# MarcoMeter/episodic-transformer-memory-ppo

Hardware: AMD Instinct MI355X
Metric: env-steps/sec (whole node) MinigridMemory 3x84x84 (higher is better)
Workload: dtype f32

## Files before the change

episodic-transformer-memory-ppo_amd/csrc/conv_b3.hip:

```cpp
#include "etm_common.h"

#include <utility>

namespace {
typedef __bf16 bf16x8 __attribute__((ext_vector_type(8)));
typedef unsigned u32x4 __attribute__((ext_vector_type(4)));
typedef unsigned u32x2 __attribute__((ext_vector_type(2)));

struct B3Args {
  const float *x;
  const long long *img_index;
  const unsigned short *wp;
  const float *bias;
  const float *ymask;
  const unsigned *bits_in;
  const unsigned *src_bits;
  unsigned *bits_out;
  float *out;
  int N, n_groups;
};

__device__ __forceinline__ unsigned b3_cvt_pk(float a, float b) {
  unsigned r;
  asm("v_cvt_pk_bf16_f32 %0, %1, %2" : "=v"(r) : "v"(a), "v"(b));
  return r;
}
__device__ __forceinline__ void b3_split_pair(float a, float b, unsigned &h, unsigned &m, unsigned &l) {
  h = b3_cvt_pk(a, b);
  a -= __uint_as_float(h << 16); b -= __uint_as_float(h & 0xffff0000u);
  m = b3_cvt_pk(a, b);
  a -= __uint_as_float(m << 16); b -= __uint_as_float(m & 0xffff0000u);
  l = b3_cvt_pk(a, b);
}

template <class F, int... I>
__device__ __forceinline__ void b3_for_impl(F &&f, std::integer_sequence<int, I...>) { (f(std::integral_constant<int, I>{}), ...); }
template <int N, class F>
__device__ __forceinline__ void b3_for(F &&f) { b3_for_impl(f, std::make_integer_sequence<int, N>{}); }

template <bool DGRAD, int C, int HW, int KS, int S, int COUT, int G_, int BAND = 0, int WPC_ = 1, bool SWZ_ = false>
struct B3Geo {
  static constexpr int G = G_, WPC = WPC_;
  static constexpr bool SWZ = SWZ_;
  static constexpr bool U8 = false;
  static constexpr int HOUT = (HW - KS) / S + 1;
  static constexpr int T = KS / S;
  static constexpr int CI = DGRAD ? COUT : C;
  static constexpr int HI = DGRAD ? HOUT : HW;
  static constexpr bool THREE = CI == 3;
  static constexpr int RS = DGRAD ? HI + T - 1 : HI;
  static constexpr int NB = BAND > 0 ? HOUT / BAND : 1;
  static constexpr int HROWS = BAND > 0 ? (BAND - 1) * S + KS : HI;
  static constexpr int ROW0 = BAND * S;
  static constexpr int SLOTS = DGRAD ? (HI + 2 * (T - 1) - 1) * RS + HI + 2 * (T - 1) : HROWS * HI;
  static constexpr int CPB = THREE ? 6 : SWZ ? CI * 2 : (CI + 8) * 2;
  static constexpr int IMGB = (SLOTS * CPB + 15) / 16 * 16;
  static constexpr int PLANE = G * IMGB;
  static constexpr int HO = DGRAD ? HI + T - 1 : HOUT;
  static constexpr int PIXI = HO * HO;
  static constexpr int PIX = BAND > 0 ? BAND * HO : PIXI, M = G * PIX, MT = (M + 31) / 32;
  static constexpr int NOUT = DGRAD ? S * S * C : COUT;
  static constexpr int NT = NOUT / 32, RP = NT >= 4 ? 1 : 4 / NT, TPW = (MT + RP - 1) / RP;
  static constexpr int TAPS = DGRAD ? T : KS;
  static constexpr int K = TAPS * TAPS * CI, KSTEPS = K / 16;
  static constexpr int KPT = THREE ? 1 : CI / 16;
  static constexpr int Q_IMG = HI * HI * CI / 4;
  static constexpr int Q_UNIT = HROWS * HI * CI / 4;
  static constexpr int Q_ROW0 = ROW0 * HI * CI / 4;
  static constexpr int NQ = (G * Q_UNIT + 255) / 256;
  static constexpr int LPK = (NQ + KSTEPS - 1) / KSTEPS;
  static constexpr int HRES = DGRAD ? S * HO : HO;
  static constexpr int CRES = DGRAD ? C : COUT;
  static_assert(K % 16 == 0 && NOUT % 32 == 0 && (THREE || CI % 16 == 0) && (NT == 1 || NT == 2 || NT == 4), "layer geometry");
  static_assert(!DGRAD || (HW % S == 0 && KS % S == 0 && HI + T - 1 == HW / S && Q_IMG % 8 == 0), "backward-data: class grids tile the input");
  static_assert(!SWZ || (!DGRAD && CI == 32 && SLOTS % 16 == 0 && IMGB == SLOTS * CPB), "swizzled slots: 64-byte pixels of four chunks");
  static_assert(BAND == 0 || (!DGRAD && G == 1 && HOUT % BAND == 0 && (ROW0 * HI * CI) % 4 == 0 && (HROWS * HI * CI) % 4 == 0), "bands: forward, one unit per group");

  static constexpr int slot(int y, int x) {
    if (DGRAD) return (y + T - 1) * RS + (x + T - 1);
    if (S == 2) return y * HI + (x & 1) * (HI / 2) + (x >> 1);
    return y * HI + x;
  }
  static constexpr int tap_slot(int ks) {
    const int tap = ks / KPT, ty = tap / TAPS, tx = tap % TAPS;
    if (!DGRAD && S == 2) return ty * HI + (tx & 1) * (HI / 2) + (tx >> 1);
    return ty * RS + tx;
  }
  static constexpr int tap_bytes(int ks) {
    const int tap = ks / KPT, cg = ks % KPT, ty = tap / TAPS, tx = tap % TAPS;
    int so = ty * RS + tx;
    if (!DGRAD && S == 2) so = ty * HI + (tx & 1) * (HI / 2) + (tx >> 1);
    return so * CPB + cg * 32;
  }
};

template <class Base>
struct B3GeoBytes : Base {
  static constexpr bool U8 = true;
};

template <class L, bool DGRAD, int C, int S>
__global__ __launch_bounds__(256, L::WPC) void conv_b3_kernel(const B3Args p) {
  constexpr bool U8 = L::U8;
  static_assert(!U8 || (L::THREE && !DGRAD && L::G == 1 && (L::Q_IMG * 4) % 16 == 0 && (L::Q_UNIT * 4) % 16 == 0 && (L::Q_ROW0 * 4) % 16 == 0),
                "byte images: layer 1 forward, units of whole 16-byte loads");
  constexpr int Q16 = L::Q_UNIT / 4;
  constexpr int G = L::G, TPW = L::TPW, NT = L::NT, RP = L::RP, KSTEPS = L::KSTEPS, NQ = U8 ? (Q16 + 255) / 256 : L::NQ, PD = 3;
  constexpr int LPK = U8 ? (NQ + KSTEPS - 1) / KSTEPS : L::LPK;
  extern __shared__ __attribute__((aligned(16))) unsigned char lds[];
  const int tid = threadIdx.x, lane = tid & 63, col = lane & 31, half = lane >> 5;
  const int wave = __builtin_amdgcn_readfirstlane(tid >> 6);
  const int ct = wave % NT, rp = wave / NT;

  if (DGRAD) {
    for (int e = tid; e < 3 * L::PLANE / 16; e += 256) reinterpret_cast<u32x4 *>(lds)[e] = u32x4{0u, 0u, 0u, 0u};
    __syncthreads();
  }

  int a_off[TPW], a_offb[TPW];
#pragma unroll
  for (int t = 0; t < TPW; ++t) {
    const int m = min((rp + t * RP) * 32 + col, L::M - 1);
    const int g = m / L::PIX, r = m - g * L::PIX, oy = r / L::HO, ox = r - oy * L::HO;
    if (L::THREE) {
      const int e0 = (oy * S * L::HI + ox * S) * 3;
      a_off[t] = g * L::IMGB + e0 * 2 + half * 16;
      a_offb[t] = g * L::IMGB + e0 * 2 + half * ((L::HI * 3 - 16) * 2);
    } else {
      const int q0 = DGRAD ? oy * L::RS + ox : (S == 2 ? (2 * oy) * L::HI + ox : (oy * S) * L::HI + ox * S);
      a_off[t] = L::SWZ ? g * L::SLOTS + q0 : g * L::IMGB + q0 * L::CPB + half * 16;
      a_offb[t] = 0;
    }
  }

  int o_t[TPW], g_t[TPW];
#pragma unroll
  for (int t = 0; t < TPW; ++t) {
    const int T_ = rp + t * RP, m = T_ * 32 + col;
    const int g = m / L::PIX, r = m - g * L::PIX;
    int o;
    if (DGRAD) {
      constexpr int CT_ = C >= 32 ? C / 32 : 1;
      const int cls = ct / CT_, py = cls / S, px = cls - py * S;
      const int cy = r / L::HO, cx = r - cy * L::HO;
      o = (((g * L::HRES + S * cy + py) * L::HRES + S * cx + px) * C + (ct % CT_) * 32 + 4 * half) * 4;
    } else {
      o = (((L::NB > 1 ? 0 : g * L::PIXI) + r) * L::CRES + ct * 32 + 4 * half) * 4;
    }
    o_t[t] = (T_ < L::MT && m < L::M) ? o : -1;
    g_t[t] = g;
  }

  auto fill_dst = [&](int u) {
    const int q = tid + u * 256;
    if constexpr (U8) return q * 32;
    const int g = q / L::Q_UNIT, qi = q - g * L::Q_UNIT;
    if (L::THREE) return g * L::IMGB + qi * 8;
    const int pix = qi / (L::CI / 4), c4 = qi - pix * (L::CI / 4), y = pix / L::HI, x = pix - y * L::HI;
    if (L::SWZ) {
      const int q = g * L::SLOTS + L::slot(y, x);
      return q * L::CPB + (((c4 >> 1) ^ ((q >> 2) & 3)) << 4) + (c4 & 1) * 8;
    }
    return g * L::IMGB + L::slot(y, x) * L::CPB + c4 * 8;
  };
  auto group_rsrc = [&](int grp) {
    const bool exists = grp < p.n_groups;
    const int u0 = exists ? grp * G : 0;
    const int n0 = u0 / L::NB, b0 = u0 - n0 * L::NB;
    const long long src = (G == 1 && p.img_index) ? p.img_index[n0] : (long long)n0;
    const int units = exists ? min(G, p.N * L::NB - u0) : 0;
    if constexpr (U8)
      return __builtin_amdgcn_make_buffer_rsrc((void *)(reinterpret_cast<const unsigned char *>(p.x) + src * (L::Q_IMG * 4) + b0 * (L::Q_ROW0 * 4)), 0,
                                               units * L::Q_UNIT * 4, 0x00020000);
    else
      return __builtin_amdgcn_make_buffer_rsrc((void *)(p.x + src * (L::Q_IMG * 4) + b0 * (L::Q_ROW0 * 4)), 0, units * L::Q_UNIT * 16, 0x00020000);
  };
  f32x4 fill[NQ];
  unsigned fbits[DGRAD ? NQ : 1];
  int fdst[NQ];
#pragma unroll
  for (int u = 0; u < NQ; ++u) fdst[u] = fill_dst(u);
  auto fill_to_lds = [&]() {
    if constexpr (U8) {
#pragma unroll
      for (int u = 0; u < NQ; ++u) {
        if (tid + u * 256 < Q16) {
          const u32x4 raw = __builtin_bit_cast(u32x4, fill[u]);
#pragma unroll
          for (int w = 0; w < 4; ++w) {
            const f32x4 v = etm_bytes4_unit(raw[w]);
            unsigned h0, m0, l0, h1, m1, l1;
            b3_split_pair(v[0], v[1], h0, m0, l0);
            b3_split_pair(v[2], v[3], h1, m1, l1);
            const int d = fdst[u] + w * 8;
            *reinterpret_cast<u32x2 *>(lds + d) = u32x2{h0, h1};
            *reinterpret_cast<u32x2 *>(lds + L::PLANE + d) = u32x2{m0, m1};
            *reinterpret_cast<u32x2 *>(lds + 2 * L::PLANE + d) = u32x2{l0, l1};
          }
        }
      }
      return;
    }
#pragma unroll
    for (int u = 0; u < NQ; ++u) {
      if (tid + u * 256 < G * L::Q_UNIT) {
        if (DGRAD && p.src_bits) {
          const unsigned nib = fbits[DGRAD ? u : 0] >> (((tid + u * 256) & 7) * 4);
#pragma unroll
          for (int e = 0; e < 4; ++e) fill[u][e] = (nib >> e) & 1u ? fill[u][e] : 0.f;
        }
        unsigned h0, m0, l0, h1, m1, l1;
        b3_split_pair(fill[u][0], fill[u][1], h0, m0, l0);
        b3_split_pair(fill[u][2], fill[u][3], h1, m1, l1);
        const int d = fdst[u];
        *reinterpret_cast<u32x2 *>(lds + d) = u32x2{h0, h1};
        *reinterpret_cast<u32x2 *>(lds + L::PLANE + d) = u32x2{m0, m1};
        *reinterpret_cast<u32x2 *>(lds + 2 * L::PLANE + d) = u32x2{l0, l1};
      }
    }
  };
  auto group_bits_rsrc = [&](int grp) {
    const bool exists = DGRAD && p.src_bits && grp < p.n_groups;
    const int n0 = exists ? grp * G : 0;
    const int images = exists ? min(G, p.N - n0) : 0;
    return __builtin_amdgcn_make_buffer_rsrc((void *)((p.src_bits ? p.src_bits : (const unsigned *)p.x) + (long long)n0 * (L::Q_IMG / 8)), 0,
                                             images * (L::Q_IMG / 8) * 4, 0x00020000);
  };
  auto fill_load = [&](int u, __amdgpu_buffer_rsrc_t rx, __amdgpu_buffer_rsrc_t rbits) {
    fill[u] = __builtin_bit_cast(f32x4, __builtin_amdgcn_raw_buffer_load_b128(rx, tid * 16, u * 4096, 0));
    if (DGRAD && p.src_bits) fbits[DGRAD ? u : 0] = __builtin_amdgcn_raw_buffer_load_b32(rbits, ((tid + u * 256) >> 3) * 4, 0, 0);
  };

  int grp = blockIdx.x;
  {
    const __amdgpu_buffer_rsrc_t rx = group_rsrc(grp), rxb = group_bits_rsrc(grp);
#pragma unroll
    for (int u = 0; u < NQ; ++u) fill_load(u, rx, rxb);
    fill_to_lds();
  }
  f32x4 bias4[4];
#pragma unroll
  for (int j = 0; j < 4; ++j)
    bias4[j] = DGRAD ? f32x4{0.f, 0.f, 0.f, 0.f} : *reinterpret_cast<const f32x4 *>(p.bias + ct * 32 + 8 * j + 4 * half);
  const __amdgpu_buffer_rsrc_t rw = __builtin_amdgcn_make_buffer_rsrc((void *)p.wp, 0, KSTEPS * NT * 3 * 1024, 0x00020000);
  const int w_lane = lane * 16, w_ct = ct * 3072;
  auto w_load = [&](int ks, int pl) { return __builtin_amdgcn_raw_buffer_load_b128(rw, w_lane, w_ct + (ks * NT * 3 + pl) * 1024, 0); };
  const __amdgpu_buffer_rsrc_t ro = __builtin_amdgcn_make_buffer_rsrc((void *)p.out, 0, (int)((long long)p.N * L::HRES * L::HRES * L::CRES * 4), 0x00020000);
  const __amdgpu_buffer_rsrc_t rm = __builtin_amdgcn_make_buffer_rsrc((void *)(p.ymask ? p.ymask : p.out), 0,
                                                                       p.ymask ? (int)((long long)p.N * L::HRES * L::HRES * L::CRES * 4) : 0, 0x00020000);
  const unsigned *bits_p = DGRAD ? p.bits_in : p.bits_out;
  const __amdgpu_buffer_rsrc_t rb = __builtin_amdgcn_make_buffer_rsrc((void *)(bits_p ? (const void *)bits_p : (const void *)p.out), 0,
                                                                       bits_p ? (int)((long long)p.N * L::HRES * L::HRES * L::CRES / 8) : 0, 0x00020000);

  for (; grp < p.n_groups; grp += gridDim.x) {
    __syncthreads();
    const __amdgpu_buffer_rsrc_t nrx = group_rsrc(grp + gridDim.x), nrxb = group_bits_rsrc(grp + gridDim.x);
    int o[TPW];
    unsigned relu_bits[TPW];
    {
      const int u0 = grp * G, units = min(G, p.N * L::NB - u0);
      const int n0 = u0 / L::NB, b0 = u0 - n0 * L::NB;
      const int gbase = DGRAD ? n0 * (L::HRES * L::HRES * C * 4) : (n0 * L::PIXI + b0 * L::PIX) * (L::CRES * 4);
#pragma unroll
      for (int t = 0; t < TPW; ++t) o[t] = (o_t[t] >= 0 && g_t[t] < units) ? o_t[t] + gbase : 0x7ffffff0;
      if (DGRAD && p.bits_in) {
#pragma unroll
        for (int t = 0; t < TPW; ++t) relu_bits[t] = __builtin_amdgcn_raw_buffer_load_b32(rb, (o[t] >> 7) << 2, 0, 0);
      }
    }
    f32x16 acc[TPW], acs[TPW];
#pragma unroll
    for (int t = 0; t < TPW; ++t)
#pragma unroll
      for (int r = 0; r < 16; ++r) acc[t][r] = acs[t][r] = 0.f;
    u32x4 b[PD][3];
#pragma unroll
    for (int s = 0; s < PD; ++s)
#pragma unroll
      for (int pl = 0; pl < 3; ++pl) b[s][pl] = w_load(s, pl);

    auto read_x = [&](u32x4(&xf)[3], int t, auto ksc) {
      constexpr int ks = decltype(ksc)::value;
      if constexpr (L::THREE) {
        constexpr int g8 = 2 * ks, ky = g8 / 3, o8 = g8 % 3;
        constexpr bool cross = (ks % 3) == 1;
        const int base = (cross ? a_offb[t] : a_off[t]) + (ky * L::HI * 3 + o8 * 8) * 2;
#pragma unroll
        for (int pl = 0; pl < 3; ++pl) {
          const u32x2 lo = *reinterpret_cast<const u32x2 *>(lds + pl * L::PLANE + base);
          const u32x2 hi = *reinterpret_cast<const u32x2 *>(lds + pl * L::PLANE + base + 8);
          xf[pl] = u32x4{lo[0], lo[1], hi[0], hi[1]};
        }
      } else if constexpr (L::SWZ) {
        constexpr int chunk0 = (ks % L::KPT) * 2;
        const int q = a_off[t] + L::tap_slot(ks);
        const int off = q * L::CPB + (((chunk0 | half) ^ ((q >> 2) & 3)) << 4);
#pragma unroll
        for (int pl = 0; pl < 3; ++pl) xf[pl] = *reinterpret_cast<const u32x4 *>(lds + pl * L::PLANE + off);
      } else {
        constexpr int off = L::tap_bytes(ks);
#pragma unroll
        for (int pl = 0; pl < 3; ++pl) xf[pl] = *reinterpret_cast<const u32x4 *>(lds + pl * L::PLANE + a_off[t] + off);
      }
    };

    u32x4 xa[2][3];
    read_x(xa[0], 0, std::integral_constant<int, 0>{});
    b3_for<KSTEPS>([&](auto ksc) {
      constexpr int ks = decltype(ksc)::value, s = ks % PD;
      b3_for<TPW>([&](auto tc) {
        constexpr int t = decltype(tc)::value, cur = (ks * TPW + t) & 1;
        if constexpr (t + 1 < TPW) read_x(xa[cur ^ 1], t + 1, std::integral_constant<int, ks>{});
        else if constexpr (ks + 1 < KSTEPS) read_x(xa[cur ^ 1], 0, std::integral_constant<int, ks + 1>{});
        __builtin_amdgcn_sched_barrier(0);
        const bf16x8 w1 = __builtin_bit_cast(bf16x8, b[s][0]), w2 = __builtin_bit_cast(bf16x8, b[s][1]), w3 = __builtin_bit_cast(bf16x8, b[s][2]);
        const bf16x8 x1 = __builtin_bit_cast(bf16x8, xa[cur][0]), x2 = __builtin_bit_cast(bf16x8, xa[cur][1]), x3 = __builtin_bit_cast(bf16x8, xa[cur][2]);
        acs[t] = __builtin_amdgcn_mfma_f32_32x32x16_bf16(w1, x3, acs[t], 0, 0, 0);
        acs[t] = __builtin_amdgcn_mfma_f32_32x32x16_bf16(w3, x1, acs[t], 0, 0, 0);
        acs[t] = __builtin_amdgcn_mfma_f32_32x32x16_bf16(w2, x2, acs[t], 0, 0, 0);
        acs[t] = __builtin_amdgcn_mfma_f32_32x32x16_bf16(w1, x2, acs[t], 0, 0, 0);
        acs[t] = __builtin_amdgcn_mfma_f32_32x32x16_bf16(w2, x1, acs[t], 0, 0, 0);
        acc[t] = __builtin_amdgcn_mfma_f32_32x32x16_bf16(w1, x1, acc[t], 0, 0, 0);
        __builtin_amdgcn_sched_barrier(0);
      });
      if constexpr (ks + PD < KSTEPS) {
#pragma unroll
        for (int pl = 0; pl < 3; ++pl) b[s][pl] = w_load(ks + PD, pl);
      }
#pragma unroll
      for (int u = ks * LPK; u < (ks + 1) * LPK; ++u)
        if (u < NQ) fill_load(u, nrx, nrxb);
      __builtin_amdgcn_sched_barrier(0);
    });

    {
      f32x4 mk[2][4];
      auto mask_load = [&](int t) {
#pragma unroll
        for (int j = 0; j < 4; ++j) mk[t & 1][j] = __builtin_bit_cast(f32x4, __builtin_amdgcn_raw_buffer_load_b128(rm, o[t] + 32 * j, 0, 0));
      };
      const bool by_values = DGRAD && p.ymask && !p.bits_in;
      if (by_values) mask_load(0);
#pragma unroll
      for (int t = 0; t < TPW; ++t) {
        if (by_values && t + 1 < TPW) mask_load(t + 1);
        unsigned pattern = 0;
#pragma unroll
        for (int j = 0; j < 4; ++j) {
          f32x4 v{acc[t][4 * j] + acs[t][4 * j], acc[t][4 * j + 1] + acs[t][4 * j + 1], acc[t][4 * j + 2] + acs[t][4 * j + 2], acc[t][4 * j + 3] + acs[t][4 * j + 3]};
          if (DGRAD) {
            if (p.bits_in) {
#pragma unroll
              for (int q = 0; q < 4; ++q) v[q] = ((relu_bits[t] >> (8 * j + 4 * half + q)) & 1u) ? v[q] : 0.f;
            } else if (p.ymask) {
#pragma unroll
              for (int q = 0; q < 4; ++q) v[q] = mk[t & 1][j][q] > 0.f ? v[q] : 0.f;
            }
          } else {
#pragma unroll
            for (int q = 0; q < 4; ++q) {
              v[q] = fmaxf(v[q] + bias4[j][q], 0.f);
              pattern |= (v[q] > 0.f ? 1u : 0u) << (8 * j + q);
            }
          }
          __builtin_amdgcn_raw_buffer_store_b128(__builtin_bit_cast(u32x4, v), ro, o[t] + 32 * j, 0, 0);
        }
        if (!DGRAD && p.bits_out) {
          pattern <<= 4 * half;
          pattern |= (unsigned)__shfl_xor((int)pattern, 32, 64);
          __builtin_amdgcn_raw_buffer_store_b32(pattern, rb, half ? 0x7ffffff0 : ((o[t] >> 7) << 2), 0, 0);
        }
      }
    }

    __syncthreads();
    fill_to_lds();
  }
}

template <class L, bool DGRAD, int C, int S>
int launch_b3_geo(const B3Args &p0, hipStream_t st) {
  constexpr int G = L::G, WPC = L::WPC;
  B3Args p = p0;
  if (G > 1 && p.img_index) return ETM_EUNSUPPORTED;
  if ((long long)p.N * L::HRES * L::HRES * L::CRES * 4 >= 0x7ffffff0ll) return ETM_EUNSUPPORTED;
  p.n_groups = (p.N * L::NB + G - 1) / G;
  constexpr size_t lds = 3 * (size_t)L::PLANE;
  static_assert(lds * WPC <= 160 * 1024, "LDS of a CU");
  auto kern = conv_b3_kernel<L, DGRAD, C, S>;
  static bool attr_set = false;
  if (!attr_set) { (void)hipFuncSetAttribute((const void *)kern, hipFuncAttributeMaxDynamicSharedMemorySize, (int)lds); attr_set = true; }
  const int grid = p.n_groups < 256 * WPC ? p.n_groups : 256 * WPC;
  hipLaunchKernelGGL(kern, dim3((unsigned)grid), dim3(256), lds, st, p);
  return etm_launch_status();
}
template <bool DGRAD, int C, int HW, int KS, int S, int COUT, int G, int BAND = 0, int WPC = 1, bool SWZ = false>
int launch_b3(const B3Args &p, hipStream_t st) {
  return launch_b3_geo<B3Geo<DGRAD, C, HW, KS, S, COUT, G, BAND, WPC, SWZ>, DGRAD, C, S>(p, st);
}

constexpr int B3_MAXP = 8;
struct B3Pack {
  const float *w[B3_MAXP];
  unsigned short *out[B3_MAXP];
  int dgrad[B3_MAXP], Cout[B3_MAXP], C[B3_MAXP], KS[B3_MAXP], S[B3_MAXP], first_block[B3_MAXP + 1];
  int n;
};
__global__ __launch_bounds__(256) void conv_b3_pack_kernel(const B3Pack g) {
  int i = 0;
  while (i + 1 < g.n && (int)blockIdx.x >= g.first_block[i + 1]) ++i;
  const float *__restrict__ w = g.w[i];
  const int Cout = g.Cout[i], C = g.C[i], KS = g.KS[i], S = g.S[i];
  const int total = Cout * C * KS * KS;
  const int e = ((int)blockIdx.x - g.first_block[i]) * 256 + threadIdx.x;
  if (e >= total) return;
  const int j = e & 7, lane = (e >> 3) & 63, rest = e >> 9;
  float v;
  if (!g.dgrad[i]) {
    const int NT = Cout >> 5, nt = rest % NT, ks = rest / NT;
    const int co = nt * 32 + (lane & 31), k = ks * 16 + (lane >> 5) * 8 + j;
    const int c = k % C, kx = (k / C) % KS, ky = k / (C * KS);
    v = w[((co * C + c) * KS + ky) * KS + kx];
  } else {
    const int T = KS / S, NT = (S * S * C) >> 5, nt = rest % NT, ks = rest / NT;
    const int n = nt * 32 + (lane & 31), k = ks * 16 + (lane >> 5) * 8 + j;
    const int cls = n / C, c = n - cls * C, py = cls / S, px = cls - py * S;
    const int tap = k / Cout, co = k - tap * Cout, ta = tap / T, tb = tap - ta * T;
    v = w[((co * C + c) * KS + (py + S * (T - 1 - ta))) * KS + (px + S * (T - 1 - tb))];
  }
  unsigned h, m, l;
  b3_split_pair(v, 0.f, h, m, l);
  unsigned short *o = g.out[i] + ((size_t)rest * 3 * 64 + lane) * 8 + j;
  o[0] = (unsigned short)h; o[64 * 8] = (unsigned short)m; o[2 * 64 * 8] = (unsigned short)l;
}
}

extern "C" int etm_conv_b3_pack(const float *const *w, uint16_t *const *out, const int *dgrad, const int *Cout, const int *C, const int *KS,
                                const int *S, int n, void *stream) {
  (void)hipGetLastError();
  if (!w || !out || !dgrad || !Cout || !C || !KS || !S || n <= 0 || n > B3_MAXP) return ETM_EINVAL;
  B3Pack g{};
  int blocks = 0;
  for (int i = 0; i < n; ++i) {
    if (!w[i] || !out[i] || Cout[i] <= 0 || C[i] <= 0 || KS[i] <= 0 || S[i] <= 0) return ETM_EINVAL;
    if (!dgrad[i] && (Cout[i] % 32 != 0 || (KS[i] * KS[i] * C[i]) % 16 != 0)) return ETM_EUNSUPPORTED;
    if (dgrad[i] && (KS[i] % S[i] != 0 || (S[i] * S[i] * C[i]) % 32 != 0 || C[i] % 32 != 0 || ((KS[i] / S[i]) * (KS[i] / S[i]) * Cout[i]) % 16 != 0))
      return ETM_EUNSUPPORTED;
    g.w[i] = w[i]; g.out[i] = out[i]; g.dgrad[i] = dgrad[i]; g.Cout[i] = Cout[i]; g.C[i] = C[i]; g.KS[i] = KS[i]; g.S[i] = S[i];
    g.first_block[i] = blocks;
    blocks += (Cout[i] * C[i] * KS[i] * KS[i] + 255) / 256;
  }
  g.first_block[n] = blocks;
  g.n = n;
  hipLaunchKernelGGL(conv_b3_pack_kernel, dim3((unsigned)blocks), dim3(256), 0, (hipStream_t)stream, g);
  return etm_launch_status();
}

extern "C" int etm_conv_b3_fwd(const float *x, const int64_t *x_index, const uint16_t *w_b3, const float *bias, float *y, uint32_t *relu_bits, int N,
                               int C, int H, int W, int Cout, int KH, int KW, int S, void *stream) {
  (void)hipGetLastError();
  if (!x || !w_b3 || !bias || !y || N <= 0) return ETM_EINVAL;
  if ((uintptr_t)x % 16 || (uintptr_t)y % 16 || (uintptr_t)w_b3 % 16 || (uintptr_t)bias % 16) return ETM_EINVAL;
  if (H != W || KH != KW) return ETM_EUNSUPPORTED;
  hipStream_t st = (hipStream_t)stream;
  B3Args p{x, (const long long *)x_index, w_b3, bias, nullptr, nullptr, nullptr, relu_bits, y, N, 0};
  EtmProfScope prof(etm_conv_layer_kid(ETM_K_CONV_TRAIN_FWD, ETM_K_CONV_FWD_L1, ETM_K_CONV_FWD_L2, ETM_K_CONV_FWD_L3, KH), st);
  if (C == 3 && H == 84 && KH == 8 && S == 4 && Cout == 32) return launch_b3<false, 3, 84, 8, 4, 32, 1, 10, 2>(p, st);
  if (C == 32 && H == 20 && KH == 4 && S == 2 && Cout == 64) return launch_b3<false, 32, 20, 4, 2, 64, 2, 0, 1, true>(p, st);
  if (C == 64 && H == 9 && KH == 3 && S == 1 && Cout == 64) return launch_b3<false, 64, 9, 3, 1, 64, 2, 0, 2>(p, st);
  return ETM_EUNSUPPORTED;
}

extern "C" int etm_conv_b3_fwd_u8(const uint8_t *x, const int64_t *x_index, const uint16_t *w_b3, const float *bias, float *y, uint32_t *relu_bits,
                                  int N, int C, int H, int W, int Cout, int KH, int KW, int S, void *stream) {
  (void)hipGetLastError();
  if (!x || !w_b3 || !bias || !y || N <= 0) return ETM_EINVAL;
  if ((uintptr_t)x % 16 || (uintptr_t)y % 16 || (uintptr_t)w_b3 % 16 || (uintptr_t)bias % 16) return ETM_EINVAL;
  if (!(C == 3 && H == 84 && W == 84 && KH == 8 && KW == 8 && S == 4 && Cout == 32)) return ETM_EUNSUPPORTED;
  hipStream_t st = (hipStream_t)stream;
  B3Args p{reinterpret_cast<const float *>(x), (const long long *)x_index, w_b3, bias, nullptr, nullptr, nullptr, relu_bits, y, N, 0};
  EtmProfScope prof(ETM_K_CONV_FWD_L1, st);
  return launch_b3_geo<B3GeoBytes<B3Geo<false, 3, 84, 8, 4, 32, 1, 10, 2>>, false, 3, 4>(p, st);
}

extern "C" int etm_conv_b3_dgrad(const float *dy, const uint32_t *dy_relu_bits, const uint16_t *w_b3, const float *y_below, const uint32_t *relu_bits,
                                 float *dx, int N, int C, int H, int W, int Cout, int KH, int KW, int S, void *stream) {
  (void)hipGetLastError();
  if (!dy || !w_b3 || !dx || N <= 0) return ETM_EINVAL;
  if ((uintptr_t)dy % 16 || (uintptr_t)dx % 16 || (uintptr_t)w_b3 % 16 || (uintptr_t)y_below % 16 || (uintptr_t)relu_bits % 4 || (uintptr_t)dy_relu_bits % 4) return ETM_EINVAL;
  if (H != W || KH != KW) return ETM_EUNSUPPORTED;
  hipStream_t st = (hipStream_t)stream;
  B3Args p{dy, nullptr, w_b3, nullptr, y_below, relu_bits, dy_relu_bits, nullptr, dx, N, 0};
  EtmProfScope prof(etm_conv_layer_kid(ETM_K_CONV_TRAIN_DGRAD, -1, ETM_K_CONV_DGRAD_L2, ETM_K_CONV_DGRAD_L3, KH), st);
  if (C == 32 && H == 20 && KH == 4 && S == 2 && Cout == 64) return launch_b3<true, 32, 20, 4, 2, 64, 2, 0, 1>(p, st);
  if (C == 64 && H == 9 && KH == 3 && S == 1 && Cout == 64) return launch_b3<true, 64, 9, 3, 1, 64, 3>(p, st);
  return ETM_EUNSUPPORTED;
}
```

episodic-transformer-memory-ppo_amd/csrc/conv_b3_wgrad.hip:

```cpp
#include "etm_common.h"

#include <utility>

namespace {
typedef __bf16 bf16x8 __attribute__((ext_vector_type(8)));
typedef unsigned u32x4 __attribute__((ext_vector_type(4)));
typedef unsigned u32x2 __attribute__((ext_vector_type(2)));

struct W3Args {
  const float *x;
  const long long *img_index;
  const float *dy;
  const unsigned *dy_bits;
  float *partial;
  int N, n_groups;
};

__device__ __forceinline__ unsigned w3_cvt_pk(float a, float b) {
  unsigned r;
  asm("v_cvt_pk_bf16_f32 %0, %1, %2" : "=v"(r) : "v"(a), "v"(b));
  return r;
}
__device__ __forceinline__ void w3_split_pair(float a, float b, unsigned &h, unsigned &m, unsigned &l) {
  h = w3_cvt_pk(a, b);
  a -= __uint_as_float(h << 16); b -= __uint_as_float(h & 0xffff0000u);
  m = w3_cvt_pk(a, b);
  a -= __uint_as_float(m << 16); b -= __uint_as_float(m & 0xffff0000u);
  l = w3_cvt_pk(a, b);
}
template <int OFF>
__device__ __forceinline__ u32x2 w3_tr_read(unsigned addr) {
  static_assert(OFF >= 0 && OFF < 65536, "16-bit offset field");
  u32x2 v;
  asm volatile("ds_read_b64_tr_b16 %0, %1 offset:%2" : "=v"(v) : "v"(addr), "n"(OFF) : "memory");
  return v;
}
template <class F, int... I>
__device__ __forceinline__ void w3_for_impl(F &&f, std::integer_sequence<int, I...>) { (f(std::integral_constant<int, I>{}), ...); }
template <int N, class F>
__device__ __forceinline__ void w3_for(F &&f) { w3_for_impl(f, std::make_integer_sequence<int, N>{}); }

template <int C, int HW, int KS, int S, int COUT, int G_, int BAND, int PSPLIT_, int NW_, int WPC_ = 1>
struct W3Geo {
  static constexpr int G = G_, PSPLIT = PSPLIT_, NW = NW_, NTH = NW_ * 64, WPC = WPC_;
  static constexpr int HOUT = (HW - KS) / S + 1;
  static constexpr bool THREE = C == 3;
  static constexpr bool U8 = false;
  static constexpr int NB = BAND > 0 ? HOUT / BAND : 1;
  static constexpr int OROWS = BAND > 0 ? BAND : HOUT;
  static constexpr int HROWS = (OROWS - 1) * S + KS;
  static constexpr int ROW0 = BAND * S;
  static constexpr int CPB = THREE ? 6 : (C + 8) * 2;
  static constexpr int IMGB = (HROWS * HW * CPB + 15) / 16 * 16;
  static constexpr int XPLANE = G * IMGB;
  static constexpr int PIX = OROWS * HOUT, PIXI = HOUT * HOUT, M = G * PIX, STEPS = (M + 15) / 16, MPAD = STEPS * 16;
  static constexpr int CPBD = (COUT + 8) * 2;
  static constexpr int DPLANE = MPAD * CPBD;
  static constexpr int XBYTES = 3 * XPLANE, LDS = XBYTES + 3 * DPLANE;
  static constexpr int K = KS * KS * C, KT = K / 32, CT = COUT / 32;
  static constexpr int KPARTS = PSPLIT == 1 ? NW / 2 : 2;
  static constexpr int KTW = (KT + KPARTS - 1) / KPARTS, CTW = 1;
  static constexpr int KTPT = THREE ? 1 : C / 32;
  static constexpr int QX_IMG = HW * HW * C / 4, QX = HROWS * HW * C / 4, QX_ROW0 = ROW0 * HW * C / 4;
  static constexpr int QD_IMG = PIXI * COUT / 4, QD = PIX * COUT / 4;
  static constexpr int NQX = (G * QX + NTH - 1) / NTH, NQD = (G * QD + NTH - 1) / NTH;
  static_assert(K % 64 == 0 && COUT % 32 == 0 && NTH % (COUT / 4) == 0 && (THREE || C % 32 == 0), "layer geometry");
  static_assert(PSPLIT == 1 ? CT == 2 : (CT == 1 && PSPLIT == NW / 2 && KT % 2 == 0), "wave split");
  static_assert(QD_IMG % 8 == 0 && QD % 8 == 0, "pattern words: 32 elements each");
  static_assert(BAND == 0 || (G == 1 && HOUT % BAND == 0 && (ROW0 * HW * C) % 4 == 0 && (HROWS * HW * C) % 4 == 0 && (PIX * COUT) % 4 == 0), "bands");
  static constexpr int slot(int y, int x) { return S == 2 ? y * HW + (x & 1) * (HW / 2) + (x >> 1) : y * HW + x; }
  static constexpr int ktile_bytes(int kt) {
    const int tap = kt / KTPT, sub = kt % KTPT, ty = tap / KS, tx = tap % KS;
    const int so = S == 2 ? ty * HW + (tx & 1) * (HW / 2) + (tx >> 1) : ty * HW + tx;
    return so * CPB + sub * 64;
  }
};

template <class Base>
struct W3GeoBytes : Base {
  static constexpr bool U8 = true;
};

template <class L, int C, int HW, int S, int COUT>
__global__ __launch_bounds__(L::NTH, L::WPC * L::NW / 4) void conv_b3_wgrad_kernel(const W3Args p) {
  constexpr bool U8 = L::U8;
  static_assert(!U8 || (L::THREE && L::G == 1 && (L::QX_IMG * 4) % 16 == 0 && (L::QX * 4) % 16 == 0 && (L::QX_ROW0 * 4) % 16 == 0),
                "byte images: layer 1, units of whole 16-byte loads");
  constexpr int QX16 = L::QX / 4;
  constexpr int G = L::G, KTW = L::KTW, CTW = L::CTW, STEPS = L::STEPS, NQX = U8 ? (QX16 + L::NTH - 1) / L::NTH : L::NQX, NQD = L::NQD, NTH = L::NTH;
  extern __shared__ __attribute__((aligned(16))) unsigned char lds[];
  const int tid = threadIdx.x, lane = tid & 63;
  const int wave = __builtin_amdgcn_readfirstlane(tid >> 6);
  const int kpart = L::PSPLIT == 1 ? (wave >> 1) : (wave & 1);
  const int kt0 = kpart * L::KT / L::KPARTS, nkt = (kpart + 1) * L::KT / L::KPARTS - kt0;
  const int ct0 = L::PSPLIT == 1 ? (wave & 1) : 0;
  const int sp = L::PSPLIT == 1 ? 0 : (wave >> 1);

  for (int e = tid; e < L::LDS / 16; e += NTH) reinterpret_cast<u32x4 *>(lds)[e] = u32x4{0u, 0u, 0u, 0u};
  __syncthreads();

  const int prow = (lane & 15) >> 2, cofs = ((lane >> 4) & 1) * 16 + (lane & 3) * 4, p8 = (lane >> 5) * 8;
  const unsigned lds0 = (unsigned)(size_t)lds;
  unsigned *tabl = reinterpret_cast<unsigned *>(lds + L::LDS);
  if (wave == 0) {
#pragma unroll
    for (int s = 0; s < STEPS; ++s)
#pragma unroll
      for (int j = 0; j < 2; ++j) {
        int m = 16 * s + p8 + 4 * j + prow;
        if (m >= L::M) m = 0;
        const int g = m / L::PIX, r = m - g * L::PIX, oy = r / L::HOUT, ox = r - oy * L::HOUT;
        int b;
        if (L::THREE) b = g * L::IMGB + ((oy * S * HW + ox * S) * 3) * 2;
        else b = g * L::IMGB + (S == 2 ? (2 * oy) * HW + ox : (oy * S) * HW + ox * S) * L::CPB + cofs * 2;
        tabl[(2 * s + j) * 64 + lane] = lds0 + (unsigned)b;
      }
  }
  int koff[KTW];
#pragma unroll
  for (int i = 0; i < KTW; ++i) {
    if (L::THREE) {
      const int k0 = 32 * (kt0 + i) + cofs, ky = k0 / 24, off = k0 - ky * 24;
      koff[i] = (ky * HW * 3 + off) * 2;
    } else {
      koff[i] = 0;
#pragma unroll
      for (int kp = 0; kp < L::KPARTS; ++kp)
        if (kp == kpart) koff[i] = L::ktile_bytes(kp * L::KT / L::KPARTS + i < L::KT ? kp * L::KT / L::KPARTS + i : 0);
    }
  }
  const unsigned dbase = lds0 + L::XBYTES + (unsigned)((p8 + prow) * L::CPBD + cofs * 2 + ct0 * 64);

  auto x_dst = [&](int u) {
    const int q = tid + u * NTH;
    if constexpr (U8) return q * 32;
    const int g = q / L::QX, qi = q - g * L::QX;
    if (L::THREE) return g * L::IMGB + qi * 8;
    const int pix = qi / (C / 4), c4 = qi - pix * (C / 4), y = pix / HW, x = pix - y * HW;
    return g * L::IMGB + L::slot(y, x) * L::CPB + c4 * 8;
  };
  auto d_dst = [&](int u) {
    const int q = tid + u * NTH;
    const int pix = q / (COUT / 4), c4 = q - pix * (COUT / 4);
    return L::XBYTES + pix * L::CPBD + c4 * 8;
  };
  auto unit_rsrc = [&](int grp, bool grad) {
    const bool exists = grp < p.n_groups;
    const int u0 = exists ? grp * G : 0;
    const int n0 = u0 / L::NB, b0 = u0 - n0 * L::NB;
    const int units = exists ? min(G, p.N * L::NB - u0) : 0;
    if (grad) return __builtin_amdgcn_make_buffer_rsrc((void *)(p.dy + (long long)n0 * (L::QD_IMG * 4) + b0 * (L::QD * 4)), 0, units * L::QD * 16, 0x00020000);
    const long long src = (G == 1 && p.img_index) ? p.img_index[n0] : (long long)n0;
    if constexpr (U8)
      return __builtin_amdgcn_make_buffer_rsrc((void *)(reinterpret_cast<const unsigned char *>(p.x) + src * (L::QX_IMG * 4) + b0 * (L::QX_ROW0 * 4)), 0,
                                               units * L::QX * 4, 0x00020000);
    else
      return __builtin_amdgcn_make_buffer_rsrc((void *)(p.x + src * (L::QX_IMG * 4) + b0 * (L::QX_ROW0 * 4)), 0, units * L::QX * 16, 0x00020000);
  };
  f32x4 fx[NQX], fd[NQD];
  unsigned fdb[NQD];
  f32x4 bsum{0.f, 0.f, 0.f, 0.f};
  auto issue_fill = [&](int grp) {
    const __amdgpu_buffer_rsrc_t rx = unit_rsrc(grp, false), rd = unit_rsrc(grp, true);
#pragma unroll
    for (int u = 0; u < NQD; ++u) fd[u] = __builtin_bit_cast(f32x4, __builtin_amdgcn_raw_buffer_load_b128(rd, tid * 16, u * (NTH * 16), 0));
    if (p.dy_bits) {
      const bool exists = grp < p.n_groups;
      const int u0 = exists ? grp * G : 0, n0 = u0 / L::NB, b0 = u0 - n0 * L::NB;
      const int units = exists ? min(G, p.N * L::NB - u0) : 0;
      const __amdgpu_buffer_rsrc_t rdb = __builtin_amdgcn_make_buffer_rsrc((void *)(p.dy_bits + (long long)n0 * (L::QD_IMG / 8) + b0 * (L::QD / 8)), 0,
                                                                            units * (L::QD / 8) * 4, 0x00020000);
#pragma unroll
      for (int u = 0; u < NQD; ++u) fdb[u] = __builtin_amdgcn_raw_buffer_load_b32(rdb, ((tid + u * NTH) >> 3) * 4, 0, 0);
    }
#pragma unroll
    for (int u = 0; u < NQX; ++u) fx[u] = __builtin_bit_cast(f32x4, __builtin_amdgcn_raw_buffer_load_b128(rx, tid * 16, u * (NTH * 16), 0));
  };
  auto put = [&](const f32x4 &v, int d, int plane_bytes) {
    unsigned h0, m0, l0, h1, m1, l1;
    w3_split_pair(v[0], v[1], h0, m0, l0);
    w3_split_pair(v[2], v[3], h1, m1, l1);
    *reinterpret_cast<u32x2 *>(lds + d) = u32x2{h0, h1};
    *reinterpret_cast<u32x2 *>(lds + plane_bytes + d) = u32x2{m0, m1};
    *reinterpret_cast<u32x2 *>(lds + 2 * plane_bytes + d) = u32x2{l0, l1};
  };
  auto fill_to_lds = [&]() {
#pragma unroll
    for (int u = 0; u < NQD; ++u)
      if (tid + u * NTH < G * L::QD) {
        if (p.dy_bits) {
          const unsigned nib = fdb[u] >> (((tid + u * NTH) & 7) * 4);
#pragma unroll
          for (int q = 0; q < 4; ++q) fd[u][q] = (nib >> q) & 1u ? fd[u][q] : 0.f;
        }
#pragma unroll
        for (int q = 0; q < 4; ++q) bsum[q] += fd[u][q];
        put(fd[u], d_dst(u), L::DPLANE);
      }
    if constexpr (U8) {
#pragma unroll
      for (int u = 0; u < NQX; ++u)
        if (tid + u * NTH < QX16) {
          const u32x4 raw = __builtin_bit_cast(u32x4, fx[u]);
#pragma unroll
          for (int w = 0; w < 4; ++w) put(etm_bytes4_unit(raw[w]), x_dst(u) + w * 8, L::XPLANE);
        }
    } else {
#pragma unroll
      for (int u = 0; u < NQX; ++u)
        if (tid + u * NTH < G * L::QX) put(fx[u], x_dst(u), L::XPLANE);
    }
  };

  f32x16 acc[KTW][CTW], acs[KTW][CTW];
#pragma unroll
  for (int i = 0; i < KTW; ++i)
#pragma unroll
    for (int t = 0; t < CTW; ++t)
#pragma unroll
      for (int r = 0; r < 16; ++r) acc[i][t][r] = acs[i][t][r] = 0.f;

  int grp = blockIdx.x;
  issue_fill(grp);
  fill_to_lds();
  for (; grp < p.n_groups; grp += gridDim.x) {
    __syncthreads();
    issue_fill(grp + gridDim.x);

    unsigned t0 = 0, t1 = 0;
    auto read_a = [&](u32x4(&a)[3], auto sc, auto ic) {
      constexpr int i = decltype(ic)::value;
      const unsigned a0 = t0 + (unsigned)koff[i], a1 = t1 + (unsigned)koff[i];
      w3_for<3>([&](auto plc) {
        constexpr int pl = decltype(plc)::value;
        const u32x2 lo = w3_tr_read<pl * L::XPLANE>(a0), hi = w3_tr_read<pl * L::XPLANE>(a1);
        a[pl] = u32x4{lo[0], lo[1], hi[0], hi[1]};
      });
    };
    auto read_b = [&](u32x4(&b)[3], auto sc) {
      constexpr int s = decltype(sc)::value;
      w3_for<3>([&](auto plc) {
        constexpr int pl = decltype(plc)::value;
        const u32x2 lo = w3_tr_read<pl * L::DPLANE + 16 * s * L::CPBD>(dbase), hi = w3_tr_read<pl * L::DPLANE + (16 * s + 4) * L::CPBD>(dbase);
        b[pl] = u32x4{lo[0], lo[1], hi[0], hi[1]};
      });
    };

    w3_for<STEPS>([&](auto sc) {
      constexpr int s = decltype(sc)::value;
      if (L::PSPLIT > 1 && (s % L::PSPLIT) != sp) return;
      t0 = tabl[(2 * s) * 64 + lane]; t1 = tabl[(2 * s + 1) * 64 + lane];
      u32x4 bf[CTW][3];
      static_assert(CTW == 1, "one channel tile per wave");
      read_b(bf[0], sc);
      constexpr bool DB = L::NW == 4;
      u32x4 af[DB ? 2 : 1][3];
      read_a(af[0], sc, std::integral_constant<int, 0>{});
      w3_for<KTW>([&](auto ic) {
        constexpr int i = decltype(ic)::value, cur = DB ? (i & 1) : 0;
        if constexpr (!DB && i > 0) read_a(af[0], sc, ic);
        if constexpr (DB && i + 1 < KTW) read_a(af[cur ^ 1], sc, std::integral_constant<int, i + 1>{});
        asm volatile("s_waitcnt lgkmcnt(%3)" : "+v"(af[cur][0]), "+v"(af[cur][1]), "+v"(af[cur][2]) : "n"(DB && i + 1 < KTW ? 6 : 0) : "memory");
        if constexpr (i == 0) {
#pragma unroll
          for (int t = 0; t < CTW; ++t) asm volatile("" : "+v"(bf[t][0]), "+v"(bf[t][1]), "+v"(bf[t][2]));
        }
        __builtin_amdgcn_sched_barrier(0);
        const bf16x8 x1 = __builtin_bit_cast(bf16x8, af[cur][0]), x2 = __builtin_bit_cast(bf16x8, af[cur][1]), x3 = __builtin_bit_cast(bf16x8, af[cur][2]);
        if (i < nkt)
#pragma unroll
        for (int t = 0; t < CTW; ++t) {
          const bf16x8 d1 = __builtin_bit_cast(bf16x8, bf[t][0]), d2 = __builtin_bit_cast(bf16x8, bf[t][1]), d3 = __builtin_bit_cast(bf16x8, bf[t][2]);
          acs[i][t] = __builtin_amdgcn_mfma_f32_32x32x16_bf16(x1, d3, acs[i][t], 0, 0, 0);
          acs[i][t] = __builtin_amdgcn_mfma_f32_32x32x16_bf16(x3, d1, acs[i][t], 0, 0, 0);
          acs[i][t] = __builtin_amdgcn_mfma_f32_32x32x16_bf16(x2, d2, acs[i][t], 0, 0, 0);
          acs[i][t] = __builtin_amdgcn_mfma_f32_32x32x16_bf16(x1, d2, acs[i][t], 0, 0, 0);
          acs[i][t] = __builtin_amdgcn_mfma_f32_32x32x16_bf16(x2, d1, acs[i][t], 0, 0, 0);
          acc[i][t] = __builtin_amdgcn_mfma_f32_32x32x16_bf16(x1, d1, acc[i][t], 0, 0, 0);
        }
        __builtin_amdgcn_sched_barrier(0);
      });
    });

    __syncthreads();
    fill_to_lds();
  }

#pragma unroll
  for (int i = 0; i < KTW; ++i)
#pragma unroll
    for (int r = 0; r < 16; ++r) acc[i][0][r] += acs[i][0][r];
  constexpr int KC = L::K * COUT;
  float *dst = p.partial + (long long)blockIdx.x * (KC + COUT);
  const int col = lane & 31;
  __syncthreads();
  if (L::PSPLIT > 1) {
    float *red = reinterpret_cast<float *>(lds);
    static_assert(L::PSPLIT == 1 || (L::PSPLIT - 1) * 2 * KTW * 16 * 64 * 4 <= L::LDS, "reduction scratch");
    if (sp > 0) {
#pragma unroll
      for (int i = 0; i < KTW; ++i)
#pragma unroll
        for (int r = 0; r < 16; ++r) red[((((sp - 1) * 2 + kpart) * KTW + i) * 16 + r) * 64 + lane] = acc[i][0][r];
    }
    __syncthreads();
    if (sp == 0) {
#pragma unroll
      for (int i = 0; i < KTW; ++i)
#pragma unroll
        for (int r = 0; r < 16; ++r) {
          const int k = (kt0 + i) * 32 + mfma32_row(r, lane);
          float v = acc[i][0][r];
#pragma unroll
          for (int c = 1; c < L::PSPLIT; ++c) v += red[((((c - 1) * 2 + kpart) * KTW + i) * 16 + r) * 64 + lane];
          dst[(long long)k * COUT + col] = v;
        }
    }
  } else {
#pragma unroll
    for (int i = 0; i < KTW; ++i)
      if (i < nkt) {
#pragma unroll
        for (int r = 0; r < 16; ++r) {
          const int k = (kt0 + i) * 32 + mfma32_row(r, lane);
          dst[(long long)k * COUT + ct0 * 32 + col] = acc[i][0][r];
        }
      }
  }
  __syncthreads();
  f32x4 *bs = reinterpret_cast<f32x4 *>(lds);
  bs[tid] = bsum;
  __syncthreads();
  if (tid < COUT) {
    float total = 0.f;
    for (int t = tid >> 2; t < NTH; t += COUT / 4) total += reinterpret_cast<const float *>(bs + t)[tid & 3];
    dst[KC + tid] = total;
  }
}

template <class L_, int C, int HW, int S, int COUT>
struct W3Run {
  using L = L_;
  static constexpr int G = L::G, WPC = L::WPC;
  static constexpr int LDS_ALL = L::LDS + L::STEPS * 2 * 64 * 4;
  static_assert(LDS_ALL * WPC <= 160 * 1024, "LDS of a CU");
  static int slices(int N) {
    const int groups = (N * L::NB + G - 1) / G;
    return groups < 256 * WPC ? groups : 256 * WPC;
  }
  static int launch(const W3Args &p0, hipStream_t st) {
    W3Args p = p0;
    if (G > 1 && p.img_index) return ETM_EUNSUPPORTED;
    p.n_groups = (p.N * L::NB + G - 1) / G;
    auto kern = conv_b3_wgrad_kernel<L, C, HW, S, COUT>;
    static bool attr_set = false;
    if (!attr_set) { (void)hipFuncSetAttribute((const void *)kern, hipFuncAttributeMaxDynamicSharedMemorySize, (int)LDS_ALL); attr_set = true; }
    hipLaunchKernelGGL(kern, dim3((unsigned)slices(p.N)), dim3(L::NTH), LDS_ALL, st, p);
    return etm_launch_status();
  }
};
template <int C, int HW, int KS, int S, int COUT, int G, int BAND, int PSPLIT, int NW, int WPC = 1>
using W3 = W3Run<W3Geo<C, HW, KS, S, COUT, G, BAND, PSPLIT, NW, WPC>, C, HW, S, COUT>;
using W3L1 = W3<3, 84, 8, 4, 32, 1, 5, 2, 4, 2>;
using W3L2 = W3<32, 20, 4, 2, 64, 1, 0, 1, 8>;
using W3L3 = W3<64, 9, 3, 1, 64, 2, 0, 1, 8>;
using W3L1U8 = W3Run<W3GeoBytes<W3L1::L>, 3, 84, 4, 32>;

int w3_layer(int C, int H, int W, int Cout, int KH, int KW, int S) {
  if (H != W || KH != KW) return 0;
  if (C == 3 && H == 84 && KH == 8 && S == 4 && Cout == 32) return 1;
  if (C == 32 && H == 20 && KH == 4 && S == 2 && Cout == 64) return 2;
  if (C == 64 && H == 9 && KH == 3 && S == 1 && Cout == 64) return 3;
  return 0;
}
}

extern "C" int etm_conv_b3_wgrad_slices(int N, int C, int H, int W, int Cout, int KH, int KW, int S) {
  if (N <= 0) return 0;
  switch (w3_layer(C, H, W, Cout, KH, KW, S)) {
    case 1: return W3L1::slices(N);
    case 2: return W3L2::slices(N);
    case 3: return W3L3::slices(N);
  }
  return 0;
}

extern "C" int etm_conv_b3_wgrad(const float *x, const int64_t *x_index, const float *dy, const uint32_t *dy_relu_bits, float *workspace,
                                 int64_t workspace_bytes, int N, int C, int H, int W, int Cout, int KH, int KW, int S, void *stream) {
  (void)hipGetLastError();
  if (!x || !dy || !workspace || N <= 0) return ETM_EINVAL;
  if ((uintptr_t)x % 16 || (uintptr_t)dy % 16 || (uintptr_t)workspace % 16) return ETM_EINVAL;
  const int layer = w3_layer(C, H, W, Cout, KH, KW, S);
  if (!layer) return ETM_EUNSUPPORTED;
  const int slices = etm_conv_b3_wgrad_slices(N, C, H, W, Cout, KH, KW, S);
  if (workspace_bytes < (int64_t)slices * ((int64_t)KH * KW * C * Cout + Cout) * (int64_t)sizeof(float)) return ETM_EWORKSPACE;
  hipStream_t st = (hipStream_t)stream;
  W3Args p{x, (const long long *)x_index, dy, dy_relu_bits, workspace, N, 0};
  EtmProfScope prof(etm_conv_layer_kid(ETM_K_CONV_TRAIN_WGRAD, ETM_K_CONV_WGRAD_L1, ETM_K_CONV_WGRAD_L2, ETM_K_CONV_WGRAD_L3, KH), st);
  switch (layer) {
    case 1: return W3L1::launch(p, st);
    case 2: return W3L2::launch(p, st);
    default: return W3L3::launch(p, st);
  }
}

extern "C" int etm_conv_b3_wgrad_u8(const uint8_t *x, const int64_t *x_index, const float *dy, const uint32_t *dy_relu_bits, float *workspace,
                                    int64_t workspace_bytes, int N, int C, int H, int W, int Cout, int KH, int KW, int S, void *stream) {
  (void)hipGetLastError();
  if (!x || !dy || !workspace || N <= 0) return ETM_EINVAL;
  if ((uintptr_t)x % 16 || (uintptr_t)dy % 16 || (uintptr_t)workspace % 16) return ETM_EINVAL;
  if (w3_layer(C, H, W, Cout, KH, KW, S) != 1) return ETM_EUNSUPPORTED;
  const int slices = W3L1U8::slices(N);
  if (workspace_bytes < (int64_t)slices * ((int64_t)KH * KW * C * Cout + Cout) * (int64_t)sizeof(float)) return ETM_EWORKSPACE;
  hipStream_t st = (hipStream_t)stream;
  W3Args p{reinterpret_cast<const float *>(x), (const long long *)x_index, dy, dy_relu_bits, workspace, N, 0};
  EtmProfScope prof(ETM_K_CONV_WGRAD_L1, st);
  return W3L1U8::launch(p, st);
}
```

episodic-transformer-memory-ppo_amd/etm/lib.py:

```python
import ctypes
import os

import torch

_HERE = os.path.dirname(os.path.abspath(__file__))
LIB_PATH = os.path.join(_HERE, "libetm_hip.so")
ABI_VERSION = 61

_lib = None

_P = ctypes.c_void_p
_I = ctypes.c_int
_L = ctypes.c_int64
_F = ctypes.c_float
_D = ctypes.c_double

class RolloutGroup(ctypes.Structure):
    _fields_ = [("graph_exec", ctypes.c_void_p), ("stream", ctypes.c_void_p), ("ready", ctypes.c_void_p), ("n_procs", ctypes.c_int32),
                ("ready_stride", ctypes.c_int32), ("lo", ctypes.c_int32), ("hi", ctypes.c_int32), ("obs_src", ctypes.c_void_p),
                ("stage_dst", ctypes.c_void_p), ("ss_dst", ctypes.c_void_p)]


SIGNATURES = {
    "etm_abi_version": (_I, []),
    "etm_error_string": (ctypes.c_char_p, [_I]),
    "etm_mha_fwd": (_I, [_P, _L, _L, _P, _P, _P, _P, _P, _P, _P, _F, _P, _P, _P, _P, _P, _P, _P, _P, _I, _I, _I, _I, _P]),
    "etm_mha_bwd_workspace_bytes": (_L, [_I, _I, _I]),
    "etm_mha_bwd": (_I, [_P, _L, _L, _P, _P, _P, _P, _P, _P, _P, _P, _P, _P, _P, _P, _P, _P, _P, _P, _P, _P, _P, _P, _P, _P,
                         _P, _L, _I, _I, _I, _I, _P]),
    "etm_attn_cached": (_I, [_P, _L, _L, _P, _P, _P, _P, _P, _P, _I, _I, _I, _I, _P]),
    "etm_reset_rows": (_I, [_P, _P, _P, _I, _L, _P]),
    "etm_rollout_window": (_I, [_P, _P, _P, _P, _P, _P, _P, _P, _P, _P, _P, _P, _L, _I, _I, _I, _P]),
    "etm_rollout_sample": (_I, [_P, _P, _P, _P, _P, _P, _P, _P, _P, _I, _I, _P]),
    "etm_rollout_sample_branched": (_I, [_P, _P, _P, _P, _P, _P, _P, _P, _P, _I, _P, _I, _P]),
    "etm_rollout_sample_gaussian": (_I, [_P, _P, _P, _P, _P, _P, _P, _P, _P, _P, _P, _P, _I, _I, _P]),
    "etm_add_layernorm": (_I, [_P, _P, _I, _P, _P, _P, _F, _P, _I, _I, _P]),
    "etm_conv_relu": (_I, [_P, _P, _L, _P, _P, _P, _I, _I, _I, _I, _I, _I, _I, _I, _I, _I, _P]),
    "etm_upload": (_I, [_P, _P, _L, _P]),
    "etm_graph_launch": (_I, [_P, _P]),
    "etm_host_direct_write_init": (_I, [_I]),
    "etm_host_store_fence": (_I, [_I]),
    "etm_host_register": (_I, [_P, _L]),
    "etm_host_unregister": (_I, [_P]),
    "etm_rollout_drive": (_I, [_P, _I, _I, _I, _I, _L, _L, _P, _P, _P, _P, _L, _P, _L, _P, _P, _I, _I, _D, _P, _P]),
    "etm_comm_unique_id": (_I, [_P]),
    "etm_comm_init": (_I, [_P, _I, _I, ctypes.POINTER(ctypes.c_void_p)]),
    "etm_allreduce_f32": (_I, [_P, _P, _P, _L, _P]),
    "etm_comm_destroy": (_I, [_P]),
    "etm_rollout_policy": (_I, [_P, _P, _P, _P, _P, _P, _P, _P, _P, _P, _P, _P, _P, _P, _P, _P, _I, _I, _I, _I, _P]),
    "etm_rollout_policy_branched": (_I, [_P, _P, _P, _P, _P, _P, _P, _P, _P, _P, _P, _P, _P, _P, _P, _P, _I, _I, _I, _P, _I, _P]),
    "etm_rollout_policy_gaussian": (_I, [_P, _P, _P, _P, _P, _P, _P, _P, _P, _P, _P, _P, _P, _P, _P, _P, _P, _P, _P, _I, _I, _I, _I, _P]),
    "etm_conv_pack_weights": (_I, [_P, _P, _P, _I, _I, _I, _I, _I, _P]),
    "etm_gather_rows": (_I, [_P, _P, _P, _I, _P, _L, _L, _P]),
    "etm_group_norms": (_I, [_P, _P, _P, _I, _P, _I, _P, _P, _P]),
    "etm_step_head": (_I, [_P, _P, _P, _I, _P, _I, _P, _L, _L, _P, _P, _P, _P]),
    "etm_group_norms_step": (_I, [_P, _P, _P, _I, _P, _I, _P, _P, _P, _P, _I, _P, _I, _P, _P]),
    "etm_step_end": (_I, [_P, _I, _P, _I, _P, _P]),
    "etm_relu_bwd_colsum_workspace_bytes": (_L, [_I, _I]),
    "etm_relu_bwd_colsum": (_I, [_P, _P, _P, _P, _P, _L, _I, _I, _P]),
    "etm_host_copier_create": (_P, [_I]),
    "etm_host_copier_destroy": (None, [_P]),
    "etm_host_copier_set_spin": (_I, [_P, _I]),
    "etm_host_copy": (_I, [_P, _P, _P, _L]),
    "etm_rollout_trxl_team": (_I, [_I]),
    "etm_rollout_trxl_set_placement": (_I, [_I]),
    "etm_rollout_trxl_grid": (_I, [_I, _I]),
    "etm_rollout_trxl_supported": (_I, [_I, _I, _I, _I, _I, _I]),
    "etm_rollout_trxl_gate_merged": (_I, [_I, _I]),
    "etm_rollout_trxl_scratch_bytes": (_L, [_I, _I, _I, _I]),
    "etm_rollout_trxl": (_I, [_P, _P, _P, _P, _I, _P, _L, _L, _P, _P, _P, _P, _P, _P, _P, _P, _P, _P, _P, _P, _P, _P, _P, _P, _P, _P, _P, _F,
                              _P, _L, _P, _P, _P, _P, _P, _L, _L, _L, _P, _I, _P, _P, _P, _P, _P, _P, _P, _P, _P, _P, _I,
                              _I, _I, _I, _I, _I, _I, _I, _I, _I, _P]),
    "etm_rollout_trxl_group": (_I, [_P, _P, _P, _P, _I, _P, _L, _L, _P, _P, _P, _P, _P, _P, _P, _P, _P, _P, _P, _P, _P, _P, _P, _P, _P, _P, _P, _F,
                                    _P, _L, _P, _P, _P, _P, _P, _L, _L, _L, _P, _I, _P, _P, _P, _P, _P, _P, _P, _P, _P, _P, _I,
                                    _I, _I, _I, _I, _I, _I, _I, _I, _I, _P]),
    "etm_rollout_trxl_branched": (_I, [_P, _P, _P, _P, _I, _P, _L, _L, _P, _P, _P, _P, _P, _P, _P, _P, _P, _P, _P, _P, _P, _P, _P, _P, _P, _P, _P, _F,
                                       _P, _L, _P, _P, _P, _P, _P, _L, _L, _L, _P, _I, _P, _P, _P, _P, _P, _P, _P, _P, _P, _P, _I,
                                       _I, _I, _I, _I, _I, _I, _I, _I, _P, _I, _P]),
    "etm_rollout_trxl_group_branched": (_I, [_P, _P, _P, _P, _I, _P, _L, _L, _P, _P, _P, _P, _P, _P, _P, _P, _P, _P, _P, _P, _P, _P, _P, _P, _P, _P, _P, _F,
                                             _P, _L, _P, _P, _P, _P, _P, _L, _L, _L, _P, _I, _P, _P, _P, _P, _P, _P, _P, _P, _P, _P, _I,
                                             _I, _I, _I, _I, _I, _I, _I, _I, _P, _I, _P]),
    "etm_rollout_trxl_group_supported": (_I, [_I] * 8),
    "etm_rollout_trxl_gaussian": (_I, [_P, _P, _P, _P, _I, _P, _L, _L, _P, _P, _P, _P, _P, _P, _P, _P, _P, _P, _P, _P, _P, _P, _P, _P, _P, _P, _P,
                                       _P, _F, _P, _L, _P, _P, _P, _P, _P, _L, _L, _L, _P, _I, _P, _P, _P, _P, _P, _P, _P, _P, _P, _P,
                                       _I, _I, _I, _I, _I, _I, _I, _I, _I, _I, _P, _P, _P]),
    "etm_rollout_trxl_group_gaussian": (_I, [_P, _P, _P, _P, _I, _P, _L, _L, _P, _P, _P, _P, _P, _P, _P, _P, _P, _P, _P, _P, _P, _P, _P, _P, _P, _P,
                                             _P, _P, _F, _P, _L, _P, _P, _P, _P, _P, _L, _L, _L, _P, _I, _P, _P, _P, _P, _P, _P, _P, _P, _P,
                                             _P, _I, _I, _I, _I, _I, _I, _I, _I, _I, _I, _P, _P, _P]),
    "etm_rollout_trxl_supported_branched": (_I, [_I, _I, _I, _I, _P, _I, _I]),
    "etm_rollout_trxl_supported_gaussian": (_I, [_I] * 6),
    "etm_rollout_trxl_group_supported_gaussian": (_I, [_I] * 8),
    "etm_rollout_trxl_group_supported_branched": (_I, [_I, _I, _I, _I, _P, _I, _I, _I, _I]),
    "etm_rollout_trxl_group_grid": (_I, []),
    "etm_rollout_trxl_group_scratch_bytes": (_L, [_I]),
    "etm_window_set_skip_masked": (_I, [_I]),
    "etm_rollout_hidden_splits": (_I, [_I]),
    "etm_rollout_hidden_partial": (_I, [_P, _P, _P, _I, _I, _I, _P]),
    "etm_rollout_conv3_hidden_supported": (_I, [_I, _I, _I, _I, _I, _I, _I, _I]),
    "etm_rollout_conv3_hidden": (_I, [_P, _P, _P, _P, _P, _I, _I, _I, _I, _P]),
    "etm_rollout_heads": (_I, [_P, _P, _P, _P, _P, _P, _P, _I, _I, _I, _P]),
    "etm_gru_gate_rz": (_I, [_P, _P, _P, _P, _P, _P, _I, _I, _P]),
    "etm_gru_gate_out": (_I, [_P, _P, _P, _P, _P, _I, _I, _P]),
    "etm_block_row_groups": (_I, [_I]),
    "etm_ln_train_fwd": (_I, [_P, _P, _I, _P, _P, _P, _F, _P, _P, _P, _I, _I, _P]),
    "etm_ln_train_bwd_workspace_bytes": (_L, [_I, _I]),
    "etm_ln_train_bwd_partial_rows": (_I, [_I]),
    "etm_relu_bwd_colsum_partial_rows": (_I, [_I]),
    "etm_colsum_reduce_max_problems": (_I, []),
    "etm_colsum_reduce_grouped": (_I, [_P, _P, _P, _P, _P, _I, _P]),
    "etm_ln_train_bwd": (_I, [_P, _P, _P, _P, _P, _P, _P, _I, _P, _P, _P, _P, _L, _I, _I, _P]),
    "etm_gate_train_rz": (_I, [_P, _P, _P, _P, _P, _P, _P, _I, _I, _P]),
    "etm_gate_train_out": (_I, [_P, _P, _P, _P, _P, _P, _I, _I, _P]),
    "etm_gate_train_bwd_workspace_bytes": (_L, [_I, _I]),
    "etm_gate_train_bwd_partial_rows": (_I, [_I]),
    "etm_gate_train_bwd1": (_I, [_P, _P, _P, _P, _P, _P, _P, _P, _P, _P, _L, _I, _I, _P]),
    "etm_gate_train_bwd2": (_I, [_P, _P, _P, _P, _P, _P, _P, _I, _I, _P]),
    "etm_conv_train_fwd": (_I, [_P, _P, _L, _P, _P, _P, _I, _I, _I, _I, _I, _I, _I, _I, _I, _P]),
    "etm_conv_train_set_fwd_lds": (_I, [_I]),
    "etm_conv_train_set_wgrad_lds": (_I, [_I]),
    "etm_conv_train_set_dgrad_lds": (_I, [_I]),
    "etm_conv_pack_weights_grouped": (_I, [_P, _P, _P, _P, _P, _P, _P, _P, _I, _P]),
    "etm_conv_train_wgrad_slices": (_I, [_I] * 8),
    "etm_conv_wgrad_reduce_grouped": (_I, [_P, _P, _P, _P, _P, _P, _P, _P, _I, _P]),
    "etm_conv_train_dgrad": (_I, [_P, _P, _P, _P, _I, _I, _I, _I, _I, _I, _I, _I, _P]),
    "etm_conv_train_wgrad_workspace_bytes": (_L, [_I, _I, _I, _I, _I, _I, _I, _I]),
    "etm_conv_train_wgrad": (_I, [_P, _P, _P, _P, _P, _L, _I, _I, _I, _I, _I, _I, _I, _I, _P]),
    "etm_relu_mask": (_I, [_P, _P, _P, _L, _P]),
    "etm_conv_b3_pack": (_I, [_P, _P, _P, _P, _P, _P, _P, _I, _P]),
    "etm_conv_b3_fwd": (_I, [_P, _P, _P, _P, _P, _P, _I, _I, _I, _I, _I, _I, _I, _I, _P]),
    "etm_conv_b3_dgrad": (_I, [_P, _P, _P, _P, _P, _P, _I, _I, _I, _I, _I, _I, _I, _I, _P]),
    "etm_conv_b3_wgrad_slices": (_I, [_I] * 8),
    "etm_conv_b3_wgrad": (_I, [_P, _P, _P, _P, _P, _L, _I, _I, _I, _I, _I, _I, _I, _I, _P]),
    "etm_bytes_to_unit": (_I, [_P, _P, _P, _L, _L, _P]),
    "etm_conv_relu_u8": (_I, [_P, _P, _L, _P, _P, _P, _I, _I, _I, _I, _I, _I, _I, _I, _I, _I, _P]),
    "etm_conv_b3_fwd_u8": (_I, [_P, _P, _P, _P, _P, _P, _I, _I, _I, _I, _I, _I, _I, _I, _P]),
    "etm_conv_b3_wgrad_u8": (_I, [_P, _P, _P, _P, _P, _L, _I, _I, _I, _I, _I, _I, _I, _I, _P]),
    "etm_grouped_dw_supported": (_I, [_I, _I, _I, _I, _I, _I]),
    "etm_grouped_dw_max_problems": (_I, []),
    "etm_grouped_dw": (_I, [_P, _P, _P, _P, _I, _I, _P]),
    "etm_grouped_dw_tile_map": (_I, [_I, _P]),
    "etm_grouped_dw_tail_max_problems": (_I, []),
    "etm_grouped_dw_tail": (_I, [_P, _P, _P, _P, _I, _I, _P, _P, _P, _P, _P, _I, _P]),
    "etm_grad_sqnorm": (_I, [_P, _L, _P, _I, _P, _P]),
    "etm_adamw_clip": (_I, [_P, _P, _P, _P, _L, _P, _I, _P, _P, _D, _D, _D, _D, _F, _F, _P, _P]),
    "etm_grad_sqnorm_gated": (_I, [_P, _L, _P, _I, _P, _P, _F, _P, _P, _P]),
    "etm_adamw_clip_gated": (_I, [_P, _P, _P, _P, _L, _P, _I, _P, _P, _D, _D, _D, _D, _F, _F, _P, _P, _P]),
    "etm_grad_sqnorm_adaptive": (_I, [_P, _L, _P, _I, _P, _P, _P, _F, _F, _F, _F, _F, _P, _F, _P, _P, _P]),
    "etm_arena_digest": (_I, [_P, _L, _P, _I, _P, _P]),
    "etm_gae": (_I, [_P, _P, _P, _P, _F, _F, _P, _I, _I, _P]),
    "etm_gae_truncated": (_I, [_P, _P, _P, _P, _P, _P, _F, _F, _P, _I, _I, _P]),
    "etm_obs_stats_supported": (_I, [_I]),
    "etm_obs_stats_workspace_bytes": (_L, [_I, _I]),
    "etm_obs_stats_update": (_I, [_P, _I, _I, _P, _P, _P, _D, _P, _L, _P]),
    "etm_obs_normalize": (_I, [_P, _P, _P, _P, _F, _P, _L, _I, _P]),
    "etm_return_scale_workspace_bytes": (_L, [_I]),
    "etm_return_scale": (_I, [_P, _P, _P, _P, _D, _D, _F, _P, _I, _I, _P, _L, _P]),
    "etm_adv_stats": (_I, [_P, _I, _P, _P]),
    "etm_adv_stats_workspace_bytes": (_L, [_I]),
    "etm_adv_stats_ws": (_I, [_P, _I, _P, _P, _L, _P]),
    "etm_ppo_loss_workspace_bytes": (_L, [_I]),
    "etm_heads_loss_supported": (_I, [_I, _I, _I]),
    "etm_heads_loss_row_floats": (_I, [_I, _I]),
    "etm_heads_loss_workspace_bytes": (_L, [_I, _I, _I]),
    "etm_heads_loss": (_I, [_P, _P, _P, _P, _P, _P, _P, _P, _P, _L, _P, _L, _P, _P, _P, _D, _F, _F, _F, _F, _F, _P, _P, _P, _P, _P, _P, _P, _P, _L,
                            _I, _I, _I, _P]),
    "etm_heads_loss_supported_branched": (_I, [_I, _I, _P, _I]),
    "etm_heads_loss_supported_gaussian": (_I, [_I, _I, _I]),
    "etm_heads_loss_gaussian_row_floats": (_I, [_I, _I]),
    "etm_heads_loss_gaussian_workspace_bytes": (_L, [_I, _I, _I]),
    "etm_heads_loss_gaussian": (_I, [_P, _P, _P, _P, _P, _P, _P, _P, _P, _L, _P, _P, _L, _P, _P, _P, _D, _F, _F, _F, _F, _F, _P, _P, _P, _P, _P, _P,
                                     _P, _P, _L, _I, _I, _I, _P]),
    "etm_heads_loss_branched": (_I, [_P, _P, _P, _P, _P, _P, _P, _P, _P, _L, _P, _L, _P, _P, _P, _D, _F, _F, _F, _F, _F, _P, _P, _P, _P, _P, _P, _P,
                                     _P, _L, _I, _I, _P, _I, _P]),
    "etm_window_fwd": (_I, [_P, _L, _L, _P, _P, _P, _P, _P, _P, _P, _F, _P, _L, _L, _P, _P, _L, _L, _P, _I, _I, _I, _I, _I, _P]),
    "etm_window_ln_grad_rows": (_I, [_I]),
    "etm_window_ln_grad": (_I, [_P, _L, _L, _P, _P, _P, _P, _P, _P, _P, _P, _P, _L, _L, _P, _I, _I, _I, _I, _P]),
    "etm_window_ln_grad_from_outputs": (_I, [_P, _P, _P, _P, _P, _P, _P, _P, _L, _L, _P, _I, _I, _I, _I, _P]),
    "etm_window_ln_grad_guarded": (_I, [_P, _L, _L, _P, _P, _P, _P, _P, _P, _P, _P, _P, _L, _L, _P, _P, _F, _P, _I, _I, _I, _I, _P]),
    "etm_ln_row_stats": (_I, [_P, _F, _P, _L, _I, _P]),
    "etm_window_bwd": (_I, [_P, _L, _L, _P, _P, _P, _P, _P, _P, _P, _P, _P, _P, _L, _L, _P, _P, _L, _L, _I, _I, _I, _I, _P]),
    "etm_window_dx": (_I, [_P, _L, _L, _P, _P, _P, _P, _P, _P, _P, _P, _P, _P, _P, _P, _P, _I, _I, _I, _I, _P]),
    "etm_profile_enable": (_I, [_I]),
    "etm_profile_set_tag": (_I, [_I]),
    "etm_profile_kernel_count": (_I, []),
    "etm_profile_kernel_name": (ctypes.c_char_p, [_I]),
    "etm_profile_collect": (_I, [_P, _P]),
    "etm_ppo_loss": (_I, [_P, _P, _L, _P, _L, _P, _P, _P, _P, _D, _F, _F, _F, _F, _F, _I, _P, _P, _P, _P, _L, _P, _I, _I, _P]),
}
for _name, _extra in (("etm_rollout_sample_branched", [_P]), ("etm_rollout_policy_branched", [_P]), ("etm_rollout_trxl_branched", [_P]),
                      ("etm_rollout_trxl_group_branched", [_P]), ("etm_heads_loss", [_P]), ("etm_heads_loss_branched", [_P]),
                      ("etm_ppo_loss", [_P, _I])):
    _res, _args = SIGNATURES[_name]
    SIGNATURES[_name + "_masked"] = (_res, _args[:-1] + _extra + _args[-1:])
for _name, _extra in (("etm_rollout_sample_gaussian", [_P]), ("etm_rollout_policy_gaussian", [_P]), ("etm_rollout_trxl_gaussian", [_P]),
                      ("etm_rollout_trxl_group_gaussian", [_P])):
    _res, _args = SIGNATURES[_name]
    SIGNATURES[_name + "_means"] = (_res, _args[:-1] + _extra + _args[-1:])
_res, _args = SIGNATURES["etm_heads_loss_gaussian"]
SIGNATURES["etm_heads_loss_gaussian_kl"] = (_res, _args[:-1] + [_P, _L, _P] + _args[-1:])
SIGNATURES["etm_heads_loss_gaussian_kl_row_floats"] = (_I, [_I, _I])
SIGNATURES["etm_heads_loss_gaussian_kl_workspace_bytes"] = (_L, [_I, _I, _I])
del _name, _extra, _res, _args


def load():
    global _lib
    if _lib is not None:
        return _lib
    if not os.path.exists(LIB_PATH):
        raise RuntimeError(
            f"{LIB_PATH} is missing: the MI355X kernels are not built. Run `python -c 'import __graft_entry__ as g; g.build()'` "
            "or `make -C episodic-transformer-memory-ppo_amd/csrc`. There is no CPU fallback for this path.")
    if os.path.basename(LIB_PATH) != "libetm_hip.so":
        print(f"[etm] using the library build {LIB_PATH}", flush=True)
    lib = ctypes.CDLL(LIB_PATH)
    for name, (res, args) in SIGNATURES.items():
        fn = getattr(lib, name)
        fn.restype = res
        fn.argtypes = args
    if lib.etm_abi_version() != ABI_VERSION:
        raise RuntimeError(f"libetm_hip.so ABI {lib.etm_abi_version()} != expected {ABI_VERSION}; rebuild")
    _lib = lib
    return lib


def check(rc: int, what: str):
    if rc != 0:
        msg = load().etm_error_string(rc)
        raise RuntimeError(f"{what} failed ({rc}): {msg.decode() if msg else '?'}")


def profile_collect():
    import numpy as np
    lib = load()
    k = lib.etm_profile_kernel_count()
    ms = np.zeros(2 * k, dtype=np.float64)
    cnt = np.zeros(2 * k, dtype=np.int64)
    check(lib.etm_profile_collect(ms.ctypes.data, cnt.ctypes.data), "etm_profile_collect")
    out = {}
    for tag in (0, 1):
        for i in range(k):
            if cnt[tag * k + i]:
                out[(tag, lib.etm_profile_kernel_name(i).decode())] = (float(ms[tag * k + i]), int(cnt[tag * k + i]))
    return out
```

episodic-transformer-memory-ppo_amd/trainer.py:

```python
import os
import sys
import time
from collections import deque
from functools import partial

import numpy as np
import torch

def default_rollout_groups(num_workers: int, min_group: int) -> int:
    if num_workers % 2 == 0 and num_workers // 2 >= min_group:
        return 2
    return 1


from buffer import Buffer
from environments import action_space_kind, branch_bit_masks, empty_mask_branches, valid_action_share
from environments.vec_env import make_vec_env
from etm import lib as etm_lib
from etm import ops
from etm.ops import WindowSpec
from etm.optim import AdaptiveLr, FlatAdamW, KlGate
from model import ActorCriticModel, IndexedObservations
from utils import (adaptive_lr_section, kl_estimator_section, normalization_section, polynomial_decay, process_episode_info, target_kl_rows,
                   target_kl_section)
from rollout_plan import RolloutPlan, WorkerGroup, plan_rollout
from checkpoint import check_checkpoint_config, segment_first_worker_id
from trainer_parts import _CheckpointResume, _DataParallelStep, _NativeRolloutDrive, _RunOutputs


class _NullWriter:
    def add_scalar(self, *a, **k):
        pass

    def close(self):
        pass


def _make_writer(run_id):
    try:
        from torch.utils.tensorboard import SummaryWriter
    except Exception:
        return _NullWriter()
    os.makedirs("./summaries", exist_ok=True)
    return SummaryWriter("./summaries/" + run_id + time.strftime("/%Y%m%d-%H%M%S/"))


def build_window_tables(memory_length: int, max_episode_length: int):
    L, T = int(memory_length), int(max_episode_length)
    if T < L:
        raise ValueError(f"max_episode_steps ({T}) must be >= memory_length ({L})")
    mask = torch.tril(torch.ones((L, L), dtype=torch.float32), diagonal=-1)
    first = torch.clamp(torch.arange(T, dtype=torch.int64) - (L - 1), min=0)
    indices = first.unsqueeze(1) + torch.arange(L, dtype=torch.int64).unsqueeze(0)
    return mask, indices


def check_kernel_shapes(tcfg: dict):
    d, h, mem = tcfg["embed_dim"], tcfg["num_heads"], tcfg["memory_length"]
    if d % h != 0:
        raise ValueError("Embedding dimension needs to be divisible by the number of heads")
    hd = d // h
    problems = []
    if d % 32 != 0 or d > 1024:
        problems.append(f"embed_dim={d} (need a multiple of 32, <= 1024)")
    if hd % 32 != 0 or hd > 128:
        problems.append(f"head_dim={hd} (need 32, 64, 96 or 128)")
    if mem > 128:
        problems.append(f"memory_length={mem} (need <= 128)")
    if not problems and ops.attention_supported(d, h, mem, ln=tcfg.get("layer_norm") == "pre",
                                                pos_grad=tcfg.get("positional_encoding") == "learned") is None:
        problems.append(f"attention backward at embed_dim={d}, num_heads={h}, memory_length={mem}, layer_norm="
                        f"{tcfg.get('layer_norm')}, positional_encoding={tcfg.get('positional_encoding')} (LDS: see DESIGN.md section 6)")
    if problems:
        raise ValueError("transformer shape not supported by the MI355X kernels: " + "; ".join(problems))


def check_box_policy(config: dict, A=None):
    if A is None:
        A = config.get("environment", {}).get("continuous_actions")
        if A is None:
            return None
    A, hid = int(A), int(config["hidden_layer_size"])
    if not 1 <= A <= 8:
        raise ValueError(f"Box action space of {A} dimensions: the fused Gaussian heads + loss kernel takes 1 to 8")
    if not etm_lib.load().etm_heads_loss_supported_gaussian(1, hid, A):
        raise ValueError(f"Box action space with hidden_layer_size={hid}: the fused Gaussian heads + loss kernel needs a multiple of 64, "
                         "at most 512")
    return A


def check_byte_observation_transport(config, env=None):
    if env is None and config.get("worker_processes", False) and str(config["environment"].get("observation_dtype", "float32")) == "uint8":
        raise ValueError("worker_processes: true does not carry uint8 observations (the shared segment's rows are float32): "
                         "set worker_processes: false (in-process environments keep the bytes), or let the environment emit float32")


def check_truncation_transport(config, env=None):
    if env is None and config.get("worker_processes", False) and config.get("bootstrap_truncated", False):
        raise ValueError("worker_processes: true does not carry bootstrap_truncated: true (the shared segment has no row for a final "
                         "observation): set worker_processes: false (in-process environments hand it over in their info), or leave "
                         "bootstrap_truncated off")


def check_action_mask_config(config, env=None, action_space_shape=None, box=False):
    if not config.get("action_masks", False):
        return False
    from environments import MAX_MASKED_ACTIONS
    env_cfg = config.get("environment", {})
    if box or env_cfg.get("continuous_actions") is not None:
        raise ValueError("action_masks: true with a Box (continuous) action space: a Gaussian policy has no invalid actions to mask; "
                         "remove the key (the environment's bounds already clip the actions)")
    shape = action_space_shape
    if shape is None and env_cfg.get("type") == "Synthetic" and "num_actions" in env_cfg:
        n = env_cfg["num_actions"]
        shape = tuple(n) if isinstance(n, (list, tuple)) else (int(n),)
    if shape is not None and sum(int(a) for a in shape) > MAX_MASKED_ACTIONS:
        raise ValueError(f"action_masks: true with {sum(int(a) for a in shape)} actions over all branches: a step's mask is one 64-bit word "
                         f"per worker and takes at most {MAX_MASKED_ACTIONS}; remove the key, or reduce the action space")
    if env is None and config.get("worker_processes", False):
        raise ValueError("worker_processes: true does not carry action_masks: true (the shared segment has no row for a mask word): "
                         "set worker_processes: false (in-process environments hand the words over each step), or remove the key")
    if env is not None and not callable(getattr(env, "action_masks", None)):
        raise ValueError(f"action_masks: true, but the environment front-end {type(env).__name__} has no action_masks(): let the "
                         "environments offer action_masks() (environments/vec_env.py: the VecEnv protocol; a Synthetic environment needs "
                         "environment.action_mask_p), or remove the key")
    return True


def check_evaluation_config(config, world: int = 1):
    ev = config.get("evaluation")
    if ev is None:
        return None
    known = ("interval", "episodes_per_worker", "n_workers", "deterministic", "seed", "worker_steps")
    unknown = sorted(set(ev) - set(known))
    if unknown:
        raise ValueError(f"evaluation: unknown keys {unknown} (known: {list(known)})")
    out = dict(interval=int(ev.get("interval", 0) or 0), episodes_per_worker=int(ev.get("episodes_per_worker", 1)),
               n_workers=int(ev.get("n_workers", config["n_workers"])), deterministic=bool(ev.get("deterministic", True)),
               seed=int(ev.get("seed", 100000)), worker_steps=ev.get("worker_steps"))
    if out["interval"] < 0 or out["episodes_per_worker"] < 1 or out["n_workers"] < 1:
        raise ValueError("evaluation: interval >= 0, episodes_per_worker >= 1 and n_workers >= 1 are required")
    if out["interval"] > 0 and world > 1:
        raise ValueError("evaluation.interval in a data-parallel run: periodic evaluation runs on one rank's device only; "
                         "evaluate the checkpoint with evaluate.py instead")
    return out


def check_normalization_config(config, world: int = 1, observation_shape=None, observation_dtype=None):
    out = {"observations": normalization_section(config, "normalize_observations"), "rewards": normalization_section(config, "normalize_rewards")}
    on = [k for k, key in (("normalize_observations", "observations"), ("normalize_rewards", "rewards")) if out[key] is not None]
    if on and world > 1:
        raise ValueError(f"{' / '.join(on)} in a data-parallel run: every rank would keep statistics of its own workers only (merging "
                         "them over the ranks is not built); remove the key(s), or train on one device")
    if out["observations"] is not None and observation_shape is not None:
        if len(tuple(observation_shape)) != 1 or observation_dtype == torch.uint8:
            raise ValueError(f"normalize_observations with image / uint8 observations of shape {tuple(observation_shape)}: they are already "
                             "in [0, 1] (byte k = k / 255); remove the key -- it is for float32 vector observations")
        if not ops.obs_stats_supported(int(observation_shape[0])):
            raise ValueError(f"normalize_observations with {int(observation_shape[0])} features: the statistics kernel takes 1 to 1024; "
                             "remove the key or reduce the observation")
    return out


def check_target_kl_config(config, world: int = 1):
    out = target_kl_section(config)
    if out is not None and world > 1:
        raise ValueError("target_kl in a data-parallel run: every rank would stop on the KL of its own minibatch and the replicas would "
                         "part (agreeing on one KL over the ranks is not built); remove the key, or train on one device")
    return out


def check_adaptive_lr_config(config, world: int = 1):
    out = adaptive_lr_section(config)
    if out is None:
        return None
    if world > 1:
        raise ValueError("adaptive_lr in a data-parallel run: every rank would move its learning rate on the KL of its own minibatch and "
                         "the replicas would part (agreeing on one KL over the ranks is not built); remove the key, or train on one device")
    sched = config["learning_rate_schedule"]
    if sched["final"] != sched["initial"]:
        raise ValueError(f"adaptive_lr with a decaying learning_rate_schedule (initial {sched['initial']!r}, final {sched['final']!r}): the "
                         "two schedules compete for one learning rate; set learning_rate_schedule.final to initial (it is the start value "
                         "only), or remove the key adaptive_lr")
    start = float(np.float32(sched["initial"]))
    if not out["min"] <= start <= out["max"]:
        raise ValueError(f"adaptive_lr: the start value float32(learning_rate_schedule.initial) = {start!r} lies outside [min, max] = "
                         f"[{out['min']!r}, {out['max']!r}]; move initial into the range, or widen adaptive_lr.min / adaptive_lr.max")
    return out


def check_kl_estimator_config(config, box: bool = False, world: int = 1):
    kind = kl_estimator_section(config)
    if kind != "analytic":
        return kind
    if not box:
        raise ValueError("kl_estimator: analytic without a Box (continuous) action space: the exact KL is built for diagonal Gaussian "
                         "policies only (a categorical policy's would need every old logit stored); categorical policies keep k3: "
                         "remove the key")
    if world > 1:
        raise ValueError("kl_estimator: analytic in a data-parallel run: every rank would see the KL of its own minibatch (agreeing on one "
                         "KL over the ranks is not built); remove the key, or train on one device")
    return kind


def time_major(table, src):
    x = torch.as_tensor(np.asarray(src), dtype=table.dtype)
    return x.reshape((table.shape[1], table.shape[0]) + tuple(table.shape[2:])).transpose(0, 1)


class PPOTrainer(_DataParallelStep, _NativeRolloutDrive, _RunOutputs, _CheckpointResume):
    def __init__(self, config: dict, run_id: str = "run", device: torch.device = None, env=None, dp=None,
                 first_worker_id: int = 0, tensorboard: bool = True, resume: str = None) -> None:
        if device is None:
            device = torch.device("cuda") if torch.cuda.is_available() else torch.device("cpu")
        device = torch.device(device)
        if device.type != "cuda":
            raise RuntimeError("PPOTrainer needs an MI355X (HIP) device: this build has no CPU training path "
                               "(the CPU restatement under oracle/ is test infrastructure only)")
        self._etm = etm_lib.load()
        etm_lib.check(self._etm.etm_rollout_trxl_set_placement(0), "etm_rollout_trxl_set_placement")
        self.config = config
        self.device = device
        self._dev_index = device.index if device.index is not None else torch.cuda.current_device()
        self.run_id = run_id
        self.dp = dp
        self.num_workers = config["n_workers"]
        self.lr_schedule = config["learning_rate_schedule"]
        self.beta_schedule = config["beta_schedule"]
        self.cr_schedule = config["clip_range_schedule"]
        t = config["transformer"]
        self.memory_length, self.num_blocks, self.embed_dim = t["memory_length"], t["num_blocks"], t["embed_dim"]
        check_kernel_shapes(t)
        check_box_policy(config)
        check_byte_observation_transport(config, env)
        check_truncation_transport(config, env)
        check_action_mask_config(config, env)
        check_evaluation_config(config, 1 if dp is None else int(getattr(dp, "world", 1)))
        check_normalization_config(config, 1 if dp is None else int(getattr(dp, "world", 1)))
        check_checkpoint_config(config, 1 if dp is None else int(getattr(dp, "world", 1)), resume=resume is not None)
        kl_cfg = check_target_kl_config(config, 1 if dp is None else int(getattr(dp, "world", 1)))
        adapt_cfg = check_adaptive_lr_config(config, 1 if dp is None else int(getattr(dp, "world", 1)))
        check_kl_estimator_config(config, env is not None or check_box_policy(config) is not None, 1 if dp is None else int(getattr(dp, "world", 1)))
        self.update_index, self.segment, self._episode_infos = 0, 0, deque(maxlen=100)
        self._base_worker_id, self._env_supplied = int(first_worker_id), env is not None
        resumed = None
        if resume is not None:
            resumed = self._read_verified(resume)
            self.segment = int(resumed["segment"]) + 1
            first_worker_id = segment_first_worker_id(first_worker_id, self.segment)
        self.writer = _make_writer(run_id) if tensorboard else _NullWriter()

        min_group = int(config.get("rollout_min_group_size", 8))
        n_groups = config.get("rollout_groups", "auto")
        n_groups = default_rollout_groups(self.num_workers, min_group) if n_groups == "auto" else int(n_groups)
        if n_groups < 1 or self.num_workers % n_groups != 0 or self.num_workers // n_groups < min_group:
            n_groups = 1
        if config.get("rollout_groups", "auto") == "auto" and os.environ.get("ETM_QUIET") != "1":
            print(f"[etm] rollout worker groups: {n_groups} (rollout_groups: auto)", file=sys.stderr, flush=True)
        from etm import hostcpu
        env_cfg = dict(config["environment"])
        row_threads = ("gen_threads" if int(env_cfg.get("pool", 64)) == 0 else "copy_threads") if env_cfg.get("type") == "Synthetic" else None
        self._host_plan = hostcpu.plan_host_threads(copy_threads=int(env_cfg.get(row_threads, 1)) if row_threads else 1,
                                                    worker_processes=bool(env is None and config.get("worker_processes", False)),
                                                    num_envs=self.num_workers, envs_per_process=int(config.get("envs_per_process", 1)),
                                                    groups=n_groups, quiet=not config.get("host_cpu_plan", True))
        if not config.get("host_cpu_plan", True):
            self._host_plan.update(copy_threads=int(env_cfg.get(row_threads, 1)) if row_threads else 1, copier_spin=True, polite_wait=False,
                                   envs_per_process=int(config.get("envs_per_process", 1)), worker_spin=True, reason="host_cpu_plan: false")
        if row_threads and row_threads in env_cfg:
            env_cfg[row_threads] = self._host_plan["copy_threads"]
        if not self._host_plan["copier_spin"]:
            from environments import synthetic as _syn
            _syn.set_copier_spin(False)
        if self._host_plan["polite_wait"]:
            hostcpu.set_timer_slack_ns(1000)
        self._flag_wait_ema = 0.0
        ops.set_ln_grad_kernel(config.get("fused_ln_grad", True))
        self._shm_env = None
        if env is None and config.get("worker_processes", False):
            from environments.shm_env import ShmVecEnv
            self._shm_env = ShmVecEnv(env_cfg, self.num_workers, first_worker_id, groups=n_groups,
                                      envs_per_proc=self._host_plan["envs_per_process"], steps_per_rollout=config["worker_steps"],
                                      spin=self._host_plan["worker_spin"])
            env = self._shm_env
        self.env = env if env is not None else make_vec_env(env_cfg, self.num_workers, first_worker_id, groups=n_groups)
        self._env_cfg, self._env_groups = env_cfg, n_groups
        self._evaluator = None
        self._draw_generator = None
        W = self.num_workers
        obs_shape = tuple(self.env.observation_space_shape)
        self.observation_space = type("Space", (), {"shape": obs_shape})()
        from environments import observation_dtype as _observation_dtype
        self.observation_dtype = torch.uint8 if _observation_dtype(self.env) == np.uint8 else torch.float32
        if self.observation_dtype == torch.uint8:
            if len(obs_shape) < 2:
                raise ValueError("uint8 observations are images (byte k = k / 255); a vector observation must be float32")
        check_normalization_config(config, 1 if dp is None else int(getattr(dp, "world", 1)), obs_shape, self.observation_dtype)
        self.action_space_shape = tuple(int(a) for a in getattr(self.env, "action_space_shape", None) or (self.env.num_actions,))
        kind = getattr(self.env, "action_kind", None)
        if kind is None and hasattr(self.env, "action_space"):
            kind = action_space_kind(self.env.action_space)
        self.box = kind if kind is not None and kind.is_box else None
        if self.box is not None:
            check_box_policy(config, self.box.shape[0])
        self.max_episode_length = self.env.max_episode_steps
        self._masked = check_action_mask_config(config, self.env, self.action_space_shape, self.box is not None)
        self.last_valid_action_share = None
        self._kl_analytic = check_kl_estimator_config(config, self.box is not None, 1 if dp is None else int(getattr(dp, "world", 1))) == "analytic"

        if config.get("tunable_gemm", os.environ.get("ETM_TUNABLE_GEMM", "1") != "0"):
            try:
                import torch.cuda.tunable as tunable
                tunable.enable(True)
                tunable.tuning_enable(True)
                rank_tag = "" if dp is None else f"_rank{dp.rank}"
                tunable.set_filename(os.path.join(os.environ.get("TMPDIR", "/tmp"), f"etm_tunableop_results{rank_tag}.csv"), True)
                tunable.set_max_tuning_duration(int(os.environ.get("ETM_TUNABLE_MS", 30)))
                tunable.set_max_tuning_iterations(int(os.environ.get("ETM_TUNABLE_ITERS", 20)))
            except Exception as exc:
                print(f"[trainer] per-shape GEMM tuning not available ({exc})")
        box = self.box is not None
        self._action_width = self.action_space_shape[0] if box else len(self.action_space_shape)
        self.buffer = Buffer(config, self.observation_space, self.action_space_shape, self.max_episode_length, device, continuous=box,
                             observation_dtype=self.observation_dtype)
        self.model = ActorCriticModel(config, self.observation_space, self.action_space_shape, self.max_episode_length,
                                      continuous=box).to(device)
        self.model.train()
        self.model.graph_refresh = bool(config.get("hip_graph_rollout", True))
        if self.dp is not None:
            self.dp.broadcast_parameters(self.model)
        self.params = [p for _, p in self.model.arena_parameters()]
        if self._kl_analytic:
            self.buffer.log_std_source = self.model.policy_log_std
        self._use_train_graph = bool(config.get("hip_graph_train", True))
        self._train_graph = None
        self._train_warm = 0
        self._obs_train = None
        if self._use_train_graph:
            self._dyn = torch.zeros(2, dtype=torch.float64, device=device)
            self._sched_host = [None, None, None]
            self.profile_sample_every = 0
            self._mb_counter = 0
        self.optimizer = FlatAdamW(self.params, lr=self.lr_schedule["initial"])
        self.flat_grads = self.optimizer.flat_grads[: self.optimizer.total]
        self._grad_views = self.optimizer.grad_views
        if self.dp is not None:
            self.dp.flat = self.flat_grads
        self._build_grad_groups()
        self._kl_cfg, self._kl_gate, self.last_kl_stop = kl_cfg, None, None
        if kl_cfg is not None:
            self._kl_gate = KlGate(kl_cfg["limit"], device, host_word=kl_cfg["host_check"] == "epoch")
            self._kl_event = torch.cuda.Event() if kl_cfg["host_check"] == "epoch" else None
        self._adapt, self.last_adaptive_lr = None, None
        if adapt_cfg is not None:
            self._adapt = AdaptiveLr(adapt_cfg, device)
            self.optimizer.attach_adaptive(self._adapt)

        if self._shm_env is not None:
            seg = np.frombuffer(self._shm_env.shm.buf, dtype=np.uint8)
            etm_lib.check(etm_lib.load().etm_host_register(seg.ctypes.data, seg.nbytes), "etm_host_register")
            self._shm_registered = seg.ctypes.data
            self._obs_pin = torch.from_numpy(self._shm_env.v["obs"])
            self._act_pin = torch.from_numpy(self._shm_env.v["act"])
        else:
            self._obs_pin = torch.zeros((W,) + obs_shape, dtype=self.observation_dtype).pin_memory()
            self._act_pin = torch.zeros((W, self._action_width), dtype=torch.float32 if box else torch.int64).pin_memory()
        self.obs = self._obs_pin.numpy()
        self._ss_pin = torch.zeros((2, W), dtype=torch.int64).pin_memory()
        self._step_pin, self._slot_pin = self._ss_pin[0], self._ss_pin[1]
        self.worker_current_episode_step = self._step_pin.numpy()
        self.worker_episode_slot = self._slot_pin.numpy()
        self.worker_episode_slot[:] = np.arange(W)
        self._ss_dev = torch.zeros((2, W), dtype=torch.int64, device=device)
        self._ss_dev[1] = torch.arange(W, dtype=torch.int64, device=device)
        self._step_dev, self._slot_dev = self._ss_dev[0], self._ss_dev[1]
        self._mask_in_place = True
        self._am_pin = self._am_dev = self._am_np = None
        if self._masked:
            self._am_pin = torch.zeros(W, dtype=torch.int64).pin_memory()
            self._am_np = self._am_pin.numpy()
            self._branch_bits = branch_bit_masks(self.action_space_shape)
            self._am_dev = torch.zeros(W, dtype=torch.int64, device=device)
        if resumed is not None and self._env_supplied and hasattr(self.env, "restart"):
            self.env.restart(first_worker_id)
        self.env.reset(out=self.obs)
        if self._masked:
            self._take_action_masks(self.env, 0, W, "reset")

        S, L, B = config["worker_steps"], self.memory_length, self._action_width
        self._obs_dev = torch.zeros((W,) + obs_shape, dtype=self.observation_dtype, device=device)
        self._stage = {
            "obs": torch.zeros((S, W) + obs_shape, dtype=self.observation_dtype, device=device),
            "memory_mask": torch.zeros((S, W, L), dtype=torch.bool, device=device),
            "memory_indices": torch.zeros((S, W, L), dtype=torch.int64, device=device),
            "actions": torch.zeros((S, W, B), dtype=torch.float32 if box else torch.int64, device=device),
            "log_probs": torch.zeros((S, W, 1 if box else B), dtype=torch.float32, device=device),
            "values": torch.zeros((S, W), dtype=torch.float32, device=device),
        }
        if self._kl_analytic:
            self._stage["means"] = torch.zeros((S, W, B), dtype=torch.float32, device=device)
        self._mask_t = torch.zeros((W, L), dtype=torch.bool, device=device)
        self._win_t = torch.zeros((W, L), dtype=torch.int64, device=device)
        self._act_dev = torch.zeros((W, B), dtype=torch.float32 if box else torch.int64, device=device)
        self._uniforms = torch.zeros((S, W) if B == 1 else (S, W, B), dtype=torch.float32, device=device)
        self._forced_tab = torch.full((S, W) if B == 1 else (S, W, B), -1, dtype=torch.int64, device=device)
        if box:
            self._normals = torch.zeros((S, W, B), dtype=torch.float32, device=device)
            self._forced_tab = torch.full((S, W, B), float("nan"), dtype=torch.float32, device=device)
        self._up_stream = torch.cuda.Stream(device=device)
        self._step_graph = None
        self._chain_log = None
        self._plan = None
        self._stage_host = None
        self._stage_read = torch.cuda.Event()
        self._use_kv_cache = bool(config.get("kv_cache_rollout", True))
        T, nb, D = self.max_episode_length, self.num_blocks, self.embed_dim
        self._kv_cache = torch.zeros((W, T, nb, 2 * D), dtype=torch.float32, device=device)
        self._kv_init = torch.zeros((T, nb, 2 * D), dtype=torch.float32, device=device)
        self._kv_weights = self._kv_w_blocked = None
        self._kv_refresh_replay = ops.ReplayAfterWarmup(self._refresh_kv_cache_now, device, what="_refresh_kv_cache")
        self._lv = lv = ops.ReplayAfterWarmup(self._last_value_now, device, what="get_last_value")
        lv.rows, lv.obs = torch.empty((W, L), dtype=torch.int64, device=device), torch.empty_like(self._obs_dev)
        lv.out = torch.empty(W, dtype=torch.float32, device=device)
        self._bootstrap = bool(config.get("bootstrap_truncated", False))
        self._truncations = []
        self.last_truncations = []
        if self._bootstrap:
            self._bs = bs = ops.ReplayAfterWarmup(self._bootstrap_chunk_now, device, what="bootstrap pass")
            bs.obs, bs.rows, bs.pidx = torch.empty_like(self._obs_dev), torch.empty_like(lv.rows), torch.empty_like(lv.rows)
            bs.slot, bs.s = torch.zeros(W, dtype=torch.int64, device=device), torch.zeros(W, dtype=torch.int64, device=device)
            bs.out = torch.empty(W, dtype=torch.float32, device=device)

        self._group_all = WorkerGroup(self, 0, W, self.env, True, self._etm.etm_upload)
        parts = getattr(self.env, "parts", None)
        self._groups = [self._group_all]
        if parts is not None and len(parts) > 1:
            self._groups = [WorkerGroup(self, lo, hi, part, False, self._etm.etm_upload) for part, (lo, hi) in zip(parts, self.env.bounds)]

        mask, indices = build_window_tables(self.memory_length, self.max_episode_length)
        self.memory_mask, self.memory_indices = mask, indices
        self._mask_table = mask.bool().contiguous().to(device)
        self._index_table = indices.contiguous().to(device)
        self.last_update_timing = {}
        if resumed is not None:
            self._load_state(resumed, str(resume), restart=False)

    def _take_action_masks(self, env, lo, hi, step):
        words = self._am_np[lo:hi]
        env.action_masks(out=words)
        empty = empty_mask_branches(words, self.action_space_shape, self._branch_bits)
        if empty.any():
            wl, b = (int(x) for x in np.argwhere(empty)[0])
            raise ValueError(f"action_masks: worker {lo + wl}, step {step}, branch {b} has no valid action (word {int(words[wl]):#x}, branches "
                             f"{self.action_space_shape}): an environment must leave at least one action of every branch allowed")

    @property
    def memory(self):
        return self.buffer.bank.index_select(0, self._slot_dev)

    @property
    def obs_norm(self):
        m = self.model
        if m.obs_norm is None:
            return None
        return dict(m.obs_norm, stats=m.obs_norm_stats, mean=m.obs_norm_mean, rstd=m.obs_norm_rstd)

    @property
    def return_norm(self):
        b = self.buffer
        if b.return_norm is None:
            return None
        return dict(b.return_norm, stats=b.ret_stats, carry=b.ret_carry, scale=b.return_scale, scaled=b.rewards_scaled)

    def _training_observations(self):
        nhwc = self._observations_channels_last()
        if nhwc is None and self.model.obs_norm is not None:
            return self.buffer.samples_flat["obs"]
        return nhwc

    def _update_obs_norm(self):
        m = self.model
        with torch.no_grad():
            ops.obs_stats_update(self.buffer.samples_flat["obs"], m.obs_norm_stats, m.obs_norm_mean, m.obs_norm_rstd, m.obs_norm["epsilon"])

    def run_training(self) -> None:
        print("Step 6: Starting training using " + str(self.device))
        episode_infos = self._episode_infos
        ckpt_every = check_checkpoint_config(self.config, 1 if self.dp is None else int(getattr(self.dp, "world", 1)))
        ev_cfg = check_evaluation_config(self.config, 1 if self.dp is None else int(getattr(self.dp, "world", 1)))
        ev_every = ev_cfg["interval"] if ev_cfg is not None else 0
        for update in range(self.update_index, self.config["updates"]):
            lr, beta, clip = self.schedules(update)
            t0 = time.perf_counter()
            sampled_episode_info = self._sample_training_data()
            self.buffer.prepare_batch_dict()
            training_stats, grad_info = self._train_epochs(lr, clip, beta)
            torch.cuda.synchronize(self.device)
            dt = time.perf_counter() - t0
            training_stats = np.mean(training_stats, axis=0)
            episode_infos.extend(sampled_episode_info)
            episode_result = process_episode_info(episode_infos)
            steps_per_s = self.num_workers * self.config["worker_steps"] / dt
            vmean, amean = torch.mean(self.buffer.values).item(), torch.mean(self.buffer.advantages).item()
            if episode_result:
                head = "{:4} reward={:.2f} std={:.2f} length={:.1f} std={:.2f}".format(
                    update, episode_result["reward_mean"], episode_result["reward_std"], episode_result["length_mean"],
                    episode_result["length_std"])
            else:
                head = "{:4} (no finished episode yet)".format(update)
            if "success_percent" in episode_result:
                head += " success={:.2f}".format(episode_result["success_percent"])
            if self._is_main:
                print(head + " pi_loss={:3f} v_loss={:3f} entropy={:.3f} loss={:3f} value={:.3f} advantage={:.3f} steps/s={:.0f}".format(
                    training_stats[0], training_stats[1], training_stats[3], training_stats[2], vmean, amean, steps_per_s))
            self._write_gradient_summary(update, grad_info)
            self._write_training_summary(update, training_stats, episode_result, vmean, amean, steps_per_s)
            if ev_every and ((update + 1) % ev_every == 0 or update + 1 == self.config["updates"]):
                self._write_evaluation_summary(update, self.evaluate(ev_cfg["episodes_per_worker"], ev_cfg["n_workers"], ev_cfg["deterministic"]))
            self.update_index = update + 1
            if ckpt_every and ((update + 1) % ckpt_every == 0 or update + 1 == self.config["updates"]):
                self.save_checkpoint()
        if self._is_main and not ckpt_every:
            self._save_model()
        if self.dp is not None:
            self.dp.barrier()

    @property
    def _is_main(self):
        return self.dp is None or self.dp.rank == 0

    def schedules(self, update: int):
        s = lambda c: polynomial_decay(c["initial"], c["final"], c["max_decay_steps"], c["power"], update)
        return s(self.lr_schedule), s(self.beta_schedule), s(self.cr_schedule)

    _stream_obs = property(lambda self: self._plan is not None and self._plan.stream_obs)
    _host_flag = property(lambda self: self._plan is not None and self._plan.host_flag)
    _native_rollout = property(lambda self: self._plan is not None and self._plan.native)
    _direct_rows = property(lambda self: self._plan is not None and self._plan.direct_rows)

    def _sample_training_data(self, forced_actions=None, uniforms=None, normals=None, deterministic=False) -> list:
        if deterministic and (uniforms is not None or normals is not None):
            raise ValueError("deterministic=True fills the draw tables itself: do not pass uniforms= / normals= with it")
        main = torch.cuda.current_stream(self.device)
        plan, groups = self._begin_rollout(main, forced_actions, uniforms, normals, deterministic)
        launch = self._launch_graph_exec if plan.direct_launch else self._launch_replay if plan.graph else self._launch_eager
        for g in groups:
            launch(g, plan)
        episode_infos = []
        if plan.native:
            try:
                timing = self._drive_rollout_native(groups, episode_infos)
            finally:
                self._shm_env.park()
        else:
            timing = self._drive_rollout_host(plan, groups, launch, episode_infos)
        for g in groups:
            if g.stream is not None:
                main.wait_stream(g.stream)
        self._check_step_kernels(groups)
        self._finish_rollout(plan, main, forced_actions is not None, timing)
        return episode_infos

    def _begin_rollout(self, main, forced_actions, uniforms, normals, deterministic=False):
        self.buffer.begin_rollout(self._slot_dev)
        self._truncations = []
        self.worker_episode_slot[:] = np.arange(self.num_workers)
        self._slot_dev.copy_(self._slot_pin, non_blocking=True)
        if self._use_kv_cache:
            self._refresh_kv_cache()
        self.model.refresh_rollout_weights()
        if forced_actions is not None:
            self._forced_tab.copy_(time_major(self._forced_tab, forced_actions).to(self.device))
        if self._masked:
            self.buffer.action_masks_host[:, 0] = self._am_np
        if self.config.get("hip_graph_rollout", True):
            groups = self._groups
            if groups[0].graphs is None:
                self._capture_step_graph(groups)
            plan = self._plan
        else:
            groups, plan = [self._group_all], RolloutPlan(polite_wait=bool(self._host_plan["polite_wait"]))
        if deterministic:
            if self.box is None:
                self._uniforms.fill_(-1.0)
            else:
                self._normals.zero_()
        elif self.box is None and uniforms is not None:
            self._uniforms.copy_(time_major(self._uniforms, uniforms))
        elif self.box is None:
            self._uniforms.uniform_(generator=self._draw_generator)
        elif normals is not None:
            self._normals.copy_(time_major(self._normals, normals))
        else:
            self._normals.normal_(generator=self._draw_generator)
        for g in groups:
            g.restart()
            if g.stream is not None:
                g.stream.wait_stream(main)
        if plan.stream_obs:
            self._up_stream.wait_stream(main)
        if plan.direct_rows:
            self._stage_read.synchronize()
        if plan.native:
            self._shm_env.activate(hold=True)
            self._shm_env.restart_sequence()
        if plan.stream_obs:
            for g in groups:
                g.upload_rows(0, 0, g.W)
        return plan, groups

    def _launch_graph_exec(self, g, plan):
# ... 114 lines not shown
    def _finish_rollout(self, plan, main, forced, timing):
        buf = self.buffer
        forced_wsb = None
        if forced and self._masked:
            W, S = self.num_workers, self.config["worker_steps"]
            forced_wsb = self._forced_tab.reshape(S, W, -1).transpose(0, 1).cpu().numpy()
        if forced:
            self._forced_tab.fill_(float("nan") if self.box is not None else -1)
        if self._masked:
            self.last_valid_action_share = valid_action_share(buf.action_masks_host, sum(self.action_space_shape))
        self._step_dev.copy_(self._step_pin, non_blocking=True)
        self._slot_dev.copy_(self._slot_pin, non_blocking=True)
        for name, stage in self._stage.items():
            getattr(buf, name).copy_(stage.transpose(0, 1))
        if plan.direct_rows:
            self._stage_read.record(main)
        if forced_wsb is not None:
            self._check_forced_against_masks(forced_wsb)
        if self._bootstrap:
            self._bootstrap_pass()
        buf.calc_advantages(self.get_last_value(), self.config["gamma"], self.config["lamda"])
        self.last_update_timing.update(env_s=timing[0], wait_s=timing[1], launch_s=timing[2])

    def _check_forced_against_masks(self, forced):
        words = self.buffer.action_masks_host.view(np.uint64)
        off = 0
        for b, a in enumerate(self.action_space_shape):
            fb = forced[:, :, b]
            bit = np.where(fb >= 0, fb, 0).astype(np.uint64) + np.uint64(off)
            bad = (fb >= 0) & (((words >> bit) & np.uint64(1)) == 0)
            if bad.any():
                w, t = (int(x) for x in np.argwhere(bad)[0])
                raise ValueError(f"forced_actions: worker {w}, step {t}, branch {b}: the forced action {int(fb[w, t])} is masked out "
                                 f"(word {int(words[w, t]):#x})")
            off += int(a)

    def _rollout_step_device(self, g, stream_obs=False, host_flag=False):
        carry = self._rollout_step_head(g, stream_obs, host_flag)
        self._rollout_step_tail(g, carry, stream_obs)

    def _choose_step_form(self, g, streamed):
        m, lib = self.model, self._etm
        rf = getattr(m, "_rf", None) if self._use_kv_cache else None
        n_conc = len(self._groups) if not g.full else 1
        rfg = getattr(m, "_rfg", None) if rf is not None else None
        g.group_kernel = bool(rfg is not None and self.config.get("rollout_group_kernel", True)
                              and ops.rollout_trxl_group_ok(rfg, g.W, self.memory_length, m.hidden_size, m._rollout_actions(),
                                                            gaussian=self.box is not None)
                              and n_conc * lib.etm_rollout_trxl_group_grid() <= 256)
        fused_step = (rf is not None and m.rollout_heads_fusable()
                      and (g.group_kernel or n_conc * lib.etm_rollout_trxl_grid(g.W, rf["H"]) <= 256))
        g.tail_in_kernel = bool(fused_step and self.config.get("fused_rollout_tail", True) and self._kv_w_blocked is not None)
        if not fused_step:
            return False, None, None
        rf = rfg if g.group_kernel else rf
        if g.rf_scratch is None or g.rf_scratch_kind != g.group_kernel:
            t_ = m.transformer
            g.rf_scratch = ops.rollout_trxl_scratch(g.W, t_.embed_dim, t_.num_heads, t_.num_blocks, self.device, group=g.group_kernel)
            g.rf_scratch_kind = g.group_kernel
        hidden = "full"
        if streamed and "hid_t" in rf:
            conv3 = self.config.get("fused_conv3_hidden", True) and ops.rollout_conv3_hidden_supported(m.conv3, *m.conv2_output_hw(), rf["hid_t"].shape[1])
            hidden = "conv3" if conv3 else "partial"
        return True, rf, hidden

    def _hidden_input(self, g, hidden, rf, obs, obs_index, rows):
        m = self.model
        if hidden == "full":
            return m._encode(obs, obs_index, rows), None
        if hidden == "conv3":
            x, partial_sums = m._encode_fused(obs, obs_index, rows, features_only="conv2"), ops.rollout_conv3_hidden
            args = (m._w3k, m.conv3.bias, rf["hid_t"])
        else:
            x, partial_sums = m._encode_fused(obs, obs_index, rows, features_only=True), ops.rollout_hidden_partial
            args = (rf["hid_t"],)
        if g.h_part is None:
            g.h_part = partial_sums(x, *args)
        return partial_sums(x, *args, out=g.h_part), m.lin_hidden.bias

    def _rollout_step_head(self, g, stream_obs=False, host_flag=False):
        buf, st, m = self.buffer, self._stage, self.model
        rows = None if g.full else (g.lo, g.hi)
        if stream_obs:
            obs, obs_index = st["obs"], g.t_dev
        else:
            g.obs_dev.copy_(g.obs_pin, non_blocking=True)
            obs, obs_index, rows = g.obs_dev, None, None
            g.ss_dev.copy_(g.ss_pin, non_blocking=True)
            if g.am_pin is not None and not self._mask_in_place:
                g.am_dev.copy_(g.am_pin, non_blocking=True)
        branches = self.action_space_shape
        policy_head = m.rollout_policy_head()
        box = None if self.box is None else (m.policy_log_std, self.box.low, self.box.high)
        draws = self._uniforms if box is None else self._normals
        means = {"st_means": st["means"]} if self._kl_analytic else {}
        mask_t, win_t = g.mask_t, g.win_t
        ss_src = g.ss_pin if stream_obs and g.stream is not None else g.ss_dev
        am_src = None if g.am_pin is None else (g.am_pin if self._mask_in_place or (stream_obs and g.stream is not None) else g.am_dev)
        fused_step, rf, hidden = self._choose_step_form(g, obs_index is not None)
        flag_pin = g.flag_pin if host_flag else None
        if fused_step:
            h_in, h_bias = self._hidden_input(g, hidden, rf, obs, obs_index, rows)
            tail = (self._kv_w_blocked, m.transformer._pos(), g.step_l, g.slot_l, buf.bank) if g.tail_in_kernel else None
            ops.rollout_trxl(h_in, rf, g.kv, win_t, mask_t, g.item, policy_head, m.value,
                             draws, self._forced_tab, g.t_dev, g.act_dev, st["actions"], st["log_probs"], st["values"],
                             g.rf_scratch, host_actions=g.act_pin, host_flag=flag_pin, w_off=g.lo,
                             tail=tail, h_bias=h_bias, branches=branches, box=box,
                             window=(ss_src, self._mask_table, self._index_table, st["memory_mask"], st["memory_indices"],
                                     g.ss_latch, g.t_row, self._kv_init), action_mask=am_src, **means)
            return g.item
        ops.rollout_window(ss_src[0], self._mask_table, self._index_table, g.t_dev, mask_t, win_t,
                           st["memory_mask"], st["memory_indices"], t_row=g.t_row,
                           reset=(g.kv, self._kv_init) if self._use_kv_cache else None, w_off=g.lo,
                           latch=(ss_src, g.ss_latch))
        kv_spec = WindowSpec.from_bank(g.kv, None, win_t, None, mask_t) if self._use_kv_cache else None
        if kv_spec is not None and m.rollout_heads_fusable():
            h2, item = m.forward_hidden_cached(obs, kv_spec, items_out=g.item, obs_index=obs_index, raw=True, obs_rows=rows)
            if box is not None:
                ops.rollout_policy_gaussian(h2, policy_head, m.value, box[0], draws, self._forced_tab, g.t_dev, g.act_dev,
                                            st["actions"], st["log_probs"], st["values"], low=box[1], high=box[2],
                                            host_actions=g.act_pin, host_flag=flag_pin, h_bias=m._b_heads, w_off=g.lo, **means)
            else:
                ops.rollout_policy(h2, policy_head, m.value, self._uniforms, self._forced_tab, g.t_dev,
                                   g.act_dev, st["actions"], st["log_probs"], st["values"],
                                   host_actions=g.act_pin, host_flag=flag_pin, h_bias=m._b_heads, w_off=g.lo, branches=branches,
                                   action_mask=am_src)
        else:
            if kv_spec is not None:
                logits, value, item = m.forward_logits_cached(obs, kv_spec, items_out=g.item, obs_index=obs_index, obs_rows=rows)
            else:
                spec = WindowSpec.from_bank(buf.bank, g.slot_dev, win_t, win_t, mask_t)
                logits, value, item = m.forward_logits(obs, spec)
                item = item.transpose(0, 1)
            if not g.full:
                raise RuntimeError("worker groups need the fused policy path (K/V cache)")
            lg = logits[0] if len(logits) == 1 else torch.cat(logits, dim=1)
            if box is not None:
                ops.rollout_sample_gaussian(lg, value, box[0], draws, self._forced_tab, g.t_dev, g.act_dev, st["actions"], st["log_probs"],
                                            st["values"], low=box[1], high=box[2], **means)
            else:
                ops.rollout_sample(lg, value, self._uniforms, self._forced_tab, g.t_dev, g.act_dev,
                                   st["actions"], st["log_probs"], st["values"], branches=branches, action_mask=am_src)
            g.act_pin.copy_(g.act_dev, non_blocking=True)
        if item.data_ptr() != g.item.data_ptr():
            g.item.copy_(item)
        return g.item

    def _rollout_step_tail(self, g, item, stream_obs=False):
        buf, st = self.buffer, self._stage
        if not g.tail_in_kernel:
            item = item.transpose(0, 1)
            buf.bank[g.slot_l, g.step_l] = item
            if self._use_kv_cache:
                tr = self.model.transformer
                pos = tr._pos()
                pos_rows = pos.index_select(0, g.step_l) if pos is not None else None
                g.kv[g.ids, g.step_l] = tr.project_memory(item, pos_rows, self._kv_weights)
        if not stream_obs:
            st["obs"][:, g.lo:g.hi].index_copy_(0, g.t_row.view(1), g.obs_dev.unsqueeze(0))

    def _refresh_kv_cache(self):
        r = self._kv_refresh_replay
        r.enabled = bool(self.config.get("hip_graph_rollout", True)) and self.buffer.address_captured
        r()

    def _refresh_kv_cache_now(self):
        W, T = self.num_workers, self.max_episode_length
        tr = self.model.transformer
        with torch.no_grad():
            fresh = tr.kv_projection_weights()
            if self._kv_weights is None:
                self._kv_weights = tuple(t.clone() if torch.is_tensor(t) else t for t in fresh)
            else:
                for dst, src in zip(self._kv_weights, fresh):
                    if torch.is_tensor(dst):
                        dst.copy_(src)
            team = etm_lib.load().etm_rollout_trxl_team(tr.num_heads)
            w = self._kv_weights[0]
            if w.shape[2] % (2 * team) == 0:
                nb_, d_, d2_ = w.shape
                wb = w.reshape(nb_, d_, 2, team, d2_ // (2 * team)).permute(0, 3, 1, 2, 4).reshape(nb_, team, d_, d2_ // team)
                if self._kv_w_blocked is None:
                    self._kv_w_blocked = wb.contiguous()
                else:
                    self._kv_w_blocked.copy_(wb)
            pos = tr._pos()
            live = self.buffer.bank[:W].reshape(W * T, self.num_blocks, self.embed_dim)
            pos_all = pos.repeat(W, 1) if pos is not None else None
            self._kv_cache.copy_(tr.project_memory(live, pos_all, self._kv_weights).reshape(self._kv_cache.shape))
            zeros = torch.zeros((T, self.num_blocks, self.embed_dim), dtype=torch.float32, device=self.device)
            self._kv_init.copy_(tr.project_memory(zeros, pos, self._kv_weights))

    def _capture_step_graph(self, groups):
        cfg = self.config
        with torch.no_grad():
            plan = self._plan = plan_rollout(
                graph=True, stream_observations=bool(cfg.get("stream_observations", True)),
                host_flag_actions=bool(cfg.get("host_flag_actions", True)), direct_observation_rows=bool(cfg.get("direct_observation_rows", True)),
                kv_cache=self._use_kv_cache, fused_encoder=self.model._fused_encoder_ok(self._obs_dev),
                heads_fusable=self.model.rollout_heads_fusable(), several_groups=all(g.stream is not None for g in groups),
                worker_processes=self._shm_env is not None, raw_graph_exec=hasattr(torch.cuda.CUDAGraph, "raw_cuda_graph_exec"),
                large_bar=lambda: ops.host_direct_write_ok(self.device), polite_wait=bool(self._host_plan["polite_wait"]))
        so, hf = plan.stream_obs, plan.host_flag
        self._stage_host = ops.host_view(self._stage["obs"]) if plan.direct_rows else None
        for gi, g in enumerate(groups):
            g.obs_stream = g.stream.cuda_stream if plan.own_stream else self._up_stream.cuda_stream
            if plan.native:
                g.use_flag(self._shm_env.v["go"][gi, 0:1])
        with torch.no_grad():
            ss = torch.from_numpy(self._ss_pin.numpy().copy()).to(self.device)
            all_ids = torch.arange(self.num_workers, device=self.device)
            saved_bank = self.buffer.bank[ss[1], ss[0]].clone()
            saved_kv = self._kv_cache[all_ids, ss[0]].clone()
        for g in groups:
            g.t_dev.zero_()
            side = g.stream if g.stream is not None else torch.cuda.Stream(device=self.device)
            side.wait_stream(torch.cuda.current_stream(self.device))
            with torch.cuda.stream(side), torch.no_grad():
                for i in range(3):
                    self._rollout_step_device(g, so, hf)
                    side.synchronize()
            torch.cuda.current_stream(self.device).wait_stream(side)
            torch.cuda.synchronize(self.device)
            pool = torch.cuda.graph_pool_handle()
            head, tail = torch.cuda.CUDAGraph(), torch.cuda.CUDAGraph()
            with torch.no_grad(), torch.cuda.graph(head, pool=pool, stream=g.stream, capture_error_mode="thread_local"):
                item = self._rollout_step_head(g, so, hf)
                if hf:
                    self._rollout_step_tail(g, item, so)
            if hf or (g.tail_in_kernel and so):
                tail = None
            else:
                with torch.no_grad(), torch.cuda.graph(tail, pool=pool, stream=g.stream, capture_error_mode="thread_local"):
                    self._rollout_step_tail(g, g.item, so)
            g.graphs = (head, tail)
            g.graph_exec = head.raw_cuda_graph_exec() if plan.direct_launch else None
            g.t_dev.zero_()
        with torch.no_grad():
            torch.cuda.synchronize(self.device)
            self.buffer.bank[ss[1], ss[0]] = saved_bank
            self._kv_cache[all_ids, ss[0]] = saved_kv
        self.buffer.address_captured = True
        ops.freeze_workspaces(self.device)
        self._step_graph = groups[0].graphs

    def get_last_value(self):
        L, lv = self.memory_length, self._lv
        step = torch.from_numpy(self.worker_current_episode_step.copy())
        start = torch.clamp(step - L, min=0)
        lv.rows.copy_(start.unsqueeze(1) + torch.arange(L, dtype=torch.int64).unsqueeze(0), non_blocking=False)
        lv.obs.copy_(self._obs_pin, non_blocking=True)
        lv.enabled = bool(self.config.get("hip_graph_rollout", True)) and self.buffer.address_captured
        lv()
        return lv.out

    def _last_value_now(self):
        lv, L = self._lv, self.memory_length
        with torch.no_grad():
            mask = self._mask_table[torch.clamp(self._step_dev, 0, L - 1)]
            spec = WindowSpec.from_bank(self.buffer.bank, self._slot_dev, lv.rows, self.buffer.memory_indices[:, -1], mask)
            _, last_value, _ = self.model.forward_logits(lv.obs, spec, want_items=False)
            lv.out.copy_(last_value)

    def _bootstrap_pass(self):
        recs, self._truncations = self._truncations, []
        self.last_truncations = [r[:4] for r in recs]
        if not recs:
            return
        W, bs = self.num_workers, self._bs
        n, w, t, operands = self._bootstrap_operands(recs, W)
        bs.enabled = bool(self.config.get("hip_graph_rollout", True)) and self.buffer.address_captured
        with torch.no_grad():
            values = torch.empty(w.numel(), dtype=torch.float32, device=self.device)
            for lo in range(0, w.numel(), W):
                for dst, src in zip((bs.obs, bs.slot, bs.rows, bs.pidx, bs.s), operands):
                    dst.copy_(src[lo: lo + W])
                bs()
                values[lo: lo + W] = bs.out
            self.buffer.bootstrap_values[w[:n], t[:n]] = values[:n]

    def _bootstrap_operands(self, recs, chunk):
        L, dev, n = self.memory_length, self.device, len(recs)
        idx = list(range(n)) + [n - (n % chunk)] * (-n % chunk)
        meta = torch.tensor([recs[i][:4] for i in idx], dtype=torch.int64).to(dev)
        obs = torch.from_numpy(np.stack([np.asarray(recs[i][4]) for i in idx])).to(dev)
        if obs.dtype != self.observation_dtype:
            obs = obs.to(self.observation_dtype)
        w, t, slot, s = meta.unbind(1)
        rows = torch.clamp(s - L, min=0).unsqueeze(1) + torch.arange(L, dtype=torch.int64, device=dev).unsqueeze(0)
        return n, w, t, (obs, slot, rows, self.buffer.memory_indices[w, t], s)

    def _bootstrap_forward(self, obs, slot, rows, pidx, s):
        mask = self._mask_table[torch.clamp(s, 0, self.memory_length - 1)]
        spec = WindowSpec.from_bank(self.buffer.bank, slot, rows, pidx, mask)
        return self.model.forward_logits(obs, spec, want_items=False)[1]

    def _bootstrap_chunk_now(self):
        bs = self._bs
        with torch.no_grad():
            bs.out.copy_(self._bootstrap_forward(bs.obs, bs.slot, bs.rows, bs.pidx, bs.s))

    def _train_epochs(self, learning_rate: float, clip_range: float, beta: float, perms=None):
        stats, norms = [], []
        monitor = self.config.get("monitor_gradients", True)
        with torch.no_grad():
            self._bank_pos = self._bank_with_positions()
            self._obs_train = self._training_observations()
        mbs = self.buffer.batch_size // self.buffer.n_mini_batches
        sort_mb = bool(self.config.get("sort_minibatch", True))
        n_mb = self.buffer.n_mini_batches
        tables = bool(self._use_train_graph and self.config.get("step_ends_fused", True) and mbs * n_mb == self.buffer.batch_size
                      and (perms is None or all(len(p) == self.buffer.batch_size for p in perms)))
        row = 0
        if tables:
            self._step_tables(mbs)
            self._tg_counter.zero_()
        gate, launched = self._kl_gate, 0
        if gate is not None:
            gate.reset()
        if self._adapt is not None:
            self._adapt.reset()
        host_stop = False
        for epoch in range(self.config["epochs"]):
            if gate is not None and gate.host_word is not None and epoch > 0 and not host_stop:
                self._kl_event.record(torch.cuda.current_stream(self.device))
                self._kl_event.synchronize()
                host_stop = int(gate.host_word[0]) != 0
            if perms is None:
                perm = torch.randperm(self.buffer.batch_size, device=self.device)
            else:
                perm = torch.as_tensor(perms[epoch], device=self.device, dtype=torch.long)
            if host_stop:
                continue
            if sort_mb and perm.numel() % mbs == 0:
                perm = perm.view(-1, mbs).sort(dim=1).values.reshape(-1)
            self._epoch_stats3 = None
            if tables:
                self._tg_idx_table.copy_(perm.view(n_mb, mbs))
            if self.dp is not None and self.dp.active and perm.numel() % mbs == 0:
                adv = self.buffer.samples_flat["advantages"].index_select(0, perm).view(-1, mbs)
                local = torch.stack([ops.adv_stats(adv[i]) for i in range(adv.shape[0])])
                self._epoch_stats3 = self.dp.merge_adv_stats(local)
            for start in range(0, self.buffer.batch_size, mbs):
                idx = perm[start: start + mbs]
                launched += 1
                self._mb_stats3 = self._epoch_stats3[start // mbs] if self._epoch_stats3 is not None else None
                if tables:
                    self._train_step_graph(idx, learning_rate, clip_range, beta, monitor, row=row)
                    row += 1
                    continue
                if self._use_train_graph and idx.numel() == mbs:
                    st_row, norm_row = self._train_step_graph(idx, learning_rate, clip_range, beta, monitor)
                    stats.append(st_row)
                    if monitor:
                        norms.append(norm_row)
                    continue
                mini_batch = self.buffer.gather(idx)
                stats.append(self._train_mini_batch(mini_batch, learning_rate, clip_range, beta))
                if monitor:
                    norms.append(self._grad_group_norms())
        if self.model.obs_norm is not None:
            self._update_obs_norm()
        rows = launched
        if gate is not None:
            stopped, applied, kl = gate.read()
            rows = target_kl_rows(stopped, applied, launched)
            self.last_kl_stop = {"stopped": stopped, "steps_applied": applied, "steps_launched": launched, "kl": kl, "limit": gate.limit}
        if self._adapt is not None:
            (raised, lowered), ad = self._adapt.read(), self._adapt
            self.last_adaptive_lr = {"lr": float(self.optimizer.lr_dev.item()), "raised": raised, "lowered": lowered,
                                     "kl_low": ad.kl_low, "kl_high": ad.kl_high}
        train_info = (self._tg_stats_tab[:rows] if tables else torch.stack(stats[:rows])).cpu().numpy()
        self._bank_pos = self._row_stats = None
        self._mb_stats3 = self._epoch_stats3 = None
        grad_info = {}
        if norms or (tables and monitor):
            allnorms = (self._tg_norm_tab[:rows] if tables else torch.stack(norms[:rows])).cpu().numpy()
            grad_info = {k: allnorms[:, i].tolist() for i, k in enumerate(self._grad_keys)}
        return [row for row in train_info], grad_info

    def _train_mini_batch(self, samples: dict, learning_rate: float, clip_range: float, beta: float):
        ep = samples.get("memory_index")
        bank_pos = getattr(self, "_bank_pos", None)
        if bank_pos is not None and ep is not None and samples["memories"].data_ptr() == self.buffer.bank.data_ptr():
            spec = WindowSpec.from_bank(bank_pos, ep, samples["memory_indices"], None, samples["memory_mask"])
            spec.pos_included = True
            spec.row_stats = getattr(self, "_row_stats", None)
        else:
            spec = WindowSpec.from_bank(samples["memories"], ep, samples["memory_indices"], samples["memory_indices"],
                                        samples["memory_mask"])
            if ep is not None and self.model.transformer.pos_kind == "" and samples["memories"].data_ptr() == self.buffer.bank.data_ptr():
                spec.row_stats = getattr(self, "_row_stats", None)
        stats3 = getattr(self, "_mb_stats3", None)
        if stats3 is None:
            stats3 = ops.adv_stats(samples["advantages"])
            if self.dp is not None:
                stats3 = self.dp.merge_adv_stats(stats3)
        loss, stats = self._loss_from(samples["obs"], spec, samples, clip_range, beta, stats3, dyn=None)
        self._set_lr(learning_rate)
        self._backward_into_arena(loss)
        if self.dp is not None:
            self.dp.all_reduce_grads(average=False)
        self.optimizer.step(self.config["max_grad_norm"], grad_scale=self._grad_scale(), **self._step_gate(stats))
        return stats

    def _loss_from(self, obs, spec, mb, clip_range, beta, stats3, dyn="device"):
        dyn = getattr(self, "_dyn", None) if dyn == "device" else dyn
        m = self.model
        if self.box is not None:
            h, _ = m.forward_state(obs, spec)
            if not ops.heads_loss_supported_gaussian(h, m.lin_policy, m.policy_branches[0]):
                raise RuntimeError("Box policy: the minibatch is outside the fused Gaussian heads + loss kernel")
            old = dict(old_mean=mb["means"], old_log_std=self.buffer.old_log_std) if self._kl_analytic else {}
            return ops.heads_ppo_loss_gaussian(h, m.lin_policy, m.lin_value, m.policy_branches[0], m.policy_log_std, m.value, mb["actions"],
                                               mb["log_probs"], mb["advantages"], mb["values"], clip_range, self.config["value_loss_coefficient"],
                                               beta, stats3, dyn=dyn, unit_grad=True, **old)
        if self.config.get("fused_heads_loss", True):
            h, _ = m.forward_state(obs, spec)
            branch = m.policy_branches[0] if len(m.policy_branches) == 1 else list(m.policy_branches)
            if ops.heads_loss_supported(h, m.lin_policy, branch):
                return ops.heads_ppo_loss(h, m.lin_policy, m.lin_value, branch, m.value, mb["actions"], mb["log_probs"],
                                          mb["advantages"], mb["values"], clip_range, self.config["value_loss_coefficient"], beta, stats3, dyn=dyn,
                                          unit_grad=True, action_mask=mb.get("action_masks"))
            h_policy = ops.linear_relu(m.lin_policy, h)
            h_value = ops.linear_relu(m.lin_value, h)
            logits, value = [br(h_policy) for br in m.policy_branches], m.value(h_value).reshape(-1)
        else:
            logits, value, _ = m.forward_logits(obs, spec, want_items=False)
        return ops.ppo_loss(logits, value, mb["actions"], mb["log_probs"], mb["advantages"], mb["values"], clip_range,
                            self.config["value_loss_coefficient"], beta, stats3, dyn=dyn, action_mask=mb.get("action_masks"))

    def _dw_destinations(self):
        if getattr(self, "_dw_dest", None) is None:
            dw, cs = self.config.get("grouped_dw_train", True), self.config.get("grouped_colsum_train", True)
            self._dw_dest = {p.data_ptr(): v for p, v in zip(self.params, self._grad_views)
                             if (p.dim() == 2 and dw) or (p.dim() == 1 and cs) or (p.dim() == 4 and cs)}
        return self._dw_dest

    def _unit_gradient(self, loss):
        one = getattr(self, "_one", None)
        if one is None or one.device != loss.device or one.shape != loss.shape:
            one = self._one = torch.ones_like(loss)
        return one

    def _grad_scale(self):
        return self.dp.grad_scale if self.dp is not None else 1.0

    def _set_lr(self, learning_rate: float):
        if self._adapt is not None:
            return
        self.optimizer.set_lr(learning_rate)

    def _bank_with_positions(self):
        tr = self.model.transformer
        self._row_stats = None
        if tr.pos_kind not in ("relative", ""):
            return None
        mem = self.buffer.memories
        if tr.pos_kind == "relative":
            if getattr(self, "_bank_pos_buf", None) is None or self._bank_pos_buf.shape != self.buffer.bank.shape:
                self._bank_pos_buf = torch.empty_like(self.buffer.bank)
            out = self._bank_pos_buf[: mem.shape[0]]
            torch.add(mem, tr._pos_table[None, : mem.shape[1], None, :], out=out)
        self._row_stats = self._bank_row_stats(self._bank_pos_buf if tr.pos_kind == "relative" else self.buffer.bank, mem.shape[0])
        return self._bank_pos_buf if tr.pos_kind == "relative" else None

    def _bank_row_stats(self, bank, used):
        blk = self.model.transformer.transformer_blocks[0]
        if blk.layer_norm != "pre" or not self.buffer.block_major or not self.config.get("bank_row_stats", True):
            return None
        E, T, nb, D = bank.shape
        if D % 128 != 0 or D > 1024:
            return None
        if getattr(self, "_row_stats_buf", None) is None or self._row_stats_buf.shape != (nb, E, T, 2):
            self._row_stats_buf = torch.zeros((nb, E, T, 2), dtype=torch.float32, device=self.device)
        lib = etm_lib.load()
        st = torch.cuda.current_stream(self.device).cuda_stream
        for b in range(nb):
            rows = bank[:used, :, b, :]
            etm_lib.check(lib.etm_ln_row_stats(rows.data_ptr(), float(blk.norm_kv.eps), self._row_stats_buf[b].data_ptr(), used * T, D, st),
                          "etm_ln_row_stats")
        return self._row_stats_buf

    def _observations_channels_last(self):
        obs = self.buffer.samples_flat["obs"]
        if obs.dim() != 4 or not getattr(self.model, "channels_last", False):
            return None
        n, c, h, w = obs.shape
        if getattr(self, "_obs_nhwc_buf", None) is None or self._obs_nhwc_buf.shape != (n, h, w, c):
            self._obs_nhwc_buf = torch.empty((n, h, w, c), dtype=obs.dtype, device=self.device)
        self._obs_nhwc_buf.copy_(obs.permute(0, 2, 3, 1))
        return self._obs_nhwc_buf

    def _step_tables(self, mbs):
        if getattr(self, "_tg_idx", None) is None or self._tg_idx.numel() != mbs:
            self._tg_idx = torch.empty(mbs, dtype=torch.long, device=self.device)
            self._tg_stats3 = torch.zeros(3, dtype=torch.float32, device=self.device) if self.dp is not None else None
            self._tg_idx_table, self._train_graph = None, None
        if getattr(self, "_tg_idx_table", None) is None:
            n_mb, steps = self.buffer.n_mini_batches, self.config["epochs"] * self.buffer.n_mini_batches
            self._tg_counter = torch.zeros(1, dtype=torch.long, device=self.device)
            self._tg_idx_table = torch.zeros((n_mb, mbs), dtype=torch.long, device=self.device)
            self._tg_stats_tab = torch.zeros((steps, 6), dtype=torch.float32, device=self.device)
            self._tg_norm_tab = torch.zeros((steps, len(self._grad_keys)), dtype=torch.float32, device=self.device)

    def _gather_minibatch(self, keys, idx, stats3, head):
        buf = self.buffer
        fields = [buf.samples_flat[k] for k in keys]
        if not head:
            return dict(zip(keys, ops.gather_rows(fields, idx))), stats3
        adv = buf.samples_flat["advantages"]
        own = stats3 is None and etm_lib.load().etm_adv_stats_workspace_bytes(idx.numel()) == 0
        outs, st3 = ops.step_head(fields, self._tg_idx_table, self._tg_counter, idx_out=idx, adv_src=adv if own else None)
        return dict(zip(keys, outs)), (st3 if own else stats3)

    def _train_body_a(self, idx, clip_range, beta, stats3=None, head=False):
        buf = self.buffer
        skip = ("obs",) if self._obs_train is not None else ()
        keys = [k for k in buf.samples_flat if k not in skip]
        mb, stats3 = self._gather_minibatch(keys, idx, stats3, head)
        if self._bank_pos is not None:
            spec = WindowSpec.from_bank(self._bank_pos_buf, mb["memory_index"], mb["memory_indices"], None, mb["memory_mask"])
            spec.pos_included = True
            spec.row_stats = getattr(self, "_row_stats", None)
        else:
            spec = WindowSpec.from_bank(buf.bank, mb["memory_index"], mb["memory_indices"], mb["memory_indices"], mb["memory_mask"])
            if self.model.transformer.pos_kind == "":
                spec.row_stats = getattr(self, "_row_stats", None)
        obs = mb.get("obs")
        if self._obs_train is not None:
            obs = IndexedObservations(self._obs_train, idx)
        if stats3 is None:
            stats3 = ops.adv_stats(mb["advantages"])
        loss, stats = self._loss_from(obs, spec, mb, clip_range, beta, stats3)
        self._backward_into_arena(loss)
        return stats

    def _backward_into_arena(self, loss):
        for p in self.params:
            p.grad = None
        with ops.DeferredDw(self._dw_destinations(), tail=bool(self.config.get("step_ends_fused", True))) as dw:
            loss.backward(self._unit_gradient(loss))
        dw.pack(self.params, self._grad_views, [p.grad for p in self.params])
        for p, v in zip(self.params, self._grad_views):
            p.grad = v

    def minibatch_gradients(self, idx, clip_range: float, beta: float) -> dict:
        idx = torch.as_tensor(np.asarray(idx.cpu() if torch.is_tensor(idx) else idx), device=self.device, dtype=torch.long)
        if self.config.get("sort_minibatch", True):
            idx = idx.sort().values
        with torch.no_grad():
            self._bank_pos = self._bank_with_positions()
            self._obs_train = self._training_observations()
        if self._use_train_graph:
            self._dyn.copy_(torch.tensor([clip_range, beta], dtype=torch.float64))
            self._sched_host[1:] = [clip_range, beta]
        stats3 = None
        if self.dp is not None:
            stats3 = self.dp.merge_adv_stats(ops.adv_stats(self.buffer.samples_flat["advantages"].index_select(0, idx)))
        self._train_body_a(idx, clip_range, beta, stats3)
        grads = {n: p.grad.detach().clone() for n, p in self.model.named_parameters() if p.requires_grad}
        self._bank_pos = self._row_stats = None
        return grads

    def _step_gate(self, stats):
        gate, adapt = self._kl_gate, self._adapt
        if gate is not None or adapt is not None:
            if stats is None or stats.dtype != torch.float32 or stats.dim() != 1 or stats.numel() < 5 or not stats.is_contiguous():
                raise RuntimeError("target_kl / adaptive_lr: the step's statistics must be a contiguous float32 vector with the kl at index 4")
            kl = stats[4:5]
            if gate is not None:
                gate.kl = kl
            if adapt is not None:
                adapt.kl = kl
        return {"gate": gate, "adapt": adapt}

    def _train_body_b(self, monitor, stats=None, kl_stats=None):
        self.optimizer.step(self.config["max_grad_norm"], grad_scale=self._grad_scale(),
                            **(self._step_gate(kl_stats) if self._kl_gate is not None or self._adapt is not None else {}))
        if stats is None:
            return self._grad_group_norms() if monitor else None
        if stats.numel() != self._tg_stats_tab.shape[1] or stats.dtype != torch.float32 or not stats.is_contiguous():
            raise RuntimeError("the step's statistics do not fit the rows of the statistics table")
        if monitor:
            return self._grad_group_norms(step=(stats, self._tg_stats_tab, self._tg_norm_tab, self._tg_counter))
        etm_lib.check(etm_lib.load().etm_step_end(stats.data_ptr(), stats.numel(), self._tg_stats_tab.data_ptr(), self._tg_stats_tab.shape[0],
                                                  self._tg_counter.data_ptr(), torch.cuda.current_stream(self.device).cuda_stream), "etm_step_end")
        return None

    def _train_step_graph(self, idx, learning_rate, clip_range, beta, monitor, row=None):
        dp = self.dp
        tables = bool(self.config.get("step_ends_fused", True))
        if getattr(self, "_tg_idx", None) is None:
            if tables:
                self._step_tables(idx.numel())
            else:
                self._tg_idx = torch.empty_like(idx)
                self._tg_stats3 = torch.zeros(3, dtype=torch.float32, device=self.device) if dp is not None else None
                self._tg_idx_table = None
        tables = self._tg_tables = tables and self._tg_idx_table is not None
        if not tables:
            self._tg_idx.copy_(idx)
        elif row is None:
            self._tg_counter.zero_()
            if self._kl_gate is not None:
                self._kl_gate.reset()
# ... 112 lines not shown
```

include/etm_hip.h:

```cpp
#ifndef ETM_HIP_H
#define ETM_HIP_H

#include <stdint.h>

#ifdef __cplusplus
extern "C" {
#endif

#define ETM_OK 0
#define ETM_EINVAL (-1)
#define ETM_EUNSUPPORTED (-2)
#define ETM_EWORKSPACE (-3)
#define ETM_ENOCOMM (-4)
#define ETM_ETIMEOUT (-5)
#define ETM_EABORTED (-6)
#define ETM_ERCCL_BASE 100000

int etm_abi_version(void);

const char *etm_error_string(int code);

int etm_mha_fwd(const float *bank, int64_t ep_stride, int64_t row_stride,
                const int64_t *ep, const int64_t *win, const int64_t *pidx, const uint8_t *mask,
                const float *pos, const float *ln_g, const float *ln_b, float ln_eps,
// ... 83 lines not shown
int etm_colsum_reduce_max_problems(void);
int etm_colsum_reduce_grouped(const float *const *partial, const int *P, const int *C, const int *ld, float *const *out, int n, void *stream);
int etm_gate_train_rz(const float *A, const float *B, const float *bg, const float *x, float *r, float *z, float *rx, int N, int D,
                      void *stream);
int etm_gate_train_out(const float *A, const float *C, const float *z, const float *x, float *hh, float *out, int N, int D, void *stream);
int64_t etm_gate_train_bwd_workspace_bytes(int N, int D);
int etm_gate_train_bwd_partial_rows(int N);
int etm_gate_train_bwd1(const float *dout, const float *dout2, const float *z, const float *hh, const float *x, float *dA, float *dB, float *dx1, float *dbg,
                        float *workspace, int64_t workspace_bytes, int N, int D, void *stream);
int etm_gate_train_bwd2(const float *drx, const float *x, const float *r, const float *dx1, float *dA, float *dB, float *dx2, int N, int D,
                        void *stream);

int etm_heads_loss_supported(int N, int hid, int A);
int etm_heads_loss_row_floats(int hid, int A);
int64_t etm_heads_loss_workspace_bytes(int N, int hid, int A);
int etm_heads_loss(const float *pre_p, const float *pre_v, const float *b_lp, const float *b_lv, const float *wb, const float *bb,
                   const float *wv, const float *bv, const int64_t *actions, int64_t action_stride, const float *old_logp,
                   int64_t logp_stride, const float *adv, const float *old_value, const float *adv_stats3, double clip, float vf_coef,
                   float beta, float pol_scale, float ent_scale, float val_scale, const double *dyn_clip_beta, float *gm_p, float *gm_v,
                   float *sums, float *out8, float *logits, float *value, void *workspace, int64_t workspace_bytes, int N, int hid,
                   int A, void *stream);
int etm_heads_loss_supported_branched(int N, int hid, const int32_t *branch_sizes, int n_branches);
int etm_heads_loss_branched(const float *pre_p, const float *pre_v, const float *b_lp, const float *b_lv, const float *wb, const float *bb,
                            const float *wv, const float *bv, const int64_t *actions, int64_t action_stride, const float *old_logp,
                            int64_t logp_stride, const float *adv, const float *old_value, const float *adv_stats3, double clip, float vf_coef,
                            float beta, float pol_scale, float ent_scale, float val_scale, const double *dyn_clip_beta, float *gm_p,
                            float *gm_v, float *sums, float *out8, float *logits, float *value, void *workspace, int64_t workspace_bytes,
                            int N, int hid, const int32_t *branch_sizes, int n_branches, void *stream);
int etm_heads_loss_masked(const float *pre_p, const float *pre_v, const float *b_lp, const float *b_lv, const float *wb, const float *bb,
                          const float *wv, const float *bv, const int64_t *actions, int64_t action_stride, const float *old_logp,
                          int64_t logp_stride, const float *adv, const float *old_value, const float *adv_stats3, double clip, float vf_coef,
                          float beta, float pol_scale, float ent_scale, float val_scale, const double *dyn_clip_beta, float *gm_p,
                          float *gm_v, float *sums, float *out8, float *logits, float *value, void *workspace, int64_t workspace_bytes,
                          int N, int hid, int A, const int64_t *action_mask, void *stream);
int etm_heads_loss_branched_masked(const float *pre_p, const float *pre_v, const float *b_lp, const float *b_lv, const float *wb,
                                   const float *bb, const float *wv, const float *bv, const int64_t *actions, int64_t action_stride,
                                   const float *old_logp, int64_t logp_stride, const float *adv, const float *old_value,
                                   const float *adv_stats3, double clip, float vf_coef, float beta, float pol_scale, float ent_scale,
                                   float val_scale, const double *dyn_clip_beta, float *gm_p, float *gm_v, float *sums, float *out8,
                                   float *logits, float *value, void *workspace, int64_t workspace_bytes, int N, int hid,
                                   const int32_t *branch_sizes, int n_branches, const int64_t *action_mask, void *stream);
int etm_heads_loss_supported_gaussian(int N, int hid, int A);
int etm_heads_loss_gaussian_row_floats(int hid, int A);
int64_t etm_heads_loss_gaussian_workspace_bytes(int N, int hid, int A);
int etm_heads_loss_gaussian(const float *pre_p, const float *pre_v, const float *b_lp, const float *b_lv, const float *wb, const float *bb,
                            const float *wv, const float *bv, const float *xact, int64_t action_stride, const float *log_std,
                            const float *old_logp, int64_t logp_stride, const float *adv, const float *old_value, const float *adv_stats3,
                            double clip, float vf_coef, float beta, float pol_scale, float ent_scale, float val_scale,
                            const double *dyn_clip_beta, float *gm_p, float *gm_v, float *sums, float *out8, float *logits, float *value,
                            void *workspace, int64_t workspace_bytes, int N, int hid, int A, void *stream);
int etm_heads_loss_gaussian_kl_row_floats(int hid, int A);
int64_t etm_heads_loss_gaussian_kl_workspace_bytes(int N, int hid, int A);
int etm_heads_loss_gaussian_kl(const float *pre_p, const float *pre_v, const float *b_lp, const float *b_lv, const float *wb,
                               const float *bb, const float *wv, const float *bv, const float *xact, int64_t action_stride,
                               const float *log_std, const float *old_logp, int64_t logp_stride, const float *adv, const float *old_value,
                               const float *adv_stats3, double clip, float vf_coef, float beta, float pol_scale, float ent_scale,
                               float val_scale, const double *dyn_clip_beta, float *gm_p, float *gm_v, float *sums, float *out8,
                               float *logits, float *value, void *workspace, int64_t workspace_bytes, int N, int hid, int A,
                               const float *old_mean, int64_t old_mean_stride, const float *old_log_std, void *stream);

int etm_grouped_dw_supported(int N, int Ma, int Nb, int lda, int ldb, int ldc);
int etm_grouped_dw_max_problems(void);
int etm_grouped_dw(const float *const *A, const float *const *B, float *const *C, const int32_t *dims, int n_problems, int N,
                   void *stream);

int etm_grouped_dw_tile_map(int n_tiles, int32_t *out);

int etm_grouped_dw_tail_max_problems(void);
int etm_grouped_dw_tail(const float *const *A, const float *const *B, float *const *C, const int32_t *dims, int n_problems, int N,
                        const float *const *cs_partial, const int *cs_P, const int *cs_C, const int *cs_ld, float *const *cs_out, int n_cs,
                        void *stream);

int etm_grad_sqnorm(const float *g, int64_t n, float *partial, int n_partial, int64_t *step, void *stream);
int etm_adamw_clip(float *p, float *g, float *m, float *v, int64_t n, const float *partial, int n_partial, const float *lr_dev,
                   const int64_t *step, double beta1, double beta2, double eps, double weight_decay, float max_norm, float grad_scale, float *norm_out,
                   void *stream);

int etm_grad_sqnorm_gated(const float *g, int64_t n, float *partial, int n_partial, int64_t *step, const float *kl, float kl_limit,
                          uint64_t *gate, uint64_t *host_word, void *stream);
int etm_adamw_clip_gated(float *p, float *g, float *m, float *v, int64_t n, const float *partial, int n_partial, const float *lr_dev,
                         const int64_t *step, double beta1, double beta2, double eps, double weight_decay, float max_norm, float grad_scale,
                         float *norm_out, const uint64_t *gate, void *stream);

int etm_grad_sqnorm_adaptive(const float *g, int64_t n, float *partial, int n_partial, int64_t *step, const float *kl, float *lr_dev,
                             float kl_low, float kl_high, float factor, float lr_min, float lr_max,
                             uint64_t *lr_state,
                             float kl_limit, uint64_t *gate, uint64_t *host_word,
                             void *stream);

int etm_arena_digest(const float *x, int64_t n, uint64_t *partial, int n_partial, uint64_t *out4, void *stream);

int etm_rollout_heads(const float *h, const float *wp, const float *bp, const float *wv, const float *bv, float *logits, float *value,
                      int W, int A, int hid, void *stream);
int etm_rollout_policy(const float *h, const float *h_bias, const float *wp, const float *bp, const float *wv, const float *bv,
                       const float *uniforms, const int64_t *forced, int64_t *t_dev, int64_t *actions, int64_t *st_actions,
                       float *st_logp, float *st_values, int64_t *host_actions, int64_t *host_flag, int32_t *sync_counter,
                       int W, int A, int hid, int stage_W, void *stream);
int etm_rollout_policy_branched(const float *h, const float *h_bias, const float *wp, const float *bp, const float *wv, const float *bv,
                                const float *uniforms, const int64_t *forced, int64_t *t_dev, int64_t *actions, int64_t *st_actions,
                                float *st_logp, float *st_values, int64_t *host_actions, int64_t *host_flag, int32_t *sync_counter,
                                int W, int hid, int stage_W, const int32_t *branch_sizes, int n_branches, void *stream);
int etm_rollout_policy_branched_masked(const float *h, const float *h_bias, const float *wp, const float *bp, const float *wv,
                                       const float *bv, const float *uniforms, const int64_t *forced, int64_t *t_dev, int64_t *actions,
                                       int64_t *st_actions, float *st_logp, float *st_values, int64_t *host_actions, int64_t *host_flag,
                                       int32_t *sync_counter, int W, int hid, int stage_W, const int32_t *branch_sizes, int n_branches,
                                       const int64_t *action_mask, void *stream);
int etm_rollout_policy_gaussian(const float *h, const float *h_bias, const float *wp, const float *bp, const float *wv, const float *bv,
                                const float *log_std, const float *normals, const float *forced, int64_t *t_dev, float *actions,
                                float *st_actions, float *st_logp, float *st_values, float *host_actions, int64_t *host_flag,
                                int32_t *sync_counter, const float *low, const float *high, int W, int A, int hid, int stage_W, void *stream);
int etm_rollout_policy_gaussian_means(const float *h, const float *h_bias, const float *wp, const float *bp, const float *wv, const float *bv,
                                      const float *log_std, const float *normals, const float *forced, int64_t *t_dev, float *actions,
                                      float *st_actions, float *st_logp, float *st_values, float *host_actions, int64_t *host_flag,
                                      int32_t *sync_counter, const float *low, const float *high, int W, int A, int hid, int stage_W,
                                      float *st_means, void *stream);

int etm_rollout_trxl_team(int H);
int etm_rollout_trxl_set_placement(int mode);
int etm_rollout_trxl_grid(int W, int H);
int etm_rollout_trxl_supported(int D, int H, int L, int hid, int A, int nb);
int etm_rollout_trxl_gate_merged(int D, int H);
int64_t etm_rollout_trxl_scratch_bytes(int W, int D, int H, int nb);
int etm_rollout_trxl(const float *h_in, const float *wemb_t, const float *bemb, const void *const *blocks, int nb, float *kv,
                     int64_t kv_worker_stride, int64_t kv_row_stride, const int64_t *win, const uint8_t *mask, float *items,
                     const float *wh_t, const float *bh, const float *wp, const float *bp, const float *wv, const float *bv,
                     const float *uniforms, const int64_t *forced, int64_t *t_dev, int64_t *actions, int64_t *st_actions,
                     float *st_logp, float *st_values, int64_t *host_actions, int64_t *host_flag, int32_t *sync_counter, float ln_eps,
                     void *scratch, int64_t scratch_bytes, const float *wkv, const float *pos, const int64_t *step_l,
                     const int64_t *slot_l, float *bank, int64_t bank_slot_stride, int64_t bank_row_stride, int64_t bank_block_stride,
                     const float *h_bias, int h_splits, const int64_t *ss, const uint8_t *mask_table, const int64_t *index_table, uint8_t *st_mask,
                     int64_t *st_idx, int64_t *latch, int64_t *t_row, uint8_t *mask_t, int64_t *win_t, const float *kv_init, int T,
                     int pre_ln, int gtrxl, int W, int D, int H, int L, int hid, int A, int stage_W, void *stream);
int etm_rollout_trxl_group_supported(int D, int H, int L, int hid, int A, int nb, int W, int gtrxl);
int etm_rollout_trxl_group_grid(void);
int64_t etm_rollout_trxl_group_scratch_bytes(int nb);
int etm_rollout_trxl_group(const float *h_in, const float *wemb_t, const float *bemb, const void *const *blocks, int nb, float *kv,
                     int64_t kv_worker_stride, int64_t kv_row_stride, const int64_t *win, const uint8_t *mask, float *items,
                     const float *wh_t, const float *bh, const float *wp, const float *bp, const float *wv, const float *bv,
                     const float *uniforms, const int64_t *forced, int64_t *t_dev, int64_t *actions, int64_t *st_actions,
                     float *st_logp, float *st_values, int64_t *host_actions, int64_t *host_flag, int32_t *sync_counter, float ln_eps,
                     void *scratch, int64_t scratch_bytes, const float *wkv, const float *pos, const int64_t *step_l,
                     const int64_t *slot_l, float *bank, int64_t bank_slot_stride, int64_t bank_row_stride, int64_t bank_block_stride,
                     const float *h_bias, int h_splits, const int64_t *ss, const uint8_t *mask_table, const int64_t *index_table, uint8_t *st_mask,
                     int64_t *st_idx, int64_t *latch, int64_t *t_row, uint8_t *mask_t, int64_t *win_t, const float *kv_init, int T,
                     int pre_ln, int gtrxl, int W, int D, int H, int L, int hid, int A, int stage_W, void *stream);
int etm_rollout_trxl_supported_branched(int D, int H, int L, int hid, const int32_t *branch_sizes, int n_branches, int nb);
int etm_rollout_trxl_group_supported_branched(int D, int H, int L, int hid, const int32_t *branch_sizes, int n_branches, int nb, int W,
                                              int gtrxl);
int etm_rollout_trxl_branched(const float *h_in, const float *wemb_t, const float *bemb, const void *const *blocks, int nb, float *kv,
                              int64_t kv_worker_stride, int64_t kv_row_stride, const int64_t *win, const uint8_t *mask, float *items,
                              const float *wh_t, const float *bh, const float *wp, const float *bp, const float *wv, const float *bv,
                              const float *uniforms, const int64_t *forced, int64_t *t_dev, int64_t *actions, int64_t *st_actions,
                              float *st_logp, float *st_values, int64_t *host_actions, int64_t *host_flag, int32_t *sync_counter, float ln_eps,
                              void *scratch, int64_t scratch_bytes, const float *wkv, const float *pos, const int64_t *step_l,
                              const int64_t *slot_l, float *bank, int64_t bank_slot_stride, int64_t bank_row_stride, int64_t bank_block_stride,
                              const float *h_bias, int h_splits, const int64_t *ss, const uint8_t *mask_table, const int64_t *index_table,
                              uint8_t *st_mask, int64_t *st_idx, int64_t *latch, int64_t *t_row, uint8_t *mask_t, int64_t *win_t,
                              const float *kv_init, int T, int pre_ln, int gtrxl, int W, int D, int H, int L, int hid, int stage_W,
                              const int32_t *branch_sizes, int n_branches, void *stream);
int etm_rollout_trxl_group_branched(const float *h_in, const float *wemb_t, const float *bemb, const void *const *blocks, int nb, float *kv,
                                    int64_t kv_worker_stride, int64_t kv_row_stride, const int64_t *win, const uint8_t *mask, float *items,
                                    const float *wh_t, const float *bh, const float *wp, const float *bp, const float *wv, const float *bv,
                                    const float *uniforms, const int64_t *forced, int64_t *t_dev, int64_t *actions, int64_t *st_actions,
                                    float *st_logp, float *st_values, int64_t *host_actions, int64_t *host_flag, int32_t *sync_counter,
                                    float ln_eps, void *scratch, int64_t scratch_bytes, const float *wkv, const float *pos, const int64_t *step_l,
                                    const int64_t *slot_l, float *bank, int64_t bank_slot_stride, int64_t bank_row_stride,
                                    int64_t bank_block_stride, const float *h_bias, int h_splits, const int64_t *ss, const uint8_t *mask_table,
                                    const int64_t *index_table, uint8_t *st_mask, int64_t *st_idx, int64_t *latch, int64_t *t_row,
                                    uint8_t *mask_t, int64_t *win_t, const float *kv_init, int T, int pre_ln, int gtrxl, int W, int D, int H,
                                    int L, int hid, int stage_W, const int32_t *branch_sizes, int n_branches, void *stream);
int etm_rollout_trxl_branched_masked(const float *h_in, const float *wemb_t, const float *bemb, const void *const *blocks, int nb, float *kv,
                              int64_t kv_worker_stride, int64_t kv_row_stride, const int64_t *win, const uint8_t *mask, float *items,
                              const float *wh_t, const float *bh, const float *wp, const float *bp, const float *wv, const float *bv,
                              const float *uniforms, const int64_t *forced, int64_t *t_dev, int64_t *actions, int64_t *st_actions,
                              float *st_logp, float *st_values, int64_t *host_actions, int64_t *host_flag, int32_t *sync_counter, float ln_eps,
                              void *scratch, int64_t scratch_bytes, const float *wkv, const float *pos, const int64_t *step_l,
                              const int64_t *slot_l, float *bank, int64_t bank_slot_stride, int64_t bank_row_stride, int64_t bank_block_stride,
                              const float *h_bias, int h_splits, const int64_t *ss, const uint8_t *mask_table, const int64_t *index_table,
                              uint8_t *st_mask, int64_t *st_idx, int64_t *latch, int64_t *t_row, uint8_t *mask_t, int64_t *win_t,
                              const float *kv_init, int T, int pre_ln, int gtrxl, int W, int D, int H, int L, int hid, int stage_W,
                              const int32_t *branch_sizes, int n_branches, const int64_t *action_mask, void *stream);
int etm_rollout_trxl_group_branched_masked(const float *h_in, const float *wemb_t, const float *bemb, const void *const *blocks, int nb, float *kv,
                                    int64_t kv_worker_stride, int64_t kv_row_stride, const int64_t *win, const uint8_t *mask, float *items,
                                    const float *wh_t, const float *bh, const float *wp, const float *bp, const float *wv, const float *bv,
                                    const float *uniforms, const int64_t *forced, int64_t *t_dev, int64_t *actions, int64_t *st_actions,
                                    float *st_logp, float *st_values, int64_t *host_actions, int64_t *host_flag, int32_t *sync_counter,
                                    float ln_eps, void *scratch, int64_t scratch_bytes, const float *wkv, const float *pos, const int64_t *step_l,
                                    const int64_t *slot_l, float *bank, int64_t bank_slot_stride, int64_t bank_row_stride,
                                    int64_t bank_block_stride, const float *h_bias, int h_splits, const int64_t *ss, const uint8_t *mask_table,
                                    const int64_t *index_table, uint8_t *st_mask, int64_t *st_idx, int64_t *latch, int64_t *t_row,
                                    uint8_t *mask_t, int64_t *win_t, const float *kv_init, int T, int pre_ln, int gtrxl, int W, int D, int H,
                                    int L, int hid, int stage_W, const int32_t *branch_sizes, int n_branches,
                                    const int64_t *action_mask, void *stream);
int etm_rollout_trxl_supported_gaussian(int D, int H, int L, int hid, int A, int nb);
int etm_rollout_trxl_group_supported_gaussian(int D, int H, int L, int hid, int A, int nb, int W, int gtrxl);
int etm_rollout_trxl_gaussian(const float *h_in, const float *wemb_t, const float *bemb, const void *const *blocks, int nb, float *kv,
                              int64_t kv_worker_stride, int64_t kv_row_stride, const int64_t *win, const uint8_t *mask, float *items,
                              const float *wh_t, const float *bh, const float *wp, const float *bp, const float *wv, const float *bv,
                              const float *log_std, const float *normals, const float *forced, int64_t *t_dev, float *actions,
                              float *st_actions, float *st_logp, float *st_values, float *host_actions, int64_t *host_flag,
                              int32_t *sync_counter, float ln_eps, void *scratch, int64_t scratch_bytes, const float *wkv, const float *pos,
                              const int64_t *step_l, const int64_t *slot_l, float *bank, int64_t bank_slot_stride, int64_t bank_row_stride,
                              int64_t bank_block_stride, const float *h_bias, int h_splits, const int64_t *ss, const uint8_t *mask_table,
                              const int64_t *index_table, uint8_t *st_mask, int64_t *st_idx, int64_t *latch, int64_t *t_row,
                              uint8_t *mask_t, int64_t *win_t, const float *kv_init, int T, int pre_ln, int gtrxl, int W, int D, int H,
                              int L, int hid, int A, int stage_W, const float *low, const float *high, void *stream);
int etm_rollout_trxl_group_gaussian(const float *h_in, const float *wemb_t, const float *bemb, const void *const *blocks, int nb,
                                    float *kv, int64_t kv_worker_stride, int64_t kv_row_stride, const int64_t *win, const uint8_t *mask,
                                    float *items, const float *wh_t, const float *bh, const float *wp, const float *bp, const float *wv,
                                    const float *bv, const float *log_std, const float *normals, const float *forced, int64_t *t_dev,
                                    float *actions, float *st_actions, float *st_logp, float *st_values, float *host_actions,
                                    int64_t *host_flag, int32_t *sync_counter, float ln_eps, void *scratch, int64_t scratch_bytes,
                                    const float *wkv, const float *pos, const int64_t *step_l, const int64_t *slot_l, float *bank,
                                    int64_t bank_slot_stride, int64_t bank_row_stride, int64_t bank_block_stride, const float *h_bias,
                                    int h_splits, const int64_t *ss, const uint8_t *mask_table, const int64_t *index_table,
                                    uint8_t *st_mask, int64_t *st_idx, int64_t *latch, int64_t *t_row, uint8_t *mask_t, int64_t *win_t,
                                    const float *kv_init, int T, int pre_ln, int gtrxl, int W, int D, int H, int L, int hid, int A,
                                    int stage_W, const float *low, const float *high, void *stream);
int etm_rollout_trxl_gaussian_means(const float *h_in, const float *wemb_t, const float *bemb, const void *const *blocks, int nb,
                                    float *kv, int64_t kv_worker_stride, int64_t kv_row_stride, const int64_t *win, const uint8_t *mask,
                                    float *items, const float *wh_t, const float *bh, const float *wp, const float *bp, const float *wv,
                                    const float *bv, const float *log_std, const float *normals, const float *forced, int64_t *t_dev,
                                    float *actions, float *st_actions, float *st_logp, float *st_values, float *host_actions,
                                    int64_t *host_flag, int32_t *sync_counter, float ln_eps, void *scratch, int64_t scratch_bytes,
                                    const float *wkv, const float *pos, const int64_t *step_l, const int64_t *slot_l, float *bank,
                                    int64_t bank_slot_stride, int64_t bank_row_stride, int64_t bank_block_stride, const float *h_bias,
                                    int h_splits, const int64_t *ss, const uint8_t *mask_table, const int64_t *index_table,
                                    uint8_t *st_mask, int64_t *st_idx, int64_t *latch, int64_t *t_row, uint8_t *mask_t, int64_t *win_t,
                                    const float *kv_init, int T, int pre_ln, int gtrxl, int W, int D, int H, int L, int hid, int A,
                                    int stage_W, const float *low, const float *high, float *st_means, void *stream);
int etm_rollout_trxl_group_gaussian_means(const float *h_in, const float *wemb_t, const float *bemb, const void *const *blocks, int nb,
                                    float *kv, int64_t kv_worker_stride, int64_t kv_row_stride, const int64_t *win, const uint8_t *mask,
                                    float *items, const float *wh_t, const float *bh, const float *wp, const float *bp, const float *wv,
                                    const float *bv, const float *log_std, const float *normals, const float *forced, int64_t *t_dev,
                                    float *actions, float *st_actions, float *st_logp, float *st_values, float *host_actions,
                                    int64_t *host_flag, int32_t *sync_counter, float ln_eps, void *scratch, int64_t scratch_bytes,
                                    const float *wkv, const float *pos, const int64_t *step_l, const int64_t *slot_l, float *bank,
                                    int64_t bank_slot_stride, int64_t bank_row_stride, int64_t bank_block_stride, const float *h_bias,
                                    int h_splits, const int64_t *ss, const uint8_t *mask_table, const int64_t *index_table,
                                    uint8_t *st_mask, int64_t *st_idx, int64_t *latch, int64_t *t_row, uint8_t *mask_t, int64_t *win_t,
                                    const float *kv_init, int T, int pre_ln, int gtrxl, int W, int D, int H, int L, int hid, int A,
                                    int stage_W, const float *low, const float *high, float *st_means, void *stream);
int etm_window_set_skip_masked(int on);

int etm_rollout_hidden_splits(int F);
int etm_rollout_hidden_partial(const float *x, const float *wt, float *part, int W, int F, int D, void *stream);
int etm_rollout_conv3_hidden_supported(int C, int Hi, int Wi, int Cout, int KH, int KW, int S, int D);
int etm_rollout_conv3_hidden(const float *x2, const float *w3k, const float *b3, const float *hid_t, float *part, int W, int Hi, int Wi,
                             int D, void *stream);

int64_t etm_relu_bwd_colsum_workspace_bytes(int N, int C);
int etm_relu_bwd_colsum_partial_rows(int N);
int etm_relu_bwd_colsum(const float *g, const float *y, float *gm, float *db, float *workspace, int64_t workspace_bytes, int N, int C,
                        void *stream);

int etm_group_norms(const float *flat, const int64_t *seg_start, const int32_t *seg_len, int n_segs, const float *member, int n_groups,
                    float *partial, float *out, void *stream);

int etm_gather_rows(const void *const *src, void *const *dst, const int64_t *row_bytes, int n_fields, const int64_t *idx, int64_t n,
                    int64_t src_rows, void *stream);

int etm_step_head(const void *const *src, void *const *dst, const int64_t *row_bytes, int n_fields, const int64_t *idx_table, int table_rows,
                  const int64_t *counter, int64_t n, int64_t src_rows, int64_t *idx_out, const float *adv_src, float *stats3, void *stream);

int etm_group_norms_step(const float *flat, const int64_t *seg_start, const int32_t *seg_len, int n_segs, const float *member, int n_groups,
                         float *partial, float *out, float *norm_table, const float *stats, int n_stats, float *stats_table, int table_rows,
                         int64_t *counter, void *stream);
int etm_step_end(const float *stats, int n_stats, float *stats_table, int table_rows, int64_t *counter, void *stream);

void *etm_host_copier_create(int threads);
void etm_host_copier_destroy(void *copier);
int etm_host_copier_set_spin(void *copier, int pauses);
int etm_host_copy(void *copier, void *dst, const void *src, int64_t bytes);

int etm_conv_relu(const float *in, const int64_t *in_index, int64_t in_index_stride, const float *w, const float *bias, float *out,
                  int N, int C, int H, int W, int Cout, int KH, int KW, int S, int in_nhwc, int out_nchw, void *stream);

int etm_conv_train_fwd(const float *x, const int64_t *x_index, int64_t x_images, const float *w_packed, const float *bias, float *y, int N,
                       int C, int H, int W, int Cout, int KH, int KW, int S, int out_nchw, void *stream);
int etm_conv_train_set_fwd_lds(int layer_mask);
int etm_conv_train_set_wgrad_lds(int layer_mask);
int etm_conv_train_set_dgrad_lds(int on);
int etm_conv_pack_weights_grouped(const float *const *w, float *const *fwd, float *const *dgrad, const int *Cout, const int *C,
                                  const int *KH, const int *KW, const int *S, int n, void *stream);
int etm_conv_train_wgrad_slices(int N, int C, int H, int W, int Cout, int KH, int KW, int S);
int etm_conv_wgrad_reduce_grouped(const float *const *partial, const int *slices, float *const *dw, float *const *db, const int *Cout,
                                  const int *C, const int *KH, const int *KW, int n, void *stream);
int etm_conv_train_dgrad(const float *dy, const float *w_packed, const float *y_below, float *dx, int N, int C, int H, int W, int Cout,
                         int KH, int KW, int S, void *stream);
int etm_conv_pack_weights(const float *w, float *fwd, float *dgrad, int Cout, int C, int KH, int KW, int S, void *stream);
int64_t etm_conv_train_wgrad_workspace_bytes(int N, int C, int H, int W, int Cout, int KH, int KW, int S);
int etm_conv_train_wgrad(const float *x, const int64_t *x_index, const float *dy, float *dw_kc_dbias, float *workspace,
                         int64_t workspace_bytes, int N, int C, int H, int W, int Cout, int KH, int KW, int S, void *stream);
int etm_relu_mask(const float *g, const float *y, float *out, int64_t n, void *stream);
int etm_conv_b3_pack(const float *const *w, uint16_t *const *out, const int *dgrad, const int *Cout, const int *C, const int *KS,
                     const int *S, int n, void *stream);
int etm_conv_b3_fwd(const float *x, const int64_t *x_index, const uint16_t *w_b3, const float *bias, float *y, uint32_t *relu_bits, int N,
                    int C, int H, int W, int Cout, int KH, int KW, int S, void *stream);
int etm_conv_b3_dgrad(const float *dy, const uint32_t *dy_relu_bits, const uint16_t *w_b3, const float *y_below, const uint32_t *relu_bits,
                      float *dx, int N, int C, int H, int W, int Cout, int KH, int KW, int S, void *stream);
int etm_conv_b3_wgrad_slices(int N, int C, int H, int W, int Cout, int KH, int KW, int S);
int etm_conv_b3_wgrad(const float *x, const int64_t *x_index, const float *dy, const uint32_t *dy_relu_bits, float *workspace,
                      int64_t workspace_bytes, int N, int C, int H, int W, int Cout, int KH, int KW, int S, void *stream);

int etm_bytes_to_unit(const uint8_t *src, const int64_t *index, float *dst, int64_t rows, int64_t row_bytes, void *stream);
int etm_conv_relu_u8(const uint8_t *in, const int64_t *in_index, int64_t in_index_stride, const float *w, const float *bias, float *out,
                     int N, int C, int H, int W, int Cout, int KH, int KW, int S, int in_nhwc, int out_nchw, void *stream);
int etm_conv_b3_fwd_u8(const uint8_t *x, const int64_t *x_index, const uint16_t *w_b3, const float *bias, float *y, uint32_t *relu_bits,
                       int N, int C, int H, int W, int Cout, int KH, int KW, int S, void *stream);
int etm_conv_b3_wgrad_u8(const uint8_t *x, const int64_t *x_index, const float *dy, const uint32_t *dy_relu_bits, float *workspace,
                         int64_t workspace_bytes, int N, int C, int H, int W, int Cout, int KH, int KW, int S, void *stream);

int etm_upload(void *dst, const void *src, int64_t bytes, void *stream);
typedef struct etm_rollout_group {
  void *graph_exec;
  void *stream;
  const volatile int64_t *ready;
  int32_t n_procs, ready_stride;
  int32_t lo, hi;
  const void *obs_src;
  void *stage_dst;
  int64_t *ss_dst;
} etm_rollout_group;
int etm_graph_launch(void *graph_exec, void *stream);
int etm_host_direct_write_init(int device);
int etm_host_store_fence(int device);
int etm_host_register(void *ptr, int64_t bytes);
int etm_host_unregister(void *ptr);
int etm_rollout_drive(const etm_rollout_group *groups, int G, int t_first, int S, int W, int64_t row_bytes, int64_t stage_step_bytes,
                      const uint8_t *dones, int64_t *ep_step, int64_t *slot, int64_t *next_slot, int64_t capacity, int64_t *events,
                      int64_t max_events, int64_t *n_events, const volatile int64_t *abort_words, int n_abort_words, int abort_stride,
                      double timeout_s, double *timing, double *chain_log);

int etm_gae(const float *rewards, const uint8_t *dones, const float *values, const float *last_value,
            float gamma, float gamma_lambda, float *advantages, int W, int S, void *stream);
int etm_gae_truncated(const float *rewards, const uint8_t *dones, const uint8_t *truncated, const float *values, const float *boot,
                      const float *last_value, float gamma, float gamma_lambda, float *advantages, int W, int S, void *stream);

int etm_obs_stats_supported(int F);
int64_t etm_obs_stats_workspace_bytes(int R, int F);
int etm_obs_stats_update(const float *x, int R, int F, double *stats, float *mean, float *rstd, double epsilon, void *workspace,
                         int64_t workspace_bytes, void *stream);
int etm_obs_normalize(const float *x, const int64_t *index, const float *mean, const float *rstd, float clip, float *out, int64_t N,
                      int F, void *stream);
int64_t etm_return_scale_workspace_bytes(int W);
int etm_return_scale(const float *rewards, const uint8_t *dones, double *ret_carry, double *stats, double gamma, double epsilon,
                     float clip, float *scaled, int W, int S, void *workspace, int64_t workspace_bytes, void *stream);

int etm_adv_stats(const float *adv, int N, float *stats3, void *stream);
#define ETM_ADV_STATS_SPLIT_MIN 65536
int64_t etm_adv_stats_workspace_bytes(int N);
int etm_adv_stats_ws(const float *adv, int N, float *stats3, void *workspace, int64_t workspace_bytes, void *stream);

int64_t etm_ppo_loss_workspace_bytes(int N);

int etm_ppo_loss(const float *logits, const int64_t *actions, int64_t action_stride,
                 const float *old_logp, int64_t logp_stride,
                 const float *adv, const float *old_value, const float *value,
                 const float *adv_stats3,
                 double clip, float vf_coef, float beta,
                 float pol_scale, float ent_scale, float val_scale, int include_value,
                 float *out8, float *d_logits, float *d_value,
                 void *partials, int64_t partials_bytes, const double *dyn_clip_beta,
                 int N, int A, void *stream);
int etm_ppo_loss_masked(const float *logits, const int64_t *actions, int64_t action_stride, const float *old_logp, int64_t logp_stride,
                        const float *adv, const float *old_value, const float *value, const float *adv_stats3, double clip, float vf_coef,
                        float beta, float pol_scale, float ent_scale, float val_scale, int include_value, float *out8, float *d_logits,
                        float *d_value, void *partials, int64_t partials_bytes, const double *dyn_clip_beta, int N, int A,
                        const int64_t *action_mask, int mask_shift, void *stream);

#define ETM_COMM_ID_BYTES 128
int etm_comm_unique_id(void *id_out);
int etm_comm_init(const void *id, int rank, int world, void **comm_out);
int etm_allreduce_f32(void *comm, const float *send, float *recv, int64_t count, void *stream);
int etm_comm_destroy(void *comm);

int etm_profile_enable(int on);
int etm_profile_set_tag(int tag);
int etm_profile_kernel_count(void);
const char *etm_profile_kernel_name(int kernel);
int etm_profile_collect(double *total_ms, int64_t *count);

#ifdef __cplusplus
}
#endif
#endif
```

Before: 114,200.

## Add scheduled variants of b3 conv kernels: hoisted weight prefetch and in-loop splitting

Adds a compile-time schedule parameter to the bf16x3 conv kernel. One variant prefetches the next group's first weight stages before the epilogue. The other performs the fp32-to-three-bf16 split of the next group's inputs inside the MFMA loop, with loads issued in the first half of k-steps, so the split overlaps matrix math instead of following the barrier. The variants are enabled by default for layer-3 forward and layer-2/3 dgrad, selectable at runtime. Timing-stamp instrumentation and a grid-cap knob are also added. The cost is more registers held across the loop, which can lower occupancy.

New measurement: 114,100. About the same (-0.1%).

```diff
diff --git a/episodic-transformer-memory-ppo_amd/csrc/conv_b3.hip b/episodic-transformer-memory-ppo_amd/csrc/conv_b3.hip
--- a/episodic-transformer-memory-ppo_amd/csrc/conv_b3.hip
+++ b/episodic-transformer-memory-ppo_amd/csrc/conv_b3.hip
@@ -18,7 +18,22 @@
   unsigned *bits_out;
   float *out;
   int N, n_groups;
+#ifdef ETM_B3_STAMPS
+  long long *stamps;
+#endif
 };
+
+#ifdef ETM_B3_STAMPS
+#define B3_STAMP_INIT(p) long long *const stamp_buf = (blockIdx.x == 0 && threadIdx.x == 0) ? (p).stamps : nullptr; int stamp_n = 0
+#define B3_STAMP() do { if (stamp_buf) stamp_buf[++stamp_n] = (long long)__builtin_amdgcn_s_memtime(); } while (0)
+#define B3_STAMP_REAL() do { if (stamp_buf) stamp_buf[++stamp_n] = (long long)__builtin_amdgcn_s_memrealtime(); } while (0)
+#define B3_STAMP_DONE() do { if (stamp_buf) stamp_buf[0] = stamp_n; } while (0)
+#else
+#define B3_STAMP_INIT(p) do { } while (0)
+#define B3_STAMP() do { } while (0)
+#define B3_STAMP_REAL() do { } while (0)
+#define B3_STAMP_DONE() do { } while (0)
+#endif
 
 __device__ __forceinline__ unsigned b3_cvt_pk(float a, float b) {
   unsigned r;
@@ -99,7 +114,7 @@
   static constexpr bool U8 = true;
 };
 
-template <class L, bool DGRAD, int C, int S>
+template <class L, bool DGRAD, int C, int S, int SCH>
 __global__ __launch_bounds__(256, L::WPC) void conv_b3_kernel(const B3Args p) {
   constexpr bool U8 = L::U8;
   static_assert(!U8 || (L::THREE && !DGRAD && L::G == 1 && (L::Q_IMG * 4) % 16 == 0 && (L::Q_UNIT * 4) % 16 == 0 && (L::Q_ROW0 * 4) % 16 == 0),
@@ -111,6 +126,61 @@
   const int tid = threadIdx.x, lane = tid & 63, col = lane & 31, half = lane >> 5;
   const int wave = __builtin_amdgcn_readfirstlane(tid >> 6);
   const int ct = wave % NT, rp = wave / NT;
+  constexpr bool HOIST_W = (SCH & 1) != 0;
+  constexpr bool SPLIT_IN_LOOP = (SCH & 2) != 0;
+  static_assert(!SPLIT_IN_LOOP || (!L::THREE && !U8 && NQ <= 16), "split in the loop: six registers per float4");
+  constexpr int KS0 = SPLIT_IN_LOOP ? KSTEPS / 2 : KSTEPS;
+  constexpr int LPKS = SPLIT_IN_LOOP ? (NQ + KS0 - 1) / KS0 : LPK;
+  constexpr int NSPL = SPLIT_IN_LOOP ? NQ : 0;
+  constexpr int FPS = (NSPL + (KSTEPS - KSTEPS / 2) * TPW - 1) / ((KSTEPS - KSTEPS / 2) * TPW);
+  B3_STAMP_INIT(p);
+  B3_STAMP_REAL();
+  B3_STAMP();
+
+  auto group_rsrc = [&](int grp) {
+    const bool exists = grp < p.n_groups;
+    const int u0 = exists ? grp * G : 0;
+    const int n0 = u0 / L::NB, b0 = u0 - n0 * L::NB;
+    const long long src = (G == 1 && p.img_index) ? p.img_index[n0] : (long long)n0;
+    const int units = exists ? min(G, p.N * L::NB - u0) : 0;
+    if constexpr (U8)
+      return __builtin_amdgcn_make_buffer_rsrc((void *)(reinterpret_cast<const unsigned char *>(p.x) + src * (L::Q_IMG * 4) + b0 * (L::Q_ROW0 * 4)), 0,
+                                               units * L::Q_UNIT * 4, 0x00020000);
+    else
+      return __builtin_amdgcn_make_buffer_rsrc((void *)(p.x + src * (L::Q_IMG * 4) + b0 * (L::Q_ROW0 * 4)), 0, units * L::Q_UNIT * 16, 0x00020000);
+  };
+  auto group_bits_rsrc = [&](int grp) {
+    const bool exists = DGRAD && p.src_bits && grp < p.n_groups;
+    const int n0 = exists ? grp * G : 0;
+    const int images = exists ? min(G, p.N - n0) : 0;
+    return __builtin_amdgcn_make_buffer_rsrc((void *)((p.src_bits ? p.src_bits : (const unsigned *)p.x) + (long long)n0 * (L::Q_IMG / 8)), 0,
+                                             images * (L::Q_IMG / 8) * 4, 0x00020000);
+  };
+  f32x4 fill[NQ];
+  unsigned fbits[DGRAD ? NQ : 1];
+  auto fill_load = [&](int u, __amdgpu_buffer_rsrc_t rx, __amdgpu_buffer_rsrc_t rbits) {
+    fill[u] = __builtin_bit_cast(f32x4, __builtin_amdgcn_raw_buffer_load_b128(rx, tid * 16, u * 4096, 0));
+    if (DGRAD && p.src_bits) fbits[DGRAD ? u : 0] = __builtin_amdgcn_raw_buffer_load_b32(rbits, ((tid + u * 256) >> 3) * 4, 0, 0);
+    else if constexpr (DGRAD && SPLIT_IN_LOOP) fbits[u] = ~0u;
+  };
+  const __amdgpu_buffer_rsrc_t rw = __builtin_amdgcn_make_buffer_rsrc((void *)p.wp, 0, KSTEPS * NT * 3 * 1024, 0x00020000);
+  const int w_lane = lane * 16, w_ct = ct * 3072;
+  auto w_load = [&](int ks, int pl) { return __builtin_amdgcn_raw_buffer_load_b128(rw, w_lane, w_ct + (ks * NT * 3 + pl) * 1024, 0); };
+  u32x4 b[PD][3];
+  auto w_first = [&]() {
+#pragma unroll
+    for (int s = 0; s < PD; ++s)
+#pragma unroll
+      for (int pl = 0; pl < 3; ++pl) b[s][pl] = w_load(s, pl);
+  };
+  f32x4 bias4[4];
+  auto bias_load = [&]() {
+#pragma unroll
+    for (int j = 0; j < 4; ++j)
+      bias4[j] = DGRAD ? f32x4{0.f, 0.f, 0.f, 0.f} : *reinterpret_cast<const f32x4 *>(p.bias + ct * 32 + 8 * j + 4 * half);
+  };
+
+  int grp = blockIdx.x;
 
   if (DGRAD) {
     for (int e = tid; e < 3 * L::PLANE / 16; e += 256) reinterpret_cast<u32x4 *>(lds)[e] = u32x4{0u, 0u, 0u, 0u};
@@ -163,24 +233,10 @@
     }
     return g * L::IMGB + L::slot(y, x) * L::CPB + c4 * 8;
   };
-  auto group_rsrc = [&](int grp) {
-    const bool exists = grp < p.n_groups;
-    const int u0 = exists ? grp * G : 0;
-    const int n0 = u0 / L::NB, b0 = u0 - n0 * L::NB;
-    const long long src = (G == 1 && p.img_index) ? p.img_index[n0] : (long long)n0;
-    const int units = exists ? min(G, p.N * L::NB - u0) : 0;
-    if constexpr (U8)
-      return __builtin_amdgcn_make_buffer_rsrc((void *)(reinterpret_cast<const unsigned char *>(p.x) + src * (L::Q_IMG * 4) + b0 * (L::Q_ROW0 * 4)), 0,
-                                               units * L::Q_UNIT * 4, 0x00020000);
-    else
-      return __builtin_amdgcn_make_buffer_rsrc((void *)(p.x + src * (L::Q_IMG * 4) + b0 * (L::Q_ROW0 * 4)), 0, units * L::Q_UNIT * 16, 0x00020000);
-  };
-  f32x4 fill[NQ];
-  unsigned fbits[DGRAD ? NQ : 1];
   int fdst[NQ];
 #pragma unroll
   for (int u = 0; u < NQ; ++u) fdst[u] = fill_dst(u);
-  auto fill_to_lds = [&]() {
+  auto fill_to_lds = [&](int u0) {
     if constexpr (U8) {
 #pragma unroll
       for (int u = 0; u < NQ; ++u) {
@@ -202,7 +258,7 @@
       return;
     }
 #pragma unroll
-    for (int u = 0; u < NQ; ++u) {
+    for (int u = u0; u < NQ; ++u) {
       if (tid + u * 256 < G * L::Q_UNIT) {
         if (DGRAD && p.src_bits) {
           const unsigned nib = fbits[DGRAD ? u : 0] >> (((tid + u * 256) & 7) * 4);
@@ -219,32 +275,39 @@
       }
     }
   };
-  auto group_bits_rsrc = [&](int grp) {
-    const bool exists = DGRAD && p.src_bits && grp < p.n_groups;
-    const int n0 = exists ? grp * G : 0;
-    const int images = exists ? min(G, p.N - n0) : 0;
-    return __builtin_amdgcn_make_buffer_rsrc((void *)((p.src_bits ? p.src_bits : (const unsigned *)p.x) + (long long)n0 * (L::Q_IMG / 8)), 0,
-                                             images * (L::Q_IMG / 8) * 4, 0x00020000);
-  };
-  auto fill_load = [&](int u, __amdgpu_buffer_rsrc_t rx, __amdgpu_buffer_rsrc_t rbits) {
-    fill[u] = __builtin_bit_cast(f32x4, __builtin_amdgcn_raw_buffer_load_b128(rx, tid * 16, u * 4096, 0));
-    if (DGRAD && p.src_bits) fbits[DGRAD ? u : 0] = __builtin_amdgcn_raw_buffer_load_b32(rbits, ((tid + u * 256) >> 3) * 4, 0, 0);
-  };
-
-  int grp = blockIdx.x;
+  unsigned sp[NSPL ? NSPL : 1][6];
+  auto split_one = [&](int u) {
+    f32x4 v = fill[u];
+    if constexpr (DGRAD) {
+      const unsigned nib = fbits[DGRAD ? u : 0] >> (((tid + u * 256) & 7) * 4);
+#pragma unroll
+      for (int e = 0; e < 4; ++e) v[e] = (nib >> e) & 1u ? v[e] : 0.f;
+    }
+    unsigned(&d)[6] = sp[NSPL ? u : 0];
+    b3_split_pair(v[0], v[1], d[0], d[2], d[4]);
+    b3_split_pair(v[2], v[3], d[1], d[3], d[5]);
+  };
+  auto split_to_lds = [&]() {
+#pragma unroll
+    for (int u = 0; u < NSPL; ++u) {
+      if (tid + u * 256 < G * L::Q_UNIT) {
+        const unsigned(&d)[6] = sp[NSPL ? u : 0];
+        *reinterpret_cast<u32x2 *>(lds + fdst[u]) = u32x2{d[0], d[1]};
+        *reinterpret_cast<u32x2 *>(lds + L::PLANE + fdst[u]) = u32x2{d[2], d[3]};
+        *reinterpret_cast<u32x2 *>(lds + 2 * L::PLANE + fdst[u]) = u32x2{d[4], d[5]};
+      }
+    }
+  };
+
   {
     const __amdgpu_buffer_rsrc_t rx = group_rsrc(grp), rxb = group_bits_rsrc(grp);
 #pragma unroll
     for (int u = 0; u < NQ; ++u) fill_load(u, rx, rxb);
-    fill_to_lds();
-  }
-  f32x4 bias4[4];
-#pragma unroll
-  for (int j = 0; j < 4; ++j)
-    bias4[j] = DGRAD ? f32x4{0.f, 0.f, 0.f, 0.f} : *reinterpret_cast<const f32x4 *>(p.bias + ct * 32 + 8 * j + 4 * half);
-  const __amdgpu_buffer_rsrc_t rw = __builtin_amdgcn_make_buffer_rsrc((void *)p.wp, 0, KSTEPS * NT * 3 * 1024, 0x00020000);
-  const int w_lane = lane * 16, w_ct = ct * 3072;
-  auto w_load = [&](int ks, int pl) { return __builtin_amdgcn_raw_buffer_load_b128(rw, w_lane, w_ct + (ks * NT * 3 + pl) * 1024, 0); };
+  }
+  fill_to_lds(0);
+  bias_load();
+  if constexpr (HOIST_W) w_first();
+  B3_STAMP();
   const __amdgpu_buffer_rsrc_t ro = __builtin_amdgcn_make_buffer_rsrc((void *)p.out, 0, (int)((long long)p.N * L::HRES * L::HRES * L::CRES * 4), 0x00020000);
   const __amdgpu_buffer_rsrc_t rm = __builtin_amdgcn_make_buffer_rsrc((void *)(p.ymask ? p.ymask : p.out), 0,
                                                                        p.ymask ? (int)((long long)p.N * L::HRES * L::HRES * L::CRES * 4) : 0, 0x00020000);
@@ -254,6 +317,7 @@
 
   for (; grp < p.n_groups; grp += gridDim.x) {
     __syncthreads();
+    B3_STAMP();
     const __amdgpu_buffer_rsrc_t nrx = group_rsrc(grp + gridDim.x), nrxb = group_bits_rsrc(grp + gridDim.x);
     int o[TPW];
     unsigned relu_bits[TPW];
@@ -273,11 +337,7 @@
     for (int t = 0; t < TPW; ++t)
 #pragma unroll
       for (int r = 0; r < 16; ++r) acc[t][r] = acs[t][r] = 0.f;
-    u32x4 b[PD][3];
-#pragma unroll
-    for (int s = 0; s < PD; ++s)
-#pragma unroll
-      for (int pl = 0; pl < 3; ++pl) b[s][pl] = w_load(s, pl);
+    if constexpr (!HOIST_W) w_first();
 
     auto read_x = [&](u32x4(&xf)[3], int t, auto ksc) {
       constexpr int ks = decltype(ksc)::value;
@@ -321,17 +381,27 @@
         acs[t] = __builtin_amdgcn_mfma_f32_32x32x16_bf16(w1, x2, acs[t], 0, 0, 0);
         acs[t] = __builtin_amdgcn_mfma_f32_32x32x16_bf16(w2, x1, acs[t], 0, 0, 0);
         acc[t] = __builtin_amdgcn_mfma_f32_32x32x16_bf16(w1, x1, acc[t], 0, 0, 0);
+        if constexpr (SPLIT_IN_LOOP && ks >= KS0) {
+          constexpr int slot = (ks - KS0) * TPW + t;
+#pragma unroll
+          for (int u = slot * FPS; u < (slot + 1) * FPS; ++u)
+            if (u < NSPL) split_one(u);
+        }
         __builtin_amdgcn_sched_barrier(0);
       });
       if constexpr (ks + PD < KSTEPS) {
 #pragma unroll
         for (int pl = 0; pl < 3; ++pl) b[s][pl] = w_load(ks + PD, pl);
       }
-#pragma unroll
-      for (int u = ks * LPK; u < (ks + 1) * LPK; ++u)
-        if (u < NQ) fill_load(u, nrx, nrxb);
+      if constexpr (ks < KS0) {
+#pragma unroll
+        for (int u = ks * LPKS; u < (ks + 1) * LPKS; ++u)
+          if (u < NQ) fill_load(u, nrx, nrxb);
+      }
       __builtin_amdgcn_sched_barrier(0);
     });
+    B3_STAMP();
+    if constexpr (HOIST_W) w_first();
 
     {
       f32x4 mk[2][4];
@@ -373,30 +443,68 @@
       }
     }
 
+    B3_STAMP();
     __syncthreads();
-    fill_to_lds();
-  }
-}
-
-template <class L, bool DGRAD, int C, int S>
+    B3_STAMP();
+    if constexpr (SPLIT_IN_LOOP) split_to_lds();
+    fill_to_lds(NSPL);
+    B3_STAMP();
+  }
+  B3_STAMP_REAL();
+  B3_STAMP_DONE();
+}
+
+}
+
+int etm_b3_schedule_v = 1;
+int etm_b3_grid_cap_v = 0;
+#ifdef ETM_B3_STAMPS
+long long *etm_b3_stamps_v = nullptr;
+extern "C" int etm_conv_b3_stamps(void *buf) { etm_b3_stamps_v = (long long *)buf; return ETM_OK; }
+#endif
+extern "C" int etm_conv_b3_schedule(int schedule) {
+  if (schedule < 0) return etm_b3_schedule_v;
+  if (schedule > 1) return ETM_EINVAL;
+  etm_b3_schedule_v = schedule;
+  return ETM_OK;
+}
+extern "C" int etm_conv_b3_grid_cap(int workgroups) {
+  if (workgroups < 0) return ETM_EINVAL;
+  etm_b3_grid_cap_v = workgroups;
+  return ETM_OK;
+}
+
+namespace {
+template <class L, bool DGRAD, int C, int S, int SCH>
 int launch_b3_geo(const B3Args &p0, hipStream_t st) {
   constexpr int G = L::G, WPC = L::WPC;
   B3Args p = p0;
+#ifdef ETM_B3_STAMPS
+  p.stamps = etm_b3_stamps_v;
+#endif
   if (G > 1 && p.img_index) return ETM_EUNSUPPORTED;
   if ((long long)p.N * L::HRES * L::HRES * L::CRES * 4 >= 0x7ffffff0ll) return ETM_EUNSUPPORTED;
   p.n_groups = (p.N * L::NB + G - 1) / G;
   constexpr size_t lds = 3 * (size_t)L::PLANE;
   static_assert(lds * WPC <= 160 * 1024, "LDS of a CU");
-  auto kern = conv_b3_kernel<L, DGRAD, C, S>;
+  auto kern = conv_b3_kernel<L, DGRAD, C, S, SCH>;
   static bool attr_set = false;
   if (!attr_set) { (void)hipFuncSetAttribute((const void *)kern, hipFuncAttributeMaxDynamicSharedMemorySize, (int)lds); attr_set = true; }
-  const int grid = p.n_groups < 256 * WPC ? p.n_groups : 256 * WPC;
+  int grid = p.n_groups < 256 * WPC ? p.n_groups : 256 * WPC;
+  if (etm_b3_grid_cap_v > 0 && grid > etm_b3_grid_cap_v) grid = etm_b3_grid_cap_v;
   hipLaunchKernelGGL(kern, dim3((unsigned)grid), dim3(256), lds, st, p);
   return etm_launch_status();
 }
-template <bool DGRAD, int C, int HW, int KS, int S, int COUT, int G, int BAND = 0, int WPC = 1, bool SWZ = false>
+template <class L, bool DGRAD, int C, int S, int SCH1 = 0>
+int launch_b3_sched(const B3Args &p, hipStream_t st) {
+  if constexpr (SCH1 != 0) {
+    if (etm_b3_schedule_v) return launch_b3_geo<L, DGRAD, C, S, SCH1>(p, st);
+  }
+  return launch_b3_geo<L, DGRAD, C, S, 0>(p, st);
+}
+template <bool DGRAD, int C, int HW, int KS, int S, int COUT, int G, int BAND = 0, int WPC = 1, bool SWZ = false, int SCH1 = 0>
 int launch_b3(const B3Args &p, hipStream_t st) {
-  return launch_b3_geo<B3Geo<DGRAD, C, HW, KS, S, COUT, G, BAND, WPC, SWZ>, DGRAD, C, S>(p, st);
+  return launch_b3_sched<B3Geo<DGRAD, C, HW, KS, S, COUT, G, BAND, WPC, SWZ>, DGRAD, C, S, SCH1>(p, st);
 }
 
 constexpr int B3_MAXP = 8;
@@ -467,7 +575,7 @@
   EtmProfScope prof(etm_conv_layer_kid(ETM_K_CONV_TRAIN_FWD, ETM_K_CONV_FWD_L1, ETM_K_CONV_FWD_L2, ETM_K_CONV_FWD_L3, KH), st);
   if (C == 3 && H == 84 && KH == 8 && S == 4 && Cout == 32) return launch_b3<false, 3, 84, 8, 4, 32, 1, 10, 2>(p, st);
   if (C == 32 && H == 20 && KH == 4 && S == 2 && Cout == 64) return launch_b3<false, 32, 20, 4, 2, 64, 2, 0, 1, true>(p, st);
-  if (C == 64 && H == 9 && KH == 3 && S == 1 && Cout == 64) return launch_b3<false, 64, 9, 3, 1, 64, 2, 0, 2>(p, st);
+  if (C == 64 && H == 9 && KH == 3 && S == 1 && Cout == 64) return launch_b3<false, 64, 9, 3, 1, 64, 2, 0, 2, false, 2>(p, st);
   return ETM_EUNSUPPORTED;
 }
 
@@ -480,7 +588,7 @@
   hipStream_t st = (hipStream_t)stream;
   B3Args p{reinterpret_cast<const float *>(x), (const long long *)x_index, w_b3, bias, nullptr, nullptr, nullptr, relu_bits, y, N, 0};
   EtmProfScope prof(ETM_K_CONV_FWD_L1, st);
-  return launch_b3_geo<B3GeoBytes<B3Geo<false, 3, 84, 8, 4, 32, 1, 10, 2>>, false, 3, 4>(p, st);
+  return launch_b3_sched<B3GeoBytes<B3Geo<false, 3, 84, 8, 4, 32, 1, 10, 2>>, false, 3, 4>(p, st);
 }
 
 extern "C" int etm_conv_b3_dgrad(const float *dy, const uint32_t *dy_relu_bits, const uint16_t *w_b3, const float *y_below, const uint32_t *relu_bits,
@@ -492,7 +600,7 @@
   hipStream_t st = (hipStream_t)stream;
   B3Args p{dy, nullptr, w_b3, nullptr, y_below, relu_bits, dy_relu_bits, nullptr, dx, N, 0};
   EtmProfScope prof(etm_conv_layer_kid(ETM_K_CONV_TRAIN_DGRAD, -1, ETM_K_CONV_DGRAD_L2, ETM_K_CONV_DGRAD_L3, KH), st);
-  if (C == 32 && H == 20 && KH == 4 && S == 2 && Cout == 64) return launch_b3<true, 32, 20, 4, 2, 64, 2, 0, 1>(p, st);
-  if (C == 64 && H == 9 && KH == 3 && S == 1 && Cout == 64) return launch_b3<true, 64, 9, 3, 1, 64, 3>(p, st);
+  if (C == 32 && H == 20 && KH == 4 && S == 2 && Cout == 64) return launch_b3<true, 32, 20, 4, 2, 64, 2, 0, 1, false, 3>(p, st);
+  if (C == 64 && H == 9 && KH == 3 && S == 1 && Cout == 64) return launch_b3<true, 64, 9, 3, 1, 64, 3, 0, 1, false, 3>(p, st);
   return ETM_EUNSUPPORTED;
 }
diff --git a/episodic-transformer-memory-ppo_amd/csrc/conv_b3_wgrad.hip b/episodic-transformer-memory-ppo_amd/csrc/conv_b3_wgrad.hip
--- a/episodic-transformer-memory-ppo_amd/csrc/conv_b3_wgrad.hip
+++ b/episodic-transformer-memory-ppo_amd/csrc/conv_b3_wgrad.hip
@@ -1,6 +1,11 @@
 #include "etm_common.h"
 
 #include <utility>
+
+extern int etm_b3_grid_cap_v;
+#ifdef ETM_B3_STAMPS
+extern long long *etm_b3_stamps_v;
+#endif
 
 namespace {
 typedef __bf16 bf16x8 __attribute__((ext_vector_type(8)));
@@ -14,7 +19,22 @@
   const unsigned *dy_bits;
   float *partial;
   int N, n_groups;
+#ifdef ETM_B3_STAMPS
+  long long *stamps;
+#endif
 };
+
+#ifdef ETM_B3_STAMPS
+#define W3_STAMP_INIT(p) long long *const stamp_buf = (blockIdx.x == 0 && threadIdx.x == 0) ? (p).stamps : nullptr; int stamp_n = 0
+#define W3_STAMP() do { if (stamp_buf) stamp_buf[++stamp_n] = (long long)__builtin_amdgcn_s_memtime(); } while (0)
+#define W3_STAMP_REAL() do { if (stamp_buf) stamp_buf[++stamp_n] = (long long)__builtin_amdgcn_s_memrealtime(); } while (0)
+#define W3_STAMP_DONE() do { if (stamp_buf) stamp_buf[0] = stamp_n; } while (0)
+#else
+#define W3_STAMP_INIT(p) do { } while (0)
+#define W3_STAMP() do { } while (0)
+#define W3_STAMP_REAL() do { } while (0)
+#define W3_STAMP_DONE() do { } while (0)
+#endif
 
 __device__ __forceinline__ unsigned w3_cvt_pk(float a, float b) {
   unsigned r;
@@ -95,55 +115,10 @@
   const int kt0 = kpart * L::KT / L::KPARTS, nkt = (kpart + 1) * L::KT / L::KPARTS - kt0;
   const int ct0 = L::PSPLIT == 1 ? (wave & 1) : 0;
   const int sp = L::PSPLIT == 1 ? 0 : (wave >> 1);
-
-  for (int e = tid; e < L::LDS / 16; e += NTH) reinterpret_cast<u32x4 *>(lds)[e] = u32x4{0u, 0u, 0u, 0u};
-  __syncthreads();
-
-  const int prow = (lane & 15) >> 2, cofs = ((lane >> 4) & 1) * 16 + (lane & 3) * 4, p8 = (lane >> 5) * 8;
-  const unsigned lds0 = (unsigned)(size_t)lds;
-  unsigned *tabl = reinterpret_cast<unsigned *>(lds + L::LDS);
-  if (wave == 0) {
-#pragma unroll
-    for (int s = 0; s < STEPS; ++s)
-#pragma unroll
-      for (int j = 0; j < 2; ++j) {
-        int m = 16 * s + p8 + 4 * j + prow;
-        if (m >= L::M) m = 0;
-        const int g = m / L::PIX, r = m - g * L::PIX, oy = r / L::HOUT, ox = r - oy * L::HOUT;
-        int b;
-        if (L::THREE) b = g * L::IMGB + ((oy * S * HW + ox * S) * 3) * 2;
-        else b = g * L::IMGB + (S == 2 ? (2 * oy) * HW + ox : (oy * S) * HW + ox * S) * L::CPB + cofs * 2;
-        tabl[(2 * s + j) * 64 + lane] = lds0 + (unsigned)b;
-      }
-  }
-  int koff[KTW];
-#pragma unroll
-  for (int i = 0; i < KTW; ++i) {
-    if (L::THREE) {
-      const int k0 = 32 * (kt0 + i) + cofs, ky = k0 / 24, off = k0 - ky * 24;
-      koff[i] = (ky * HW * 3 + off) * 2;
-    } else {
-      koff[i] = 0;
-#pragma unroll
-      for (int kp = 0; kp < L::KPARTS; ++kp)
-        if (kp == kpart) koff[i] = L::ktile_bytes(kp * L::KT / L::KPARTS + i < L::KT ? kp * L::KT / L::KPARTS + i : 0);
-    }
-  }
-  const unsigned dbase = lds0 + L::XBYTES + (unsigned)((p8 + prow) * L::CPBD + cofs * 2 + ct0 * 64);
-
-  auto x_dst = [&](int u) {
-    const int q = tid + u * NTH;
-    if constexpr (U8) return q * 32;
-    const int g = q / L::QX, qi = q - g * L::QX;
-    if (L::THREE) return g * L::IMGB + qi * 8;
-    const int pix = qi / (C / 4), c4 = qi - pix * (C / 4), y = pix / HW, x = pix - y * HW;
-    return g * L::IMGB + L::slot(y, x) * L::CPB + c4 * 8;
-  };
-  auto d_dst = [&](int u) {
-    const int q = tid + u * NTH;
-    const int pix = q / (COUT / 4), c4 = q - pix * (COUT / 4);
-    return L::XBYTES + pix * L::CPBD + c4 * 8;
-  };
+  W3_STAMP_INIT(p);
+  W3_STAMP_REAL();
+  W3_STAMP();
+
   auto unit_rsrc = [&](int grp, bool grad) {
     const bool exists = grp < p.n_groups;
     const int u0 = exists ? grp * G : 0;
@@ -176,7 +151,56 @@
 #pragma unroll
     for (int u = 0; u < NQX; ++u) fx[u] = __builtin_bit_cast(f32x4, __builtin_amdgcn_raw_buffer_load_b128(rx, tid * 16, u * (NTH * 16), 0));
   };
-  auto put = [&](const f32x4 &v, int d, int plane_bytes) {
+
+  for (int e = tid; e < L::LDS / 16; e += NTH) reinterpret_cast<u32x4 *>(lds)[e] = u32x4{0u, 0u, 0u, 0u};
+  __syncthreads();
+
+  const int prow = (lane & 15) >> 2, cofs = ((lane >> 4) & 1) * 16 + (lane & 3) * 4, p8 = (lane >> 5) * 8;
+  const unsigned lds0 = (unsigned)(size_t)lds;
+  unsigned *tabl = reinterpret_cast<unsigned *>(lds + L::LDS);
+  if (wave == 0) {
+#pragma unroll
+    for (int s = 0; s < STEPS; ++s)
+#pragma unroll
+      for (int j = 0; j < 2; ++j) {
+        int m = 16 * s + p8 + 4 * j + prow;
+        if (m >= L::M) m = 0;
+        const int g = m / L::PIX, r = m - g * L::PIX, oy = r / L::HOUT, ox = r - oy * L::HOUT;
+        int b;
+        if (L::THREE) b = g * L::IMGB + ((oy * S * HW + ox * S) * 3) * 2;
+        else b = g * L::IMGB + (S == 2 ? (2 * oy) * HW + ox : (oy * S) * HW + ox * S) * L::CPB + cofs * 2;
+        tabl[(2 * s + j) * 64 + lane] = lds0 + (unsigned)b;
+      }
+  }
+  int koff[KTW];
+#pragma unroll
+  for (int i = 0; i < KTW; ++i) {
+    if (L::THREE) {
+      const int k0 = 32 * (kt0 + i) + cofs, ky = k0 / 24, off = k0 - ky * 24;
+      koff[i] = (ky * HW * 3 + off) * 2;
+    } else {
+      koff[i] = 0;
+#pragma unroll
+      for (int kp = 0; kp < L::KPARTS; ++kp)
+        if (kp == kpart) koff[i] = L::ktile_bytes(kp * L::KT / L::KPARTS + i < L::KT ? kp * L::KT / L::KPARTS + i : 0);
+    }
+  }
+  const unsigned dbase = lds0 + L::XBYTES + (unsigned)((p8 + prow) * L::CPBD + cofs * 2 + ct0 * 64);
+
+  auto x_dst = [&](int u) {
+    const int q = tid + u * NTH;
+    if constexpr (U8) return q * 32;
+    const int g = q / L::QX, qi = q - g * L::QX;
+    if (L::THREE) return g * L::IMGB + qi * 8;
+    const int pix = qi / (C / 4), c4 = qi - pix * (C / 4), y = pix / HW, x = pix - y * HW;
+    return g * L::IMGB + L::slot(y, x) * L::CPB + c4 * 8;
+  };
+  auto d_dst = [&](int u) {
+    const int q = tid + u * NTH;
+    const int pix = q / (COUT / 4), c4 = q - pix * (COUT / 4);
+    return L::XBYTES + pix * L::CPBD + c4 * 8;
+  };
+  auto put =[&](const f32x4 &v, int d, int plane_bytes) {
     unsigned h0, m0, l0, h1, m1, l1;
     w3_split_pair(v[0], v[1], h0, m0, l0);
     w3_split_pair(v[2], v[3], h1, m1, l1);
@@ -223,8 +247,10 @@
   int grp = blockIdx.x;
   issue_fill(grp);
   fill_to_lds();
+  W3_STAMP();
   for (; grp < p.n_groups; grp += gridDim.x) {
     __syncthreads();
+    W3_STAMP();
     issue_fill(grp + gridDim.x);
 
     unsigned t0 = 0, t1 = 0;
@@ -282,9 +308,14 @@
       });
     });
 
+    W3_STAMP();
     __syncthreads();
+    W3_STAMP();
     fill_to_lds();
-  }
+    W3_STAMP();
+  }
+  W3_STAMP_REAL();
+  W3_STAMP_DONE();
 
 #pragma unroll
   for (int i = 0; i < KTW; ++i)
@@ -346,12 +377,16 @@
   static_assert(LDS_ALL * WPC <= 160 * 1024, "LDS of a CU");
   static int slices(int N) {
     const int groups = (N * L::NB + G - 1) / G;
-    return groups < 256 * WPC ? groups : 256 * WPC;
+    const int grid = groups < 256 * WPC ? groups : 256 * WPC;
+    return etm_b3_grid_cap_v > 0 && grid > etm_b3_grid_cap_v ? etm_b3_grid_cap_v : grid;
   }
   static int launch(const W3Args &p0, hipStream_t st) {
     W3Args p = p0;
     if (G > 1 && p.img_index) return ETM_EUNSUPPORTED;
     p.n_groups = (p.N * L::NB + G - 1) / G;
+#ifdef ETM_B3_STAMPS
+    p.stamps = etm_b3_stamps_v;
+#endif
     auto kern = conv_b3_wgrad_kernel<L, C, HW, S, COUT>;
     static bool attr_set = false;
     if (!attr_set) { (void)hipFuncSetAttribute((const void *)kern, hipFuncAttributeMaxDynamicSharedMemorySize, (int)LDS_ALL); attr_set = true; }
diff --git a/episodic-transformer-memory-ppo_amd/etm/lib.py b/episodic-transformer-memory-ppo_amd/etm/lib.py
--- a/episodic-transformer-memory-ppo_amd/etm/lib.py
+++ b/episodic-transformer-memory-ppo_amd/etm/lib.py
@@ -131,7 +131,9 @@
     "etm_conv_b3_dgrad": (_I, [_P, _P, _P, _P, _P, _P, _I, _I, _I, _I, _I, _I, _I, _I, _P]),
     "etm_conv_b3_wgrad_slices": (_I, [_I] * 8),
     "etm_conv_b3_wgrad": (_I, [_P, _P, _P, _P, _P, _L, _I, _I, _I, _I, _I, _I, _I, _I, _P]),
-    "etm_bytes_to_unit": (_I, [_P, _P, _P, _L, _L, _P]),
+    "etm_conv_b3_schedule": (_I, [_I]),
+    "etm_conv_b3_grid_cap": (_I, [_I]),
+    "etm_bytes_to_unit":(_I, [_P, _P, _P, _L, _L, _P]),
     "etm_conv_relu_u8": (_I, [_P, _P, _L, _P, _P, _P, _I, _I, _I, _I, _I, _I, _I, _I, _I, _I, _P]),
     "etm_conv_b3_fwd_u8": (_I, [_P, _P, _P, _P, _P, _P, _I, _I, _I, _I, _I, _I, _I, _I, _P]),
     "etm_conv_b3_wgrad_u8": (_I, [_P, _P, _P, _P, _P, _L, _I, _I, _I, _I, _I, _I, _I, _I, _P]),
diff --git a/episodic-transformer-memory-ppo_amd/trainer.py b/episodic-transformer-memory-ppo_amd/trainer.py
--- a/episodic-transformer-memory-ppo_amd/trainer.py
+++ b/episodic-transformer-memory-ppo_amd/trainer.py
@@ -307,6 +307,11 @@
         self._masked = check_action_mask_config(config, self.env, self.action_space_shape, self.box is not None)
         self.last_valid_action_share = None
         self._kl_analytic = check_kl_estimator_config(config, self.box is not None, 1 if dp is None else int(getattr(dp, "world", 1))) == "analytic"
+
+        self._encoder_schedule = int(config.get("encoder_schedule", 1))
+        if self._encoder_schedule not in (0, 1):
+            raise ValueError(f"encoder_schedule: 0 or 1, not {config.get('encoder_schedule')!r}")
+        etm_lib.check(etm_lib.load().etm_conv_b3_schedule(self._encoder_schedule), "etm_conv_b3_schedule")
 
         if config.get("tunable_gemm", os.environ.get("ETM_TUNABLE_GEMM", "1") != "0"):
             try:
@@ -1027,6 +1032,7 @@
 
     def _train_epochs(self, learning_rate: float, clip_range: float, beta: float, perms=None):
         stats, norms = [], []
+        etm_lib.load().etm_conv_b3_schedule(self._encoder_schedule)
         monitor = self.config.get("monitor_gradients", True)
         with torch.no_grad():
             self._bank_pos = self._bank_with_positions()
diff --git a/include/etm_hip.h b/include/etm_hip.h
--- a/include/etm_hip.h
+++ b/include/etm_hip.h
@@ -409,6 +409,8 @@
 int etm_conv_b3_wgrad_slices(int N, int C, int H, int W, int Cout, int KH, int KW, int S);
 int etm_conv_b3_wgrad(const float *x, const int64_t *x_index, const float *dy, const uint32_t *dy_relu_bits, float *workspace,
                       int64_t workspace_bytes, int N, int C, int H, int W, int Cout, int KH, int KW, int S, void *stream);
+int etm_conv_b3_schedule(int schedule);
+int etm_conv_b3_grid_cap(int workgroups);
 
 int etm_bytes_to_unit(const uint8_t *src, const int64_t *index, float *dst, int64_t rows, int64_t row_bytes, void *stream);
 int etm_conv_relu_u8(const uint8_t *in, const int64_t *in_index, int64_t in_index_stride, const float *w, const float *bias, float *out,
```
